# LFY1998/IPDM-PyTorch

Measured on AMD Instinct MI355X. Metric: CT slices/s (full proj+img partial-diffusion sample), higher is better.
Workload: dtype f32

## Files before the change

### include/ipdm_hip.h

```cpp
#ifndef IPDM_HIP_H
#define IPDM_HIP_H
#include <stddef.h>
#include <stdint.h>

#ifdef __cplusplus
extern "C" {
#endif

#define IPDM_OK 0
#define IPDM_ERR_INVALID (-1)
#define IPDM_ERR_HIP (-2)
#define IPDM_ERR_WORKSPACE (-3)
#define IPDM_ERR_UNSUPPORTED (-4)

const char *ipdm_last_error(void);
#define IPDM_ABI_VERSION 5
int ipdm_abi_version(void);

int ipdm_set_option(const char *name, int value);
int ipdm_get_option(const char *name, int *value);

typedef struct ipdm_fbp_geom {
    int32_t n_views, n_det, grid_n;
    double da, det_offset, dtheta_deg, source_origin, fov_half;
// ... 73 lines not shown
                       void *d_ws, size_t ws_bytes, void *stream);

typedef struct ipdm_reverse_args {
    int32_t mode;
    int32_t clip;
    int32_t guidance;
    double constant_guidance, lambda_power, eta;
    int32_t kernel_size;
    double amplitude;
    double p1[5], p2[3];
    uint64_t seed;
    int64_t slice_id0, draw0;
    const float *d_noise;
    const float *d_ldct;
} ipdm_reverse_args;

size_t ipdm_reverse_workspace_bytes(ipdm_unet *net, int32_t B, int32_t H, int32_t W);

int ipdm_reverse_pass(const ipdm_schedule *s, ipdm_unet *net, const float *d_x_in, const float *d_guide,
                      const float *d_Lambda, int32_t mh, int32_t mw, float *d_iter, int32_t B, int32_t H, int32_t W,
                      int32_t ts, const ipdm_reverse_args *a, void *d_ws, size_t ws_bytes, void *stream);

int ipdm_guided_reverse(const ipdm_schedule *s, ipdm_unet *net, const float *d_img, float *d_iters, int32_t B,
                        int32_t H, int32_t W, const int32_t *t_start, int32_t n_pass, const ipdm_reverse_args *a,
                        int64_t *draws_used, void *d_ws, size_t ws_bytes, void *stream);

#define IPDM_SLICE_IDS_MAX 64
int ipdm_randn_ids(float *d_out, int32_t B, int64_t n, uint64_t seed, const int64_t *slice_ids, int64_t draw,
                   void *stream);
int ipdm_q_sample_rng_ids(const ipdm_schedule *s, int32_t t, const float *d_x, float *d_out, int32_t B,
                          int64_t n_per_slice, uint64_t seed, const int64_t *slice_ids, int64_t draw, void *stream);
int ipdm_ddpm_step_rng_ids(const ipdm_schedule *s, int32_t t, const float *d_eps_pred, const float *d_x_t,
                           const float *d_x0, uint64_t seed, const int64_t *slice_ids, int64_t draw, float *d_out,
                           int32_t B, int32_t H, int32_t W, double lambda_scalar, const float *d_lambda_map, int32_t mh,
                           int32_t mw, int32_t clip_denoised, void *d_ws, size_t ws_bytes, void *stream);
int ipdm_reverse_pass_ids(const ipdm_schedule *s, ipdm_unet *net, const float *d_x_in, const float *d_guide,
                          const float *d_Lambda, int32_t mh, int32_t mw, float *d_iter, int32_t B, int32_t H, int32_t W,
                          int32_t ts, const ipdm_reverse_args *a, const int64_t *slice_ids, void *d_ws, size_t ws_bytes,
                          void *stream);

int ipdm_ddim_step_rng(const ipdm_schedule *s, int32_t t, int32_t t_prev, const float *d_eps_pred, const float *d_x_t,
                       const float *d_cond, uint64_t seed, int64_t slice_id0, int64_t draw, float *d_out, int32_t B,
                       int64_t n_per_slice, double lambda_scalar, double ddim_eta, int32_t clip_denoised, void *d_ws,
                       size_t ws_bytes, void *stream);

int ipdm_ddim_sequence(const char *method, int32_t timesteps, int32_t t_start, int32_t n, int32_t *seq, int32_t *prev);

#define IPDM_NOISE_COUNTER 1
#define IPDM_NOISE_INJECTED 2
typedef struct ipdm_sparse_args {
    int32_t clip_denoised;
    double ddim_eta, eta;
    int32_t noise;
    uint64_t seed;
    int64_t slice_id0, draw0;
    const float *d_noise;
} ipdm_sparse_args;

int ipdm_sparse_reverse(const ipdm_schedule *s, ipdm_unet *net, const float *d_cond, float *d_iters, int32_t B, int32_t H,
                        int32_t W, int32_t t_q, const int32_t *n_steps, int32_t n_pass, const int32_t *t_seq,
                        const int32_t *t_prev, const double *lambda, const ipdm_sparse_args *a, int64_t *draws_used,
                        void *d_ws, size_t ws_bytes, void *stream);

int ipdm_q_sample_rng_ts(const ipdm_schedule *s, const int32_t *ts, const float *d_x, float *d_out, int32_t B,
                         int64_t n_per_slice, uint64_t seed, const int64_t *slice_ids, int64_t draw, void *stream);
int ipdm_q_sample_ts(const ipdm_schedule *s, const int32_t *ts, const float *d_x, const float *d_noise, float *d_out, int32_t B,
                     int64_t n_per_slice, void *stream);
size_t ipdm_eps_sse_workspace_bytes(int32_t B);
int ipdm_eps_sse(const float *d_eps_pred, const float *d_noise, double *d_sse, int32_t B, int64_t n_per_slice, void *d_ws,
                 size_t ws_bytes, void *stream);
int ipdm_eps_sse_rng(const float *d_eps_pred, double *d_sse, int32_t B, int64_t n_per_slice, uint64_t seed,
                     const int64_t *slice_ids, int64_t draw, void *d_ws, size_t ws_bytes, void *stream);
size_t ipdm_eps_loss_workspace_bytes(ipdm_unet *net, int32_t B, int32_t H, int32_t W);
int ipdm_eps_loss(const ipdm_schedule *s, ipdm_unet *net, const float *d_x0, const int32_t *ts, double *d_sse, int32_t B,
                  int32_t H, int32_t W, uint64_t seed, const int64_t *slice_ids, int64_t draw, const float *d_noise, void *d_ws,
                  size_t ws_bytes, void *stream);

size_t ipdm_conv2d_grad_workspace_bytes(int32_t B, int32_t Cin, int32_t Cout, int32_t H, int32_t W, int32_t ksize,
                                        int32_t stride);
int32_t ipdm_conv2d_wgrad_slabs(int32_t B, int32_t Ho, int32_t Wo);
int ipdm_conv2d_fprop(const float *d_x, const float *d_w, const float *d_b, float *d_y, int32_t B, int32_t Cin, int32_t Cout,
                      int32_t H, int32_t W, int32_t ksize, int32_t stride, void *d_ws, size_t ws_bytes, void *stream);
int ipdm_conv2d_dgrad(const float *d_dy, const float *d_w, float *d_dx, int32_t B, int32_t Cin, int32_t Cout, int32_t H,
                      int32_t W, int32_t ksize, int32_t stride, void *d_ws, size_t ws_bytes, void *stream);
int ipdm_conv2d_wgrad(const float *d_x, const float *d_dy, float *d_dw, float *d_db, int32_t B, int32_t Cin, int32_t Cout,
                      int32_t H, int32_t W, int32_t ksize, int32_t stride, void *d_ws, size_t ws_bytes, void *stream);

int32_t ipdm_conv2d_wgrad_tuned_code(int32_t B, int32_t Cin, int32_t Cout, int32_t H, int32_t W, int32_t ksize, int32_t stride);
#define IPDM_WGRAD_PLAN_FIELDS 14
int32_t ipdm_conv2d_wgrad_tuned_plan(int32_t B, int32_t Cin, int32_t Cout, int32_t H, int32_t W, int32_t ksize, int32_t stride,
                                     int32_t *out, int32_t n);
#define IPDM_WGRAD_LAUNCH_FIELDS 9
int32_t ipdm_conv2d_wgrad_tuned_launch(int32_t B, int32_t Cin, int32_t Cout, int32_t H, int32_t W, int32_t ksize, int32_t stride,
                                       int32_t *out, int32_t n);
size_t ipdm_conv2d_wgrad_tuned_workspace_bytes(int32_t B, int32_t Cin, int32_t Cout, int32_t H, int32_t W, int32_t ksize,
                                               int32_t stride);
int ipdm_conv2d_wgrad_tuned(const float *d_x, const float *d_dy, float *d_dw, float *d_db, int32_t B, int32_t Cin, int32_t Cout,
                            int32_t H, int32_t W, int32_t ksize, int32_t stride, void *d_ws, size_t ws_bytes, void *stream);

int32_t ipdm_conv2d_wgrad_wino_code(int32_t B, int32_t Cin, int32_t Cout, int32_t H, int32_t W, int32_t ksize, int32_t stride);
#define IPDM_WGRAD_WINO_PLAN_FIELDS 11
int32_t ipdm_conv2d_wgrad_wino_plan(int32_t B, int32_t Cin, int32_t Cout, int32_t H, int32_t W, int32_t ksize, int32_t stride,
                                    int32_t *out, int32_t n);
size_t ipdm_conv2d_wgrad_wino_workspace_bytes(int32_t B, int32_t Cin, int32_t Cout, int32_t H, int32_t W, int32_t ksize,
                                              int32_t stride);
int ipdm_conv2d_wgrad_wino(const float *d_x, const float *d_dy, float *d_dw, float *d_db, int32_t B, int32_t Cin, int32_t Cout,
                           int32_t H, int32_t W, int32_t ksize, int32_t stride, void *d_ws, size_t ws_bytes, void *stream);

int32_t ipdm_conv2d_tuned_code(int32_t role, int32_t B, int32_t Cin, int32_t Cout, int32_t H, int32_t W, int32_t ksize, int32_t stride);
size_t ipdm_conv2d_tuned_workspace_bytes(int32_t role, int32_t B, int32_t Cin, int32_t Cout, int32_t H, int32_t W, int32_t ksize,
                                         int32_t stride);
int ipdm_conv2d_fprop_tuned(const float *d_x, const float *d_w, const float *d_b, float *d_y, int32_t B, int32_t Cin, int32_t Cout,
                            int32_t H, int32_t W, int32_t ksize, int32_t stride, void *d_ws, size_t ws_bytes, void *stream);
int ipdm_conv2d_dgrad_tuned(const float *d_dy, const float *d_w, float *d_dx, int32_t B, int32_t Cin, int32_t Cout, int32_t H,
                            int32_t W, int32_t ksize, int32_t stride, void *d_ws, size_t ws_bytes, void *stream);
size_t ipdm_conv_image_bytes(int32_t image, int32_t role, int32_t Cin, int32_t Cout, int32_t ksize, int32_t stride);
int ipdm_conv_pack_device(int32_t image, int32_t role, const float *d_w, int32_t Cin, int32_t Cout, int32_t ksize, int32_t stride,
                          void *d_image, void *stream);
int ipdm_conv_pack_host(int32_t image, int32_t role, const float *w_host, int32_t Cin, int32_t Cout, int32_t ksize, int32_t stride,
                        void *image_host);

size_t ipdm_gn_act_workspace_bytes(int32_t B, int32_t C, int32_t groups, int32_t HW);
int32_t ipdm_gn_act_plan(int32_t C, int32_t groups, int32_t HW, int32_t *split);
int ipdm_gn_act_fprop(const float *d_x, const float *d_shift, const float *d_gamma, const float *d_beta, float *d_y,
                      double *d_stats, int32_t B, int32_t C, int32_t groups, int32_t HW, double eps, int32_t act, void *d_ws,
                      size_t ws_bytes, void *stream);
int ipdm_gn_act_bgrad(const float *d_x, const float *d_shift, const float *d_gamma, const float *d_beta, const double *d_stats,
                      const float *d_dy, float *d_dx, float *d_dgamma, float *d_dbeta, float *d_dshift, int32_t B, int32_t C,
                      int32_t groups, int32_t HW, double eps, int32_t act, void *d_ws, size_t ws_bytes, void *stream);

size_t ipdm_attn_train_workspace_bytes(int32_t B, int32_t heads, int32_t d, int32_t T);
int32_t ipdm_attn_train_plan(int32_t d, int32_t T, int32_t out[4]);
int ipdm_attn_fprop(const float *d_qkv, float *d_out, float *d_lse, int32_t B, int32_t heads, int32_t d, int32_t T, void *d_ws,
                    size_t ws_bytes, void *stream);
int ipdm_attn_bgrad(const float *d_qkv, const float *d_out, const float *d_lse, const float *d_dout, float *d_dqkv, int32_t B,
                    int32_t heads, int32_t d, int32_t T, void *d_ws, size_t ws_bytes, void *stream);

int ipdm_op_conv2d(const float *d_x1, int32_t C1, const float *d_x2, int32_t C2, int32_t B, int32_t Hs,
                   int32_t Ws, int32_t H, int32_t W, const float *w_host, const float *b_host, int32_t Cout,
                   int32_t ksize, int32_t stride, int32_t act, int32_t groups, const float *gamma_host,
                   const float *beta_host, const float *d_res, float *d_out, void *stream);
int ipdm_op_conv_gn_conv(const float *d_x, int32_t C, int32_t B, int32_t H, int32_t W, const float *wA_host,
                         const float *bA_host, int32_t CA, int32_t ksA, int32_t strideA, const float *d_resA,
                         int32_t groups, const float *gamma_host, const float *beta_host, int32_t act,
                         const float *wB_host, const float *bB_host, int32_t CB, float *d_mid, float *d_out,
                         int32_t *fused_rows, void *stream);
int ipdm_op_up_conv_chain(const float *d_x, int32_t C, int32_t B, int32_t Hs, int32_t Ws, const float *wA_host,
                          const float *bA_host, int32_t CA, const float *d_skip, int32_t C2, int32_t groups,
                          const float *gamma_host, const float *beta_host, int32_t act, const float *wB_host,
                          const float *bB_host, int32_t CB, int32_t ksB, float *d_mid, float *d_out,
                          int32_t *used_up2, void *stream);
int ipdm_op_attention(const float *d_qkv, float *d_out, int32_t B, int32_t heads, int32_t d, int32_t T,
                      void *stream);

typedef struct ipdm_art_geom {
    float dso, dsd;
    int32_t nx, ny;
    float dx, dy, offset_x, offset_y;
    int32_t nr;
    float dr, offset_r, angle_start;
    int32_t na, ta_dimx, ta_dimy;
    float ta_deltax, ta_deltay;
} ipdm_art_geom;
typedef struct ipdm_art_plan ipdm_art_plan;
int ipdm_art_plan_create(const ipdm_art_geom *geom, const float *lut_area_host, const float *betas_host,
                         ipdm_art_plan **out);
int ipdm_art_plan_destroy(ipdm_art_plan *plan);
size_t ipdm_art_workspace_bytes(const ipdm_art_plan *plan, int32_t B);
int32_t ipdm_art_plan_info(const ipdm_art_plan *plan, int32_t out[6]);
int ipdm_art_reconstruct(ipdm_art_plan *plan, const float *d_proj, float *d_volume, int32_t B, int32_t nsart,
                         int32_t ntv, int32_t sample_rate, void *d_ws, size_t ws_bytes, void *stream);
int ipdm_art_project(ipdm_art_plan *plan, const float *d_volume, float *d_proj, int32_t B, void *d_ws,
                     size_t ws_bytes, void *stream);

#define IPDM_METRIC_PSNR 1u
#define IPDM_METRIC_SSIM 2u
#define IPDM_METRIC_FSIM 4u
#define IPDM_METRIC_VIF 8u
#define IPDM_METRIC_NQM 16u
typedef struct ipdm_metrics_plan ipdm_metrics_plan;
int ipdm_metrics_plan_create(int32_t H, int32_t W, ipdm_metrics_plan **out);
int ipdm_metrics_plan_destroy(ipdm_metrics_plan *plan);
size_t ipdm_metrics_workspace_bytes(const ipdm_metrics_plan *plan, int32_t B, uint32_t mask);
int ipdm_metrics(ipdm_metrics_plan *plan, const float *d_ref, int64_t ref_stride, const float *d_img, int32_t B,
                 uint32_t mask, double *d_out, void *d_ws, size_t ws_bytes, void *stream);
int64_t ipdm_metrics_table(const ipdm_metrics_plan *plan, int32_t which, void *host_out, int64_t cap_elems);

int ipdm_lowdose_noise(const float *d_proj, const float *d_z1, const float *d_z2, float *d_out, int32_t B,
                       int64_t n_per_slice, double factor, double n0, double ne, int32_t model, void *stream);
int ipdm_lowdose_noise_rng(const float *d_proj, float *d_out, int32_t B, int64_t n_per_slice, double factor, double n0,
                           double ne, int32_t model, uint64_t seed, int64_t slice_id0, int64_t draw0, void *stream);

size_t ipdm_yj_workspace_bytes(int32_t B);
int ipdm_yj_nll(const float *d_x, int32_t B, int64_t n_per_slice, const double *lambdas_host, double *nll_host, void *d_ws,
                size_t ws_bytes, void *stream);
int ipdm_yj_fit(const float *d_x, int32_t B, int64_t n_per_slice, double *params_host, int32_t *evals_host, void *d_ws,
                size_t ws_bytes, void *stream);
int ipdm_yj_apply(const float *d_x, float *d_out, int32_t B, int64_t n_per_slice, const double *params_host, void *stream);
int ipdm_yj_invert(const float *d_y, float *d_out, int32_t B, int64_t n_per_slice, const double *params_host, void *stream);
int ipdm_yj_fit_host(const float *x_host, int32_t B, int64_t n_per_slice, double *params_host, int32_t *evals_host);

typedef struct ipdm_adam_tensor {
    float *p;
    const float *g;
    float *m, *v;
    int64_t n;
} ipdm_adam_tensor;
typedef struct ipdm_adam_chunk {
    int32_t tensor, len;
    int64_t offset;
} ipdm_adam_chunk;
#define IPDM_ADAM_CHUNK 4096
int64_t ipdm_adam_chunks(const int64_t *sizes, int32_t n_tensors, ipdm_adam_chunk *out, int64_t cap);
int ipdm_adam_step(const ipdm_adam_tensor *d_tensors, int32_t n_tensors, const ipdm_adam_chunk *d_chunks, int64_t n_chunks,
                   double lr, double beta1, double beta2, double eps, double weight_decay, int64_t step, void *stream);
int ipdm_grad_sumsq(const ipdm_adam_tensor *d_tensors, int32_t n_tensors, const ipdm_adam_chunk *d_chunks, int64_t n_chunks,
                    double *d_partials, void *stream);
int ipdm_grad_clip_coef(const double *d_partials, int64_t n_partials, double max_norm, double *d_norm, float *d_coef, void *stream);
int ipdm_adam_step_ex(const ipdm_adam_tensor *d_tensors, int32_t n_tensors, const ipdm_adam_chunk *d_chunks, int64_t n_chunks,
                      double lr, double beta1, double beta2, double eps, double weight_decay, int64_t step,
                      const float *d_gscale, float *const *d_ema, double ema_decay, void *stream);
#define IPDM_CROP_MAX 256
int ipdm_crop_patches(const float *d_slices, float *d_out, int32_t n, int32_t m, int32_t H, int32_t W, int32_t ph, int32_t pw,
                      const int32_t *offsets_host, int32_t div10, void *stream);

#define IPDM_PROF_CLASSES 8
int ipdm_profile_begin(int32_t max_launches);
int ipdm_profile_begin_classes(int32_t max_launches, uint32_t class_mask);
int ipdm_profile_end(double *out_flops, double *out_ms, int64_t *out_launches, int32_t n_classes);
int ipdm_clock_probe(uint64_t *d_out, int32_t samples, int32_t period_us, void *stream);

int ipdm_bench_conv2d(int32_t B, int32_t C1, int32_t C2, int32_t H, int32_t W, int32_t Cout, int32_t ksize,
                      int32_t stride, int32_t act, int32_t with_res, int32_t iters, float *avg_ms);
int ipdm_bench_attention(int32_t B, int32_t heads, int32_t d, int32_t T, int32_t iters, float *avg_ms);
int32_t ipdm_conv_layout_code(int32_t Cout, int32_t ksize, int32_t stride);
int32_t ipdm_conv_kernel_code(int32_t B, int32_t Cout, int32_t Cin, int32_t ksize, int32_t stride, int32_t H, int32_t W);
int32_t ipdm_conv_kernel_code_stats(int32_t B, int32_t Cout, int32_t Cin, int32_t ksize, int32_t stride, int32_t H, int32_t W);
int32_t ipdm_attention_kernel_code(int32_t d);
int ipdm_attention_plan(int32_t B, int32_t heads, int32_t d, int32_t T, int32_t out[6]);

#ifdef __cplusplus
}
#endif
#endif
```

### ipdm-pytorch_amd/_lib.py

```python
import ctypes as C
import os

_HERE = os.path.dirname(os.path.abspath(__file__))
LIB_PATH = os.environ.get("IPDM_LIB_PATH") or os.path.join(_HERE, "libipdm_hip.so")


class IpdmError(RuntimeError):
    pass


class FbpGeom(C.Structure):
    _fields_ = [("n_views", C.c_int32), ("n_det", C.c_int32), ("grid_n", C.c_int32),
                ("da", C.c_double), ("det_offset", C.c_double), ("dtheta_deg", C.c_double),
                ("source_origin", C.c_double), ("fov_half", C.c_double)]


class UnetCfg(C.Structure):
    _fields_ = [("in_channels", C.c_int32), ("model_channels", C.c_int32), ("out_channels", C.c_int32),
                ("num_res_blocks", C.c_int32), ("num_heads", C.c_int32), ("n_mult", C.c_int32),
                ("n_attn", C.c_int32), ("channel_mult", C.c_double * 16),
                ("attention_resolutions", C.c_int32 * 16)]


class ReverseArgs(C.Structure):
    _fields_ = [("mode", C.c_int32), ("clip", C.c_int32), ("guidance", C.c_int32),
                ("constant_guidance", C.c_double), ("lambda_power", C.c_double), ("eta", C.c_double),
                ("kernel_size", C.c_int32), ("amplitude", C.c_double),
                ("p1", C.c_double * 5), ("p2", C.c_double * 3),
                ("seed", C.c_uint64), ("slice_id0", C.c_int64), ("draw0", C.c_int64),
                ("d_noise", C.c_void_p), ("d_ldct", C.c_void_p)]


class SparseArgs(C.Structure):
    _fields_ = [("clip_denoised", C.c_int32), ("ddim_eta", C.c_double), ("eta", C.c_double), ("noise", C.c_int32),
                ("seed", C.c_uint64), ("slice_id0", C.c_int64), ("draw0", C.c_int64), ("d_noise", C.c_void_p)]


NOISE_COUNTER, NOISE_INJECTED = 1, 2

_vp, _i32, _i64, _u64, _f32, _f64, _sz = C.c_void_p, C.c_int32, C.c_int64, C.c_uint64, C.c_float, C.c_double, C.c_size_t

ABI_VERSION = 5
PROF_CLASSES = 8
SLICE_IDS_MAX = 64
ADAM_CHUNK = 4096

PROTOTYPES = {
    "ipdm_last_error": (C.c_char_p, []),
    "ipdm_abi_version": (C.c_int, []),
    "ipdm_set_option": (C.c_int, [C.c_char_p, _i32]),
    "ipdm_get_option": (C.c_int, [C.c_char_p, C.POINTER(_i32)]),
    "ipdm_fbp_plan_create": (C.c_int, [C.POINTER(FbpGeom), C.POINTER(_vp)]),
    "ipdm_fbp_plan_destroy": (C.c_int, [_vp]),
    "ipdm_fbp_workspace_bytes": (_sz, [_vp, _i32]),
    "ipdm_fbp_forward": (C.c_int, [_vp, _vp, _vp, _i32, _i32, _f32, _vp, _sz, _vp]),
    "ipdm_fbp_filter": (C.c_int, [_vp, _vp, _vp, _i32, _i32, _f32, _vp]),
    "ipdm_fbp_backproject": (C.c_int, [_vp, _vp, _vp, _i32, _i32, _vp]),
    "ipdm_fbp_index_map": (C.c_int, [_vp, _vp, _i32, _vp, _vp]),
    "ipdm_fbp_table": (_i64, [_vp, _i32, _vp, _i64]),
    "ipdm_sharpen3x3": (C.c_int, [_vp, _vp, _i32, _i32, _i32, _f32, _vp]),
    "ipdm_schedule_create": (C.c_int, [_i32, _f64, C.POINTER(_vp)]),
    "ipdm_schedule_destroy": (C.c_int, [_vp]),
    "ipdm_schedule_coeffs": (C.c_int, [_vp, _i32, C.POINTER(_f32 * 8)]),
    "ipdm_schedule_alpha_cumprod": (C.c_int, [_vp, _i32, C.POINTER(_f32)]),
    "ipdm_cosine_lambda": (C.c_int, [_i32, _f64, _i32, C.POINTER(_f64)]),
    "ipdm_ddim_step": (C.c_int, [_vp, _i32, _i32, _vp, _vp, _vp, _vp, _vp, _i32, _i64, _f64, _f64, _i32, _vp, _sz, _vp]),
    "ipdm_randn": (C.c_int, [_vp, _i32, _i64, _u64, _i64, _i64, _vp]),
    "ipdm_q_sample": (C.c_int, [_vp, _i32, _vp, _vp, _vp, _i64, _vp]),
    "ipdm_ddpm_workspace_bytes": (_sz, [_i32]),
    "ipdm_ddpm_step": (C.c_int, [_vp, _i32, _vp, _vp, _vp, _vp, _vp, _i32, _i32, _i32, _f64, _vp, _i32, _i32,
                                 _i32, _vp, _sz, _vp]),
    "ipdm_clamp": (C.c_int, [_vp, _vp, _i64, _i32, _vp]),
    "ipdm_axpbypcz": (C.c_int, [_vp, _vp, _vp, _vp, _i64, _f64, _f64, _f64, _vp]),
    "ipdm_guidance_workspace_bytes": (_sz, [_i32, _i32, _i32]),
    "ipdm_guidance_map": (C.c_int, [_vp, _vp, _vp, _vp, _i32, _i32, _i32, _i32, _f64, _i32, C.POINTER(_f64),
                                    C.POINTER(_f64), _vp, _sz, _vp]),
    "ipdm_lambda_ratio": (C.c_int, [_vp, _vp, _i64, _i32, _i32, _vp]),
    "ipdm_slice_median": (C.c_int, [_vp, _vp, _i32, _i64, _vp, _sz, _vp]),
    "ipdm_unet_param_count": (C.c_int, [C.POINTER(UnetCfg)]),
    "ipdm_unet_param_info": (C.c_int, [C.POINTER(UnetCfg), _i32, C.c_char_p, _i32, C.POINTER(_i32 * 4),
                                       C.POINTER(_i32)]),
    "ipdm_unet_create": (C.c_int, [C.POINTER(UnetCfg), C.POINTER(_vp), _i32, C.POINTER(_vp)]),
    "ipdm_unet_destroy": (C.c_int, [_vp]),
    "ipdm_unet_workspace_bytes": (_sz, [_vp, _i32, _i32, _i32]),
    "ipdm_unet_forward": (C.c_int, [_vp, _vp, _i32, _vp, _i32, _i32, _i32, _vp, _sz, _vp]),
    "ipdm_unet_forward_graph": (C.c_int, [_vp, _vp, _i32, _vp, _i32, _i32, _i32, _vp, _sz, _vp]),
    "ipdm_q_sample_rng": (C.c_int, [_vp, _i32, _vp, _vp, _i32, _i64, _u64, _i64, _i64, _vp]),
    "ipdm_ddpm_step_rng": (C.c_int, [_vp, _i32, _vp, _vp, _vp, _u64, _i64, _i64, _vp, _i32, _i32, _i32, _f64, _vp, _i32, _i32,
                                     _i32, _vp, _sz, _vp]),
    "ipdm_reverse_workspace_bytes": (_sz, [_vp, _i32, _i32, _i32]),
    "ipdm_reverse_pass": (C.c_int, [_vp, _vp, _vp, _vp, _vp, _i32, _i32, _vp, _i32, _i32, _i32, _i32, C.POINTER(ReverseArgs),
                                    _vp, _sz, _vp]),
    "ipdm_guided_reverse": (C.c_int, [_vp, _vp, _vp, _vp, _i32, _i32, _i32, C.POINTER(_i32), _i32, C.POINTER(ReverseArgs),
                                      C.POINTER(_i64), _vp, _sz, _vp]),
    "ipdm_randn_ids": (C.c_int, [_vp, _i32, _i64, _u64, C.POINTER(_i64), _i64, _vp]),
    "ipdm_q_sample_rng_ids": (C.c_int, [_vp, _i32, _vp, _vp, _i32, _i64, _u64, C.POINTER(_i64), _i64, _vp]),
    "ipdm_ddpm_step_rng_ids": (C.c_int, [_vp, _i32, _vp, _vp, _vp, _u64, C.POINTER(_i64), _i64, _vp, _i32, _i32, _i32, _f64, _vp,
                                         _i32, _i32, _i32, _vp, _sz, _vp]),
    "ipdm_reverse_pass_ids": (C.c_int, [_vp, _vp, _vp, _vp, _vp, _i32, _i32, _vp, _i32, _i32, _i32, _i32, C.POINTER(ReverseArgs),
                                        C.POINTER(_i64), _vp, _sz, _vp]),
    "ipdm_ddim_step_rng": (C.c_int, [_vp, _i32, _i32, _vp, _vp, _vp, _u64, _i64, _i64, _vp, _i32, _i64, _f64, _f64, _i32, _vp, _sz,
                                     _vp]),
    "ipdm_ddim_sequence": (C.c_int, [C.c_char_p, _i32, _i32, _i32, C.POINTER(_i32), C.POINTER(_i32)]),
    "ipdm_sparse_reverse": (C.c_int, [_vp, _vp, _vp, _vp, _i32, _i32, _i32, _i32, C.POINTER(_i32), _i32, C.POINTER(_i32),
                                      C.POINTER(_i32), C.POINTER(_f64), C.POINTER(SparseArgs), C.POINTER(_i64), _vp, _sz, _vp]),
    "ipdm_q_sample_rng_ts": (C.c_int, [_vp, C.POINTER(_i32), _vp, _vp, _i32, _i64, _u64, C.POINTER(_i64), _i64, _vp]),
    "ipdm_q_sample_ts": (C.c_int, [_vp, C.POINTER(_i32), _vp, _vp, _vp, _i32, _i64, _vp]),
    "ipdm_eps_sse_workspace_bytes": (_sz, [_i32]),
    "ipdm_eps_sse": (C.c_int, [_vp, _vp, _vp, _i32, _i64, _vp, _sz, _vp]),
    "ipdm_eps_sse_rng": (C.c_int, [_vp, _vp, _i32, _i64, _u64, C.POINTER(_i64), _i64, _vp, _sz, _vp]),
    "ipdm_eps_loss_workspace_bytes": (_sz, [_vp, _i32, _i32, _i32]),
    "ipdm_eps_loss": (C.c_int, [_vp, _vp, _vp, C.POINTER(_i32), _vp, _i32, _i32, _i32, _u64, C.POINTER(_i64), _i64, _vp, _vp, _sz,
                                _vp]),
    "ipdm_conv2d_grad_workspace_bytes": (_sz, [_i32] * 7),
    "ipdm_conv2d_wgrad_slabs": (_i32, [_i32, _i32, _i32]),
    "ipdm_conv2d_fprop": (C.c_int, [_vp, _vp, _vp, _vp] + [_i32] * 7 + [_vp, _sz, _vp]),
    "ipdm_conv2d_dgrad": (C.c_int, [_vp, _vp, _vp] + [_i32] * 7 + [_vp, _sz, _vp]),
    "ipdm_conv2d_wgrad": (C.c_int, [_vp, _vp, _vp, _vp] + [_i32] * 7 + [_vp, _sz, _vp]),
    "ipdm_conv2d_wgrad_tuned_code": (_i32, [_i32] * 7),
    "ipdm_conv2d_wgrad_tuned_plan": (_i32, [_i32] * 7 + [C.POINTER(_i32), _i32]),
    "ipdm_conv2d_wgrad_tuned_launch": (_i32, [_i32] * 7 + [C.POINTER(_i32), _i32]),
    "ipdm_conv2d_wgrad_tuned_workspace_bytes": (_sz, [_i32] * 7),
    "ipdm_conv2d_wgrad_tuned": (C.c_int, [_vp, _vp, _vp, _vp] + [_i32] * 7 + [_vp, _sz, _vp]),
    "ipdm_conv2d_wgrad_wino_code": (_i32, [_i32] * 7),
    "ipdm_conv2d_wgrad_wino_plan": (_i32, [_i32] * 7 + [C.POINTER(_i32), _i32]),
    "ipdm_conv2d_wgrad_wino_workspace_bytes": (_sz, [_i32] * 7),
    "ipdm_conv2d_wgrad_wino": (C.c_int, [_vp, _vp, _vp, _vp] + [_i32] * 7 + [_vp, _sz, _vp]),
    "ipdm_conv2d_tuned_code": (_i32, [_i32] * 8),
    "ipdm_conv2d_tuned_workspace_bytes": (_sz, [_i32] * 8),
    "ipdm_conv2d_fprop_tuned": (C.c_int, [_vp, _vp, _vp, _vp] + [_i32] * 7 + [_vp, _sz, _vp]),
    "ipdm_conv2d_dgrad_tuned": (C.c_int, [_vp, _vp, _vp] + [_i32] * 7 + [_vp, _sz, _vp]),
    "ipdm_conv_image_bytes": (_sz, [_i32] * 6),
    "ipdm_conv_pack_device": (C.c_int, [_i32, _i32, _vp] + [_i32] * 4 + [_vp, _vp]),
    "ipdm_conv_pack_host": (C.c_int, [_i32, _i32, _vp] + [_i32] * 4 + [_vp]),
    "ipdm_gn_act_workspace_bytes": (_sz, [_i32] * 4),
    "ipdm_gn_act_plan": (_i32, [_i32, _i32, _i32, C.POINTER(_i32)]),
    "ipdm_gn_act_fprop": (C.c_int, [_vp] * 6 + [_i32] * 4 + [_f64, _i32, _vp, _sz, _vp]),
    "ipdm_gn_act_bgrad": (C.c_int, [_vp] * 10 + [_i32] * 4 + [_f64, _i32, _vp, _sz, _vp]),
    "ipdm_attn_train_workspace_bytes": (_sz, [_i32] * 4),
    "ipdm_attn_train_plan": (_i32, [_i32, _i32, C.POINTER(_i32 * 4)]),
    "ipdm_attn_fprop": (C.c_int, [_vp] * 3 + [_i32] * 4 + [_vp, _sz, _vp]),
    "ipdm_attn_bgrad": (C.c_int, [_vp] * 5 + [_i32] * 4 + [_vp, _sz, _vp]),
    "ipdm_op_conv2d": (C.c_int, [_vp, _i32, _vp, _i32, _i32, _i32, _i32, _i32, _i32, _vp, _vp, _i32, _i32, _i32,
                                 _i32, _i32, _vp, _vp, _vp, _vp, _vp]),
    "ipdm_op_conv_gn_conv": (C.c_int, [_vp, _i32, _i32, _i32, _i32, _vp, _vp, _i32, _i32, _i32, _vp, _i32, _vp, _vp, _i32, _vp, _vp,
                                       _i32, _vp, _vp, C.POINTER(_i32), _vp]),
    "ipdm_op_up_conv_chain": (C.c_int, [_vp, _i32, _i32, _i32, _i32, _vp, _vp, _i32, _vp, _i32, _i32, _vp, _vp, _i32, _vp, _vp,
                                        _i32, _i32, _vp, _vp, C.POINTER(_i32), _vp]),
    "ipdm_profile_begin": (C.c_int, [_i32]),
    "ipdm_profile_begin_classes": (C.c_int, [_i32, C.c_uint32]),
    "ipdm_clock_probe": (C.c_int, [_vp, _i32, _i32, _vp]),
    "ipdm_profile_end": (C.c_int, [C.POINTER(_f64 * PROF_CLASSES), C.POINTER(_f64 * PROF_CLASSES), C.POINTER(_i64 * PROF_CLASSES), _i32]),
    "ipdm_bench_conv2d": (C.c_int, [_i32] * 11 + [C.POINTER(_f32)]),
    "ipdm_bench_attention": (C.c_int, [_i32] * 5 + [C.POINTER(_f32)]),
    "ipdm_op_attention": (C.c_int, [_vp, _vp, _i32, _i32, _i32, _i32, _vp]),
    "ipdm_conv_layout_code": (_i32, [_i32, _i32, _i32]),
    "ipdm_conv_kernel_code": (_i32, [_i32, _i32, _i32, _i32, _i32, _i32, _i32]),
    "ipdm_conv_kernel_code_stats": (_i32, [_i32, _i32, _i32, _i32, _i32, _i32, _i32]),
    "ipdm_attention_kernel_code": (_i32, [_i32]),
    "ipdm_attention_plan": (C.c_int, [_i32, _i32, _i32, _i32, C.POINTER(_i32 * 6)]),
    "ipdm_art_plan_create": (C.c_int, [_vp, _vp, _vp, C.POINTER(_vp)]),
    "ipdm_art_plan_destroy": (C.c_int, [_vp]),
    "ipdm_art_workspace_bytes": (C.c_size_t, [_vp, _i32]),
    "ipdm_art_plan_info": (_i32, [_vp, C.POINTER(_i32 * 6)]),
    "ipdm_art_reconstruct": (C.c_int, [_vp, _vp, _vp, _i32, _i32, _i32, _i32, _vp, C.c_size_t, _vp]),
    "ipdm_art_project": (C.c_int, [_vp, _vp, _vp, _i32, _vp, C.c_size_t, _vp]),
    "ipdm_metrics_plan_create": (C.c_int, [_i32, _i32, C.POINTER(_vp)]),
    "ipdm_metrics_plan_destroy": (C.c_int, [_vp]),
    "ipdm_metrics_workspace_bytes": (_sz, [_vp, _i32, C.c_uint32]),
    "ipdm_metrics": (C.c_int, [_vp, _vp, _i64, _vp, _i32, C.c_uint32, _vp, _vp, _sz, _vp]),
    "ipdm_metrics_table": (_i64, [_vp, _i32, _vp, _i64]),
    "ipdm_lowdose_noise": (C.c_int, [_vp, _vp, _vp, _vp, _i32, _i64, _f64, _f64, _f64, _i32, _vp]),
    "ipdm_lowdose_noise_rng": (C.c_int, [_vp, _vp, _i32, _i64, _f64, _f64, _f64, _i32, _u64, _i64, _i64, _vp]),
    "ipdm_yj_workspace_bytes": (_sz, [_i32]),
    "ipdm_yj_nll": (C.c_int, [_vp, _i32, _i64, C.POINTER(_f64), C.POINTER(_f64), _vp, _sz, _vp]),
    "ipdm_yj_fit": (C.c_int, [_vp, _i32, _i64, C.POINTER(_f64), C.POINTER(_i32), _vp, _sz, _vp]),
    "ipdm_yj_apply": (C.c_int, [_vp, _vp, _i32, _i64, C.POINTER(_f64), _vp]),
    "ipdm_yj_invert": (C.c_int, [_vp, _vp, _i32, _i64, C.POINTER(_f64), _vp]),
    "ipdm_yj_fit_host": (C.c_int, [_vp, _i32, _i64, C.POINTER(_f64), C.POINTER(_i32)]),
    "ipdm_adam_chunks": (_i64, [_vp, _i32, _vp, _i64]),
    "ipdm_adam_step": (C.c_int, [_vp, _i32, _vp, _i64, _f64, _f64, _f64, _f64, _f64, _i64, _vp]),
    "ipdm_grad_sumsq": (C.c_int, [_vp, _i32, _vp, _i64, _vp, _vp]),
    "ipdm_grad_clip_coef": (C.c_int, [_vp, _i64, _f64, _vp, _vp, _vp]),
    "ipdm_adam_step_ex": (C.c_int, [_vp, _i32, _vp, _i64, _f64, _f64, _f64, _f64, _f64, _i64, _vp, _vp, _f64, _vp]),
    "ipdm_crop_patches": (C.c_int, [_vp, _vp] + [_i32] * 6 + [_vp, _i32, _vp]),
}

_lib = None


def lib():
    global _lib
    if _lib is None:
        if not os.path.isfile(LIB_PATH):
            raise IpdmError("%s not found: the HIP extension is mandatory (no CPU fallback). "
                            "Run __graft_entry__.build()." % LIB_PATH)
        try:
            import torch
        except ImportError:
            pass
        handle = C.CDLL(LIB_PATH)
        for name, (res, args) in PROTOTYPES.items():
            fn = getattr(handle, name)
            fn.restype = res
            fn.argtypes = args
        got = handle.ipdm_abi_version()
        if got != ABI_VERSION:
            raise IpdmError("%s has ABI version %d, this package binds version %d (include/ipdm_hip.h): rebuild with "
                            "__graft_entry__.build()" % (LIB_PATH, got, ABI_VERSION))
        _lib = handle
    return _lib


def call(name, *args):
    rc = getattr(lib(), name)(*args)
    if rc != 0:
        raise IpdmError("%s failed (%d): %s" % (name, rc, lib().ipdm_last_error().decode()))
    return rc


def set_option(name, value):
    old = get_option(name)
    call("ipdm_set_option", name.encode(), int(value))
    return old


def get_option(name):
    v = C.c_int32()
    call("ipdm_get_option", name.encode(), C.byref(v))
    return v.value


class option:

    def __init__(self, name, value):
        self.name, self.value = name, value

    def __enter__(self):
        self.old = set_option(self.name, self.value)
        return self

    def __exit__(self, *exc):
        set_option(self.name, self.old)
        return False


def ptr(t):
    if t is None:
        return None
    if hasattr(t, "data_ptr"):
        assert t.is_contiguous(), "non-contiguous tensor handed to the C ABI"
        return C.c_void_p(t.data_ptr())
    return C.c_void_p(t.ctypes.data)


def current_stream():
    import torch
    return C.c_void_p(torch.cuda.current_stream().cuda_stream)
```

### ipdm-pytorch_amd/csrc/attn.hip

```cpp
#include <cstdlib>
#include "unet_kernels.h"
#include "attn_common.h"

using namespace ipdm;
using namespace ipdm::attn;

namespace {

constexpr int KV = 64;
constexpr int KP = 68;
constexpr int VP = 68;

template <int D, int QT>
__global__ void __launch_bounds__(256, 2) attention_kernel(const float *__restrict__ qkv, float *__restrict__ out,
                                                           int heads, int T, float scale)
{
    __shared__ __attribute__((aligned(16))) float k_lds[KV * KP];
    __shared__ __attribute__((aligned(16))) float v_lds[D * VP];
    const int tid = threadIdx.x, lane = tid & 63, wave = tid >> 6;
    const int l31 = lane & 31, lh = lane >> 5;
    const int bh = blockIdx.y;
    const int b = bh / heads, head = bh % heads;
    const float *qp = qkv + ((size_t)b * heads * 3 * D + (size_t)head * 3 * D) * T;
    const float *kp = qp + (size_t)D * T;
// ... 299 lines not shown
#pragma unroll
    for (int qt = 0; qt < QT; ++qt) {
        const int t = t0 + qt * 32 + l31;
        if (t < T) {
            constexpr bool seq = ZSEQ;
            const float inv = 1.0f / (seq ? den : l_run[qt]);
#pragma unroll
            for (int cb = 0; cb < CB; ++cb)
#pragma unroll
                for (int r = 0; r < 16; ++r) {
                    const int c = cb * 32 + crow(r, lh);
                    op[(size_t)c * T + t] = (seq ? num[seq ? cb : 0][r] : o[qt][cb][r]) * inv;
                }
        }
    }
}

template <int D>
__global__ void __launch_bounds__(256) attention_combine_kernel(const float *__restrict__ part, float *__restrict__ out, int T, int Z, int ntiles)
{
    const int t = blockIdx.x * 256 + threadIdx.x, bh = blockIdx.y, c0 = blockIdx.z * 16;
    if (t >= T) return;
    const size_t slice = (size_t)gridDim.y * (D + 2) * T;
    const float *p = part + (size_t)bh * (D + 2) * T;
    const int tps = (ntiles + Z - 1) / Z;
    SliceWeights w[8];
    float M = -INFINITY, den = 0.0f;
#pragma unroll
    for (int z = 0; z < 8; ++z)
        if (z < Z && z * tps < ntiles) {
            w[z] = slice_weights(M, p[z * slice + (size_t)D * T + t]);
            den = slice_fold(den, p[z * slice + (size_t)(D + 1) * T + t], w[z]);
        }
    const float inv = 1.0f / den;
#pragma unroll 4
    for (int c = c0; c < c0 + 16; ++c) {
        float acc = 0.0f;
#pragma unroll
        for (int z = 0; z < 8; ++z)
            if (z < Z && z * tps < ntiles) acc = slice_fold(acc, p[z * slice + (size_t)c * T + t], w[z]);
        out[((size_t)bh * D + c) * T + t] = acc * inv;
    }
}

__global__ void __launch_bounds__(256) attention_combine_any_kernel(const float *__restrict__ part, float *__restrict__ out, int T, int Z, int ntiles, int d)
{
    const int t = blockIdx.x * 256 + threadIdx.x, bh = blockIdx.y, c0 = blockIdx.z * 16;
    if (t >= T) return;
    const size_t slice = (size_t)gridDim.y * (d + 2) * T;
    const float *p = part + (size_t)bh * (d + 2) * T;
    const int tps = (ntiles + Z - 1) / Z;
    SliceWeights w[8];
    float M = -INFINITY, den = 0.0f;
#pragma unroll
    for (int z = 0; z < 8; ++z)
        if (z < Z && z * tps < ntiles) {
            w[z] = slice_weights(M, p[z * slice + (size_t)d * T + t]);
            den = slice_fold(den, p[z * slice + (size_t)(d + 1) * T + t], w[z]);
        }
    const float inv = 1.0f / den;
    for (int c = c0; c < min(c0 + 16, d); ++c) {
        float acc = 0.0f;
#pragma unroll
        for (int z = 0; z < 8; ++z)
            if (z < Z && z * tps < ntiles) acc = slice_fold(acc, p[z * slice + (size_t)c * T + t], w[z]);
        out[((size_t)bh * d + c) * T + t] = acc * inv;
    }
}

int attention_kv_split(int B, int heads, int d, int T)
{
    const bool off = opt(OPT_ATTN_NO_KVSPLIT) != 0;
    (void)B;
    if (off || d != 64) return 1;
    const long wg = (long)cdiv(T, 128) * heads;
    if (wg > 128) return 1;
    const int ntiles = cdiv(T, KV);
    int Z = wg <= 32 ? 8 : (wg <= 64 ? 4 : 2);
    if (Z > ntiles / 2) Z = ntiles / 2;
    return Z < 2 ? 1 : Z;
}

struct AttnPlan {
    int family;
    int qt;
    int Z;
    int form;
    int tps;
    int empty;
};

bool attention_on_gen(int d)
{
    const int any = opt(OPT_ATTN_ANY_DIM);
    return any == 2 || (any == 1 && d != 64 && d != 32);
}

int attention_head_dim_check(int d)
{
    if (opt(OPT_ATTN_ANY_DIM) == 0) {
        if (d != 64 && d != 32) { set_error("attention: head dim %d unsupported (kernel is specialised for 64 and 32)", d); return IPDM_ERR_UNSUPPORTED; }
    } else if (d < 1 || d > ATTN_GEN_DMAX) {
        set_error("attention: head dim %d unsupported (1 .. %d under attn_any_dim)", d, ATTN_GEN_DMAX);
        return IPDM_ERR_UNSUPPORTED;
    }
    return IPDM_OK;
}

AttnPlan attention_plan(int B, int heads, int d, int T, bool have_scratch)
{
    const int ntiles = cdiv(T, KV);
    AttnPlan p = {0, 1, 1, 0, ntiles, 0};
    if (attention_on_gen(d)) {
        p.family = 3;
        p.Z = have_scratch ? attention_gen_split(heads, d, T) : 1;
        if (p.Z > 1) {
            p.form = 1;
            p.tps = cdiv(ntiles, p.Z);
            p.empty = p.Z - cdiv(ntiles, p.tps);
        }
        return p;
    }
    if (d != 64) return p;
    const long wg2 = (long)cdiv(T, 256) * B * heads, wg1 = (long)cdiv(T, 128) * B * heads;
    if (opt(OPT_ATTN_LEGACY) != 0) {
        p.qt = wg2 >= 512 && (wg2 % 512 == 0 || wg2 >= 4 * 512) ? 2 : 1;
        return p;
    }
    const bool exact = opt(OPT_ATTN_EXACT_F32) != 0;
    p.family = exact ? 1 : 2;
    p.Z = have_scratch ? attention_kv_split(B, heads, d, T) : 1;
    if (exact) {
        const auto eff = [](long wg) { return (double)wg / (double)(((wg + 255) / 256) * 256); };
        if (p.Z == 1 && wg2 >= 256 && eff(wg2) >= eff(wg1) - 0.03) p.qt = 2;
    }
    if (p.Z > 1) {
        p.form = p.Z >= 4 && opt(OPT_ATTN_NO_ZSEQ) == 0 && wg1 >= 192 ? 2 : 1;
        p.tps = cdiv(ntiles, p.Z);
        p.empty = p.Z - cdiv(ntiles, p.tps);
    }
    return p;
}

}

namespace ipdm {

size_t attention_scratch_floats(int B, int heads, int d, int T)
{
    const int Z = attention_on_gen(d) ? attention_gen_split(heads, d, T) : attention_kv_split(B, heads, d, T);
    return Z > 1 ? (size_t)Z * B * heads * (d + 2) * T : 0;
}

int attention_launch(const float *qkv, float *out, int B, int heads, int d, int T, hipStream_t st, float *scratch, float *planes)
{
    IPDM_REQUIRE(qkv && out && B > 0 && heads > 0 && T > 0, "attention: bad argument");
    if (int rc = attention_head_dim_check(d)) return rc;
    const float scale = (float)(1.0 / sqrt(sqrt((double)d)));
    const bool prof = prof_enabled();
    if (prof) prof_before(2, st);
    const AttnPlan p = attention_plan(B, heads, d, T, scratch != nullptr);
    const int Z = p.Z;
    const bool seq = p.form == 2, q2 = p.qt == 2;
    if (p.family == 3) {
        if (int rc = attention_gen_launch(qkv, out, B, heads, d, T, scale, Z, scratch, st)) return rc;
        if (p.form == 1)
            hipLaunchKernelGGL(attention_combine_any_kernel, dim3(cdiv(T, 256), B * heads, cdiv(d, 16)), dim3(256), 0, st, scratch, out, T, Z, cdiv(T, KV), d);
    } else if (p.family == 2) {
        if (!attention_planes_floats(B, heads, d, T)) planes = nullptr;
        attention_bx3_launch(qkv, out, B, heads, T, scale, Z, seq, scratch, planes, st);
        if (p.form == 1)
            hipLaunchKernelGGL((attention_combine_kernel<64>), dim3(cdiv(T, 256), B * heads, 4), dim3(256), 0, st, scratch, out, T, Z, cdiv(T, KV));
    } else if (p.family == 1) {
        constexpr size_t lds = (size_t)2 * (KV * KP + 64 * VP) * sizeof(float);
        if (int rc = ensure_dynamic_lds((const void *)attention_ws_kernel<64, 1>, lds)) return rc;
        if (int rc = ensure_dynamic_lds((const void *)attention_ws_kernel<64, 2>, lds)) return rc;
        if (int rc = ensure_dynamic_lds((const void *)attention_ws_kernel<64, 1, true>, lds)) return rc;
        dim3 grid(cdiv(T, q2 ? 256 : 128), B * heads, seq ? 1 : Z);
        if (q2) hipLaunchKernelGGL((attention_ws_kernel<64, 2>), grid, dim3(512), lds, st, qkv, out, heads, T, scale, 1, (float *)nullptr, 1);
        else if (seq) hipLaunchKernelGGL((attention_ws_kernel<64, 1, true>), grid, dim3(512), lds, st, qkv, out, heads, T, scale, 1, (float *)nullptr, Z);
        else hipLaunchKernelGGL((attention_ws_kernel<64, 1>), grid, dim3(512), lds, st, qkv, out, heads, T, scale, Z, scratch, 1);
        if (p.form == 1)
            hipLaunchKernelGGL((attention_combine_kernel<64>), dim3(cdiv(T, 256), B * heads, 4), dim3(256), 0, st, scratch, out, T, Z, cdiv(T, KV));
    } else if (d == 64) {
        dim3 grid(cdiv(T, q2 ? 256 : 128), B * heads);
        if (q2) hipLaunchKernelGGL((attention_kernel<64, 2>), grid, dim3(256), 0, st, qkv, out, heads, T, scale);
        else hipLaunchKernelGGL((attention_kernel<64, 1>), grid, dim3(256), 0, st, qkv, out, heads, T, scale);
    } else {
        dim3 grid(cdiv(T, 128), B * heads);
        hipLaunchKernelGGL((attention_kernel<32, 1>), grid, dim3(256), 0, st, qkv, out, heads, T, scale);
    }
    if (prof) prof_after(2, 4.0 * B * heads * (double)T * T * d, st);
    IPDM_LAUNCH_CHECK();
    return IPDM_OK;
}

}

extern "C" int32_t ipdm_attention_kernel_code(int32_t d)
{
    if (opt(OPT_ATTN_ANY_DIM) != 0 && (d < 1 || d > ATTN_GEN_DMAX)) return 0;
    return d == 64 || attention_on_gen(d) ? attention_plan(1, 1, d, 1, true).family : 0;
}

extern "C" int ipdm_attention_plan(int32_t B, int32_t heads, int32_t d, int32_t T, int32_t out[6])
{
    IPDM_REQUIRE(out && B > 0 && heads > 0 && T > 0, "attention_plan: bad argument");
    if (int rc = attention_head_dim_check(d)) return rc;
    const AttnPlan p = attention_plan(B, heads, d, T, true);
    out[0] = p.family; out[1] = p.qt; out[2] = p.Z; out[3] = p.form; out[4] = p.tps; out[5] = p.empty;
    return IPDM_OK;
}

extern "C" int ipdm_op_attention(const float *d_qkv, float *d_out, int32_t B, int32_t heads, int32_t d, int32_t T,
                                 void *stream)
{
    float *scratch = nullptr, *planes = nullptr;
    if (ipdm::attention_scratch_floats(B, heads, d, T)) {
        IPDM_HIP_CHECK(hipMalloc((void **)&scratch, ipdm::attention_scratch_floats(B, heads, d, T) * sizeof(float)));
    }
    if (const size_t pfl = ipdm::attention_planes_floats(B, heads, d, T)) {
        hipError_t e = hipMalloc((void **)&planes, pfl * sizeof(float));
        if (e == hipSuccess) e = hipMemsetAsync(planes, 0xFF, pfl * sizeof(float), (hipStream_t)stream);
        if (e != hipSuccess) { (void)hipFree(scratch); (void)hipFree(planes); IPDM_HIP_CHECK(e); }
    }
    const int rc = ipdm::attention_launch(d_qkv, d_out, B, heads, d, T, (hipStream_t)stream, scratch, planes);
    if (scratch || planes) {
        (void)hipStreamSynchronize((hipStream_t)stream);
        (void)hipFree(scratch);
        (void)hipFree(planes);
    }
    return rc;
}
```

### ipdm-pytorch_amd/csrc/attn_bx3.hip

```cpp
#include "unet_kernels.h"
#include "attn_common.h"
#include "attn_pipe_schedule.h"
#include <type_traits>

using namespace ipdm;
using namespace ipdm::attn;

typedef unsigned u32x4 __attribute__((ext_vector_type(4)));
typedef __bf16 bf16x8 __attribute__((ext_vector_type(8)));
typedef __bf16 bf16x2 __attribute__((ext_vector_type(2)));

namespace {

constexpr int D = 64;
constexpr int KT = 32;
constexpr int KP = 72;
constexpr int VP = 40;
constexpr int KPLANE = KT * KP, VPLANE = D * VP;
constexpr int STAGE = 3 * KPLANE + 3 * VPLANE;
constexpr int PCHUNK = 256;
constexpr int TILE_CHUNKS = 6 * PCHUNK;

__device__ inline unsigned pk_bf16(float a, float b)
{
    return __builtin_bit_cast(unsigned, bf16x2{(__bf16)a, (__bf16)b});
}
struct Split3 { unsigned h[3]; };
__device__ inline Split3 split3(float a, float b)
{
    Split3 s;
    s.h[0] = pk_bf16(a, b);
    const float ra = a - __builtin_bit_cast(float, s.h[0] << 16), rb = b - __builtin_bit_cast(float, s.h[0] & 0xffff0000u);
    s.h[1] = pk_bf16(ra, rb);
    const float qa = ra - __builtin_bit_cast(float, s.h[1] << 16), qb = rb - __builtin_bit_cast(float, s.h[1] & 0xffff0000u);
    s.h[2] = pk_bf16(qa, qb);
    return s;
}

__device__ inline f32x16 mma(u32x4 a, u32x4 b, f32x16 c)
{
    return __builtin_amdgcn_mfma_f32_32x32x16_bf16(__builtin_bit_cast(bf16x8, a), __builtin_bit_cast(bf16x8, b), c, 0, 0, 0);
}
template <bool FIRST>
__device__ inline f32x16 mma6(const u32x4 (&a)[3], const u32x4 (&b)[3], f32x16 c)
{
    if (FIRST) {
        const f32x16 zero = {0, 0, 0, 0, 0, 0, 0, 0, 0, 0, 0, 0, 0, 0, 0, 0};
        c = mma(a[0], b[2], zero);
        asm volatile("" ::"v"(a[0]), "v"(b[2]));
    } else {
        c = mma(a[0], b[2], c);
    }
    c = mma(a[2], b[0], c);
    c = mma(a[1], b[1], c);
    c = mma(a[0], b[1], c);
    c = mma(a[1], b[0], c);
    return mma(a[0], b[0], c);
}

template <int FROM, int TO, class F>
__device__ inline void static_for(F &&f)
{
    if constexpr (FROM < TO) {
        f(std::integral_constant<int, FROM>{});
        static_for<FROM + 1, TO>(f);
    }
}

__global__ void __launch_bounds__(256) attention_presplit_kernel(const float *__restrict__ qkv, u32x4 *__restrict__ planes, int heads, int T)
{
    constexpr int FP = KT + 1;
    __shared__ float kf[D * FP], vf[D * FP];
    const int bh = blockIdx.y, b = bh / heads, head = bh % heads;
    const float *qp = qkv + ((size_t)b * heads * 3 * D + (size_t)head * 3 * D) * T;
    const int s0 = blockIdx.x * KT, tid = threadIdx.x;
    {
        const int key = tid & 31, c0 = tid >> 5;
        const bool in = s0 + key < T;
#pragma unroll
        for (int r = 0; r < 8; ++r) {
            const int c = c0 + 8 * r;
            kf[c * FP + key] = in ? qp[(size_t)(D + c) * T + s0 + key] : 0.0f;
            vf[c * FP + key] = in ? qp[(size_t)(2 * D + c) * T + s0 + key] : 0.0f;
        }
    }
    __syncthreads();
    u32x4 *pt = planes + ((size_t)bh * gridDim.x + blockIdx.x) * TILE_CHUNKS + tid;
    const int ks = tid >> 3, kg = tid & 7, vc = tid >> 2, vg = tid & 3;
    const int vkey = 16 * (vg >> 1) + 4 * (vg & 1);
    u32x4 hk[3], hv[3];
#pragma unroll
    for (int e = 0; e < 8; e += 2) {
        const Split3 sk = split3(kf[(8 * kg + e) * FP + ks], kf[(8 * kg + e + 1) * FP + ks]);
        const Split3 sv = split3(vf[vc * FP + vkey + 8 * (e >> 2) + (e & 3)], vf[vc * FP + vkey + 8 * (e >> 2) + (e & 3) + 1]);
#pragma unroll
        for (int p = 0; p < 3; ++p) { hk[p][e / 2] = sk.h[p]; hv[p][e / 2] = sv.h[p]; }
    }
#pragma unroll
    for (int p = 0; p < 3; ++p) {
        pt[p * PCHUNK] = hk[p];
        pt[(3 + p) * PCHUNK] = hv[p];
    }
}

template <bool ZSEQ, bool PRE, bool PIPE>
__global__ void __launch_bounds__(384, 3) attention_bx3_kernel(const float *__restrict__ qkv, float *__restrict__ out, int heads, int T,
                                                                float scale, int zsplit, float *__restrict__ part, int zseq,
                                                                const u32x4 *__restrict__ planes)
{
    static_assert(PRE || !PIPE, "the pipelined loop copies planes");
    static_assert(!ZSEQ || !PIPE, "the pipelined loop does not fit the slice walk's registers");
    __shared__ __attribute__((aligned(16))) unsigned short lds[2 * STAGE];
    const int bh = blockIdx.y;
    const int b = bh / heads, head = bh % heads;
    const float *qp = qkv + ((size_t)b * heads * 3 * D + (size_t)head * 3 * D) * T;
    const int ntiles = (T + KT - 1) / KT;
    const int nslice = ZSEQ ? zseq : zsplit;
    const int tps = 2 * (((T + 63) / 64 + nslice - 1) / nslice);
    const int it0 = ZSEQ ? 0 : blockIdx.z * tps, it1 = ZSEQ ? ntiles : min(ntiles, it0 + tps);
    const int npipe = max(it1 - it0, 0);

    if (__builtin_amdgcn_readfirstlane(threadIdx.x >> 6) >= 4) {
        if constexpr (PRE) {
            const int tid = threadIdx.x - 256;
            const __amdgpu_buffer_rsrc_t rs = __builtin_amdgcn_make_buffer_rsrc((void *)(planes + (size_t)bh * ntiles * TILE_CHUNKS), 0,
                                                                                  ntiles * TILE_CHUNKS * 16, 0x00020000);
            int ko[2], vo[2];
#pragma unroll
            for (int n = 0; n < 2; ++n) {
                const int j = tid + 128 * n;
                ko[n] = (j >> 3) * KP + 8 * (j & 7);
                vo[n] = 3 * KPLANE + (j >> 2) * VP + 8 * (j & 3);
            }
            u32x4 r[12];
            const auto load = [&](int it) {
#pragma unroll
                for (int i = 0; i < 12; ++i)
                    r[i] = __builtin_bit_cast(u32x4, __builtin_amdgcn_raw_buffer_load_b128(rs, tid * 16, (it * TILE_CHUNKS + 128 * i) * 16, 0));
            };
            const auto store = [&](int it) {
                unsigned short *st = lds + (it & 1) * STAGE;
#pragma unroll
                for (int i = 0; i < 6; ++i) {
                    *reinterpret_cast<u32x4 *>(st + (i >> 1) * KPLANE + ko[i & 1]) = r[i];
                    *reinterpret_cast<u32x4 *>(st + (i >> 1) * VPLANE + vo[i & 1]) = r[6 + i];
                }
            };
            if constexpr (PIPE) {
                const auto load_half = [&](int it, int h) {
#pragma unroll
                    for (int i = 6 * h; i < 6 * h + 6; ++i)
                        r[i] = __builtin_bit_cast(u32x4, __builtin_amdgcn_raw_buffer_load_b128(rs, tid * 16, (it * TILE_CHUNKS + 128 * i) * 16, 0));
                };
                const auto store_k = [&](int it) {
                    unsigned short *st = lds + attn_pipe::slot(it) * STAGE;
#pragma unroll
                    for (int i = 0; i < 6; ++i) *reinterpret_cast<u32x4 *>(st + (i >> 1) * KPLANE + ko[i & 1]) = r[i];
                };
                const auto store_v = [&](int it) {
                    unsigned short *st = lds + attn_pipe::slot(it) * STAGE;
#pragma unroll
                    for (int i = 0; i < 6; ++i) *reinterpret_cast<u32x4 *>(st + (i >> 1) * VPLANE + vo[i & 1]) = r[6 + i];
                };
                if (npipe > 0) load_half(attn_pipe::k_stored(it0, npipe, 0), 0);
                for (int b = 0; b < attn_pipe::barriers(npipe); ++b) {
                    const int ks = attn_pipe::k_stored(it0, npipe, b), vs = attn_pipe::v_stored(it0, npipe, b);
                    if (ks != attn_pipe::NONE) store_k(ks);
                    if (vs != attn_pipe::NONE) store_v(vs);
                    const int kl = attn_pipe::k_loaded(it0, npipe, b), vl = attn_pipe::v_loaded(it0, npipe, b);
                    if (kl != attn_pipe::NONE) load_half(kl, 0);
                    if (vl != attn_pipe::NONE) load_half(vl, 1);
                    __syncthreads();
                }
                return;
            }
            if (it0 < it1) load(it0);
            for (int it = it0; it < it1; ++it) {
                store(it);
                if (it + 1 < it1) load(it + 1);
                __syncthreads();
            }
            return;
        }
        const int tid = threadIdx.x - 256;
        const __amdgpu_buffer_rsrc_t rs = __builtin_amdgcn_make_buffer_rsrc((void *)qp, 0, 3 * D * T * 4, 0x00020000);
        int ks[2], kg[2], koff[2], vg[2], vc[2], vkey[2], voff[2];
#pragma unroll
        for (int n = 0; n < 2; ++n) {
            const int idx = tid + 128 * n;
            ks[n] = idx & 31;
// ... 175 lines not shown
                    if constexpr (g >= 3 && g < 11 && g % 2 == 1) split_b(0, (g - 3) / 2);
                }
                if constexpr (PIN) __builtin_amdgcn_sched_barrier(0);
            });
            if constexpr (HAS_PV) {
                const unsigned short *vt = lds + attn_pipe::slot(it) * STAGE + 3 * KPLANE + l31 * VP + 8 * lh;
                const auto vterms = [&](int cb, int kb) {
#pragma unroll
                    for (int p = 0; p < 3; ++p) v[cb][p] = *reinterpret_cast<const u32x4 *>(vt + cb * 32 * VP + p * VPLANE + 16 * kb);
                };
                vterms(0, 0);

                static_for<0, 24>([&](auto gc) {
                    constexpr int g = decltype(gc)::value, kb = g / 12, cb = (g / 6) % 2, j = g % 6;
                    constexpr int TA[6] = {0, 2, 1, 0, 1, 0}, TB[6] = {2, 0, 1, 1, 0, 0};
                    o[cb] = mma(v[cb][TA[j]], pp[kb][TB[j]], o[cb]);
                    if constexpr (HAS_S || g >= 2) asm volatile("" ::"v"(ka[g % 2]));
                    if constexpr (g >= 2) asm volatile("" ::"v"(pb[g % 2]));
                    ka[g % 2] = v[cb][TA[j]];
                    pb[g % 2] = pp[kb][TB[j]];
                    if constexpr (g == 2) vterms(1, 0);
                    if constexpr (kb == 0 && j == 5) vterms(cb, 1);
                    if constexpr (g < 8 && g % 2 == 0) split_a(1, g / 2);
                    if constexpr (g < 8 && g % 2 == 1) split_b(1, g / 2);
                    if constexpr (HAS_S && g == 12) { sacc = snext; row_max_alpha(); }
                    if constexpr (PIN) __builtin_amdgcn_sched_barrier(0);
                });
                __builtin_amdgcn_sched_barrier(0);
            }
            if constexpr (HAS_S && !HAS_PV) {
                sacc = snext;
                row_max_alpha();
            }
        };
        if (attn_pipe::barriers(npipe) > 0) {
            __syncthreads();
            interval(std::true_type{}, std::false_type{}, 0);
            for (int b = 1; b <= attn_pipe::steady(npipe); ++b) {
                __syncthreads();
                interval(std::true_type{}, std::true_type{}, b);
            }
            __syncthreads();
            interval(std::false_type{}, std::true_type{}, attn_pipe::barriers(npipe) - 1);
        }
    } else
    for (int it = it0; it < it1; ++it) {
        const int s0 = it * KT;
        __syncthreads();
        reserve();
        const unsigned short *st = lds + (it & 1) * STAGE;
        f32x16 sacc;
        u32x4 k[3];
        {
            const unsigned short *krow = st + l31 * KP + 8 * lh;
#pragma unroll
            for (int kb = 0; kb < 4; ++kb) {
#pragma unroll
                for (int p = 0; p < 3; ++p) k[p] = *reinterpret_cast<const u32x4 *>(krow + p * KPLANE + 16 * kb);
                sacc = kb == 0 ? mma6<true>(k, q[kb], sacc) : mma6<false>(k, q[kb], sacc);
            }
        }
        __builtin_amdgcn_sched_barrier(0);
        if (s0 + KT > T) {
#pragma unroll
            for (int r = 0; r < 16; ++r)
                if (s0 + crow(r, lh) >= T) sacc[r] = -INFINITY;
        }
        float mx = sacc[0];
#pragma unroll
        for (int r = 1; r < 16; ++r) mx = fmaxf(mx, sacc[r]);
        mx = halves_max(mx);
        const float m_new = fmaxf(m_run, mx);
        const float alpha = __builtin_amdgcn_exp2f((m_run - m_new) * LOG2E);
        float rs0 = 0.0f, rs1 = 0.0f;
#pragma unroll
        for (int r = 0; r < 16; r += 2) {
            sacc[r] = __builtin_amdgcn_exp2f((sacc[r] - m_new) * LOG2E);
            sacc[r + 1] = __builtin_amdgcn_exp2f((sacc[r + 1] - m_new) * LOG2E);
            rs0 += sacc[r];
            rs1 += sacc[r + 1];
        }
        const float rs = halves_sum(rs0 + rs1);
        asm volatile("" ::"v"(k[0]), "v"(k[1]), "v"(k[2]));
        l_run = l_run * alpha + rs;
        m_run = m_new;
        if (__any(alpha != 1.0f)) {
#pragma unroll
            for (int cb = 0; cb < 2; ++cb)
#pragma unroll
                for (int r = 0; r < 16; ++r) o[cb][r] *= alpha;
        }
#pragma unroll
        for (int kb = 0; kb < 2; ++kb)
#pragma unroll
            for (int e = 0; e < 8; e += 2) {
                const Split3 s = split3(sacc[8 * kb + e], sacc[8 * kb + e + 1]);
#pragma unroll
                for (int p = 0; p < 3; ++p) pp[kb][p][e / 2] = s.h[p];
            }
        __builtin_amdgcn_sched_barrier(0);
#pragma unroll
        for (int cb = 0; cb < 2; ++cb) {
            const unsigned short *vrow = st + 3 * KPLANE + (cb * 32 + l31) * VP + 8 * lh;
#pragma unroll
            for (int kb = 0; kb < 2; ++kb)
#pragma unroll
                for (int p = 0; p < 3; ++p) v[kb][p] = *reinterpret_cast<const u32x4 *>(vrow + p * VPLANE + 16 * kb);
#pragma unroll
            for (int kb = 0; kb < 2; ++kb) o[cb] = mma6<false>(v[kb], pp[kb], o[cb]);
        }
        __builtin_amdgcn_sched_barrier(0);
        if constexpr (ZSEQ) if (it + 1 == slice_end || it + 1 == it1) {
            const SliceWeights w = slice_weights(M_all, m_run);
            den = slice_fold(den, l_run, w);
#pragma unroll
            for (int cb = 0; cb < 2; ++cb)
#pragma unroll
                for (int r = 0; r < 16; ++r) { num[cb][r] = slice_fold(num[cb][r], o[cb][r], w); o[cb][r] = 0.0f; }
            m_run = -INFINITY;
            l_run = 0.0f;
            slice_end += tps;
        }
    }
    if (t >= T) { reserve(); return; }
    if (zsplit > 1) {
        float *pq = part + ((size_t)blockIdx.z * gridDim.y + bh) * (D + 2) * T;
#pragma unroll
        for (int cb = 0; cb < 2; ++cb)
#pragma unroll
            for (int r = 0; r < 16; ++r) pq[(size_t)(cb * 32 + crow(r, lh)) * T + t] = o[cb][r];
        if (lh == 0) { pq[(size_t)D * T + t] = m_run; pq[(size_t)(D + 1) * T + t] = l_run; }
        reserve();
        return;
    }
    float *op = out + ((size_t)b * heads * D + (size_t)head * D) * T;
    const float inv = 1.0f / (ZSEQ ? den : l_run);
#pragma unroll
    for (int cb = 0; cb < 2; ++cb)
#pragma unroll
        for (int r = 0; r < 16; ++r) op[(size_t)(cb * 32 + crow(r, lh)) * T + t] = (ZSEQ ? num[ZSEQ ? cb : 0][r] : o[cb][r]) * inv;
    reserve();
}

}

namespace ipdm {

size_t attention_planes_floats(int B, int heads, int d, int T)
{
    if (d != D || opt(OPT_ATTN_EXACT_F32) || opt(OPT_ATTN_LEGACY) || opt(OPT_ATTN_NO_PRESPLIT) || opt(OPT_ATTN_ANY_DIM) == 2) return 0;
    return (size_t)B * heads * cdiv(T, KT) * TILE_CHUNKS * 4;
}

void attention_bx3_launch(const float *qkv, float *out, int B, int heads, int T, float scale, int Z, bool seq, float *scratch,
                          float *planes, hipStream_t st)
{
    const dim3 grid(cdiv(T, 128), B * heads, seq ? 1 : Z);
    u32x4 *pl = reinterpret_cast<u32x4 *>(planes);
    if (pl) hipLaunchKernelGGL(attention_presplit_kernel, dim3(cdiv(T, KT), B * heads), dim3(256), 0, st, qkv, pl, heads, T);
    const bool pipe = pl && !seq && !opt(OPT_ATTN_NO_PIPELINE);
    const auto launch = [&](auto kernel, int zsplit, float *part, int zseq) {
        hipLaunchKernelGGL(kernel, grid, dim3(384), 0, st, qkv, out, heads, T, scale, zsplit, part, zseq, pl);
    };
    if (seq) {
        if (pl) launch(attention_bx3_kernel<true, true, false>, 1, nullptr, Z);
        else launch(attention_bx3_kernel<true, false, false>, 1, nullptr, Z);
    } else {
        if (pipe) launch(attention_bx3_kernel<false, true, true>, Z, scratch, 1);
        else if (pl) launch(attention_bx3_kernel<false, true, false>, Z, scratch, 1);
        else launch(attention_bx3_kernel<false, false, false>, Z, scratch, 1);
    }
}

}
```

### ipdm-pytorch_amd/csrc/attn_common.h

```cpp
#pragma once
#include <hip/hip_runtime.h>
#include "kernel_util.h"

namespace ipdm {
namespace attn {

constexpr float LOG2E = 1.4426950408889634f;

__device__ inline float halves_max(float x)
{
    float a = x, b = x;
    asm volatile("s_nop 1\n\tv_permlane32_swap_b32 %0, %1" : "+v"(a), "+v"(b));
    return fmaxf(a, b);
}
__device__ inline float halves_sum(float x)
{
    float a = x, b = x;
    asm volatile("s_nop 1\n\tv_permlane32_swap_b32 %0, %1" : "+v"(a), "+v"(b));
    return a + b;
}

struct SliceWeights { float a, b; };
__device__ inline SliceWeights slice_weights(float &M, float m_k)
{
    const float Mn = fmaxf(M, m_k);
    SliceWeights w;
    w.a = __builtin_amdgcn_exp2f((M - Mn) * LOG2E);
    w.b = __builtin_amdgcn_exp2f((m_k - Mn) * LOG2E);
    M = Mn;
    return w;
}
__device__ inline float slice_fold(float acc, float v, SliceWeights w) { return fmaf(acc, w.a, v * w.b); }

}
}
```

### ipdm-pytorch_amd/csrc/common.h

```cpp
#pragma once
#include <hip/hip_runtime.h>
#include <cstdarg>
#include <cstdio>
#include <cstring>
#include <string>
#include <vector>
#include "../../include/ipdm_hip.h"

namespace ipdm {

void set_error(const char *fmt, ...);

#define IPDM_HIP_CHECK(expr)                                                                   \
    do {                                                                                       \
        hipError_t e_ = (expr);                                                                \
        if (e_ != hipSuccess) {                                                                \
            ipdm::set_error("%s failed: %s (%s:%d)", #expr, hipGetErrorString(e_), __FILE__,  \
                            __LINE__);                                                         \
            return IPDM_ERR_HIP;                                                               \
        }                                                                                      \
    } while (0)

#define IPDM_REQUIRE(cond, ...)                   \
    do {                                          \
        if (!(cond)) {                            \
            ipdm::set_error(__VA_ARGS__);         \
            return IPDM_ERR_INVALID;              \
        }                                         \
    } while (0)

#define IPDM_LAUNCH_CHECK() IPDM_HIP_CHECK(hipGetLastError())

static inline int cdiv(long a, long b) { return (int)((a + b - 1) / b); }
static inline size_t align_up(size_t v, size_t a) { return (v + a - 1) / a * a; }

enum Opt {
    OPT_CONV_NO_UP2,
    OPT_CONV_NO_WUP2,
    OPT_CONV_LEGACY, OPT_CONV1X1_LEGACY, OPT_CONVS2_LEGACY,
    OPT_CONV_NO_DIRECT, OPT_DIRECT_NO_PLANAR, OPT_DIRECT_MAX_CIN, OPT_DIRECT_NO_S2, OPT_DIRECT_NO_SKIP_FUSE,
    OPT_CONV_DBG, OPT_CONV_VEC4_STRICT, OPT_CONV_NO_SPLITK, OPT_CONV_NO_WINO, OPT_WINO_V1, OPT_WINO2_MIN_TILES, OPT_CONV1X1_NO_QUARTER, OPT_CONV_NO_PW, OPT_PW_ITEM, OPT_PW_FORCE,
    OPT_CONV_NM,
    OPT_GN_TWO_STAGE, OPT_GN_UNFUSED,
    OPT_UNET_TRANSPOSE,
    OPT_ATTN_NO_KVSPLIT, OPT_ATTN_LEGACY, OPT_ATTN_NO_ZSEQ,
    OPT_ART_PER_VIEW,
    OPT_CONV_BF16X3,
    OPT_ATTN_EXACT_F32,
    OPT_ATTN_NO_PRESPLIT,
    OPT_ATTN_NO_PIPELINE,
    OPT_GN_TRAIN_ONE_PASS_MAX,
    OPT_ATTN_ANY_DIM,
    OPT_ATTN_TRAIN_ANY_DIM,
    OPT_CONV_TUNED_ALL,
    OPT_COUNT
};
int opt(Opt o);
bool opt_per_call(int o);
const char *opt_name(int o);
void opt_snapshot(int (&dst)[OPT_COUNT]);
int opt_changed_since(const int (&rec)[OPT_COUNT]);
std::vector<int> opt_per_call_values();

int ensure_dynamic_lds(const void *kernel, size_t bytes);
int device_cu_count();

int unet_io_channels(const ipdm_unet *net, int *cin, int *cout);

__device__ inline double wave_sum(double v)
{
#pragma unroll
    for (int o = 32; o > 0; o >>= 1) v += __shfl_down(v, o, 64);
    return v;
}
__device__ inline float wave_sum(float v)
{
#pragma unroll
    for (int o = 32; o > 0; o >>= 1) v += __shfl_down(v, o, 64);
    return v;
}
__device__ inline float wave_max(float v)
{
#pragma unroll
    for (int o = 32; o > 0; o >>= 1) v = fmaxf(v, __shfl_down(v, o, 64));
    return v;
}

}
```

### ipdm-pytorch_amd/csrc/common.hip

```cpp
#include <cctype>
#include <cstdlib>
#include <mutex>
#include <strings.h>
#include <set>
#include <utility>
#include "common.h"

namespace ipdm {
static thread_local char g_err[512] = "";
void set_error(const char *fmt, ...)
{
    va_list ap;
    va_start(ap, fmt);
    vsnprintf(g_err, sizeof(g_err), fmt, ap);
    va_end(ap);
}

namespace {
std::mutex g_attr_mu;
std::set<std::pair<const void *, int>> g_attr_done;
int g_cus[64];
}

namespace {
struct OptDef { const char *name; int def; bool per_call; int lo = 0, hi = 1; };
const OptDef g_opt_def[OPT_COUNT] = {
    {"conv_no_up2", 0, true},
    {"conv_no_wup2", 0, true},
    {"conv_legacy", 0, false}, {"conv1x1_legacy", 0, false}, {"convs2_legacy", 0, false},
    {"conv_no_direct", 0, false}, {"direct_no_planar", 0, false},
    {"direct_max_cin", 160, false, 0, 160},
    {"direct_no_s2", 0, false}, {"direct_no_skip_fuse", 0, true},
    {"conv_dbg", 0, true, 0, 0x3ff}, {"conv_vec4_strict", 0, false}, {"conv_no_splitk", 0, false},
    {"conv_no_wino", 0, true}, {"wino_v1", 0, true}, {"wino2_min_tiles", 192, true, 0, 1 << 24},
    {"conv1x1_no_quarter", 0, true}, {"conv_no_pw", 0, true}, {"pw_item", 0, true, 0, 2}, {"pw_force", 0, true}, {"conv_nm", 0, true, 0, 2},
    {"gn_two_stage", 0, true}, {"gn_unfused", 0, true},
    {"unet_transpose", -1, true, -1, 1},
    {"attn_no_kvsplit", 0, false}, {"attn_legacy", 0, false}, {"attn_no_zseq", 0, true},
    {"art_per_view", 0, true},
    {"conv_bf16x3", 0, true},
    {"attn_exact_f32", 0, true},
    {"attn_no_presplit", 0, true},
    {"attn_no_pipeline", 0, true},
    {"gn_train_one_pass_max", 0, true, 0, 16384},
    {"attn_any_dim", 0, true, 0, 2},
    {"attn_train_any_dim", 0, true},
    {"conv_tuned_all", 0, true},
};
bool opt_value_ok(int i, int v)
{
    return v >= g_opt_def[i].lo && v <= g_opt_def[i].hi;
}
std::mutex g_opt_mu;
int g_opt_val[OPT_COUNT];
bool g_opt_init = false;

void opt_init_locked()
{
    if (g_opt_init) return;
    for (int i = 0; i < OPT_COUNT; ++i) {
        char env[64] = "IPDM_";
        size_t n = 5;
        for (const char *c = g_opt_def[i].name; *c && n + 1 < sizeof(env); ++c) env[n++] = (char)toupper((unsigned char)*c);
        env[n] = 0;
        const char *e = getenv(env);
        g_opt_val[i] = g_opt_def[i].def;
        if (e) {
            char *end = nullptr;
            const long v = strtol(e, &end, 10);
            const int want = (end != e) ? (int)v : 1;
            if (opt_value_ok(i, want)) g_opt_val[i] = want;
            else fprintf(stderr, "libipdm_hip: %s=%s is outside the option's range [%d, %d]: ignored\n", env, e, g_opt_def[i].lo, g_opt_def[i].hi);
        }
    }
    g_opt_init = true;
}
}

int opt(Opt o)
{
    std::lock_guard<std::mutex> lk(g_opt_mu);
    opt_init_locked();
    return g_opt_val[o];
}
bool opt_per_call(int o) { return g_opt_def[o].per_call; }
const char *opt_name(int o) { return g_opt_def[o].name; }
void opt_snapshot(int (&dst)[OPT_COUNT])
{
    std::lock_guard<std::mutex> lk(g_opt_mu);
    opt_init_locked();
    for (int i = 0; i < OPT_COUNT; ++i) dst[i] = g_opt_val[i];
}
std::vector<int> opt_per_call_values()
{
    std::lock_guard<std::mutex> lk(g_opt_mu);
    opt_init_locked();
    std::vector<int> v;
    for (int i = 0; i < OPT_COUNT; ++i)
        if (g_opt_def[i].per_call) v.push_back(g_opt_val[i]);
    return v;
}
int opt_changed_since(const int (&rec)[OPT_COUNT])
{
    std::lock_guard<std::mutex> lk(g_opt_mu);
    opt_init_locked();
    for (int i = 0; i < OPT_COUNT; ++i)
        if (!g_opt_def[i].per_call && g_opt_val[i] != rec[i]) return i;
    return -1;
}
static int opt_find(const char *name)
{
    if (!name) return -1;
    if (!strncmp(name, "IPDM_", 5) || !strncmp(name, "ipdm_", 5)) name += 5;
    for (int i = 0; i < OPT_COUNT; ++i)
        if (!strcasecmp(name, g_opt_def[i].name)) return i;
    return -1;
}

int ensure_dynamic_lds(const void *kernel, size_t bytes)
{
    int dev = 0;
    IPDM_HIP_CHECK(hipGetDevice(&dev));
    std::lock_guard<std::mutex> lk(g_attr_mu);
    if (g_attr_done.count({kernel, dev})) return IPDM_OK;
    IPDM_HIP_CHECK(hipFuncSetAttribute(kernel, hipFuncAttributeMaxDynamicSharedMemorySize, (int)bytes));
    g_attr_done.insert({kernel, dev});
    return IPDM_OK;
}

int device_cu_count()
{
    int dev = 0, v = 0;
    if (hipGetDevice(&dev) != hipSuccess || dev < 0 || dev >= 64) return 256;
    std::lock_guard<std::mutex> lk(g_attr_mu);
    if (!g_cus[dev])
        g_cus[dev] = (hipDeviceGetAttribute(&v, hipDeviceAttributeMultiprocessorCount, dev) == hipSuccess && v > 0) ? v : 256;
    return g_cus[dev];
}
}

extern "C" const char *ipdm_last_error(void) { return ipdm::g_err; }
extern "C" int ipdm_abi_version(void) { return IPDM_ABI_VERSION; }

extern "C" int ipdm_set_option(const char *name, int value)
{
    const int i = ipdm::opt_find(name);
    IPDM_REQUIRE(i >= 0, "ipdm_set_option: unknown option '%s'", name ? name : "(null)");
    IPDM_REQUIRE(ipdm::opt_value_ok(i, value), "ipdm_set_option: %s = %d is outside [%d, %d]", ipdm::g_opt_def[i].name, value,
                 ipdm::g_opt_def[i].lo, ipdm::g_opt_def[i].hi);
    std::lock_guard<std::mutex> lk(ipdm::g_opt_mu);
    ipdm::opt_init_locked();
    ipdm::g_opt_val[i] = value;
    return IPDM_OK;
}

extern "C" int ipdm_get_option(const char *name, int *value)
{
    const int i = ipdm::opt_find(name);
    IPDM_REQUIRE(i >= 0 && value, "ipdm_get_option: unknown option '%s'", name ? name : "(null)");
    *value = ipdm::opt((ipdm::Opt)i);
    return IPDM_OK;
}
```

### ipdm-pytorch_amd/csrc/conv_plan.hip

```cpp
#include "common.h"
#include "unet_kernels.h"

namespace ipdm {

ConvPlan conv_plan(const ConvArgs &args, bool want_stats, bool may_split)
{
    ConvPlan p;
    ConvArgs a = args;
    a.ksplit = 1;
    if (!a.w_interleave) {
        if (!opt(OPT_CONV_NO_DIRECT) && conv_direct_eligible(a)) {
            p.code = (!a.sk_w && conv_nm_eligible(a)) ? 6 : 5;
            p.up2 = conv_direct_up2_eligible(a);
            p.stats_rows = conv_direct_stats_rows(a);
        } else { p.code = 8; p.stats_rows = conv_igemm_stats_rows(a); }
    } else if (conv_up2_eligible(a)) {
        p.code = conv_wup2_eligible(a) ? 11 : 7;
        p.up2 = p.out_planar = true;
        p.stats_rows = conv_up2_stats_rows(a);
    } else {
        const int S = conv_ws_split(a);
        if (S == 1 && conv_pw_eligible(a, want_stats)) {
            p.code = 10;
            p.stats_rows = conv_pw_stats_rows(a);
        } else {
            const bool v1 = opt(OPT_WINO_V1) != 0;
            if (conv_wino_eligible(a) && (S == 1 || (!v1 && conv_wino_split(a) > 1))) {
                if (S > 1 && may_split) p.ksplit = conv_wino_split(a);
                p.code = p.ksplit > 1 ? 9 : conv_wino3_eligible(a) ? 12 : (!v1 && conv_wino2_eligible(a)) ? 2 : 1;
            } else {
                if (may_split) p.ksplit = S;
                p.code = p.ksplit > 1 ? 4 : 3;
            }
            p.stats_rows = p.ksplit > 1 ? conv_splitk_stats_rows(a) : conv_ws_stats_rows(a);
        }
    }
    if (p.ksplit > 1) p.split_ws_bytes = (size_t)p.ksplit * a.B * a.Cout * a.Ho * a.Wo * sizeof(float);
    if (!want_stats) p.stats_rows = 0;
    return p;
}

bool conv_planar_ok(const ConvArgs &a)
{
    if (a.upsample || (a.Hs & 1) || (a.Ws & 1)) return false;
    if (a.w_interleave) return conv_ws_planar_ok(a);
    return a.stride == 1 && !opt(OPT_CONV_NO_DIRECT) && !opt(OPT_DIRECT_NO_PLANAR) && conv_direct_eligible(a);
}

int conv2d_launch(const ConvArgs &a, hipStream_t st)
{
    IPDM_REQUIRE(a.x1 && a.w && a.out && a.B > 0 && a.Cout > 0 && a.C1 > 0, "conv2d: bad argument");
    IPDM_REQUIRE(a.C2 == 0 || a.x2, "conv2d: second source missing");
    IPDM_REQUIRE(!a.act || (a.gn_scale && a.gn_shift), "conv2d: GN prologue without scale/shift");
    const ConvPlan p = conv_plan(a, a.stats != nullptr, a.split_ws != nullptr);
    switch (p.code) {
    case 1: case 2: case 12: return conv2d_wino_launch(a, p.code, st);
    case 3: return conv2d_ws_launch(a, st);
    case 4: case 9: return conv2d_splitk_launch(a, p, st);
    case 5: return conv2d_direct_launch(a, st);
    case 6: return conv2d_nm_launch(a, st);
    case 7: return conv2d_up2_launch(a, st);
    case 10: return conv2d_pw_launch(a, st);
    case 11: return conv2d_wup2_launch(a, st, 7);
    default: return conv2d_igemm_launch(a, st);
    }
}

}
```

### ipdm-pytorch_amd/csrc/conv_pw.hip

```cpp
#include <cstdlib>
#include <type_traits>
#include "common.h"
#include "unet_kernels.h"
#include "kernel_util.h"

using namespace ipdm;

#ifndef IPDM_PW_SAFE_WAIT
#define IPDM_PW_SAFE_WAIT 0
#endif
#ifndef IPDM_PW_KO
#define IPDM_PW_KO 0
#endif

namespace {

constexpr int BN = 128;
constexpr int NW = 8;
constexpr int KC_MIN = 32;

__device__ inline f32x4 bload4(__amdgpu_buffer_rsrc_t r, int voff, int soff)
{
    return __builtin_bit_cast(f32x4, __builtin_amdgcn_raw_buffer_load_b128(r, voff, soff, 0));
}

__device__ inline i32x4 make_rsrc(const void *p, int bytes)
{
    const unsigned long long u = (unsigned long long)p;
    return i32x4{(int)(unsigned)u, (int)((unsigned)(u >> 32) & 0xffffu), bytes, 0x00020000};
}
__device__ inline void ring_load_x(float &x, int x_v, i32x4 x_rsrc, int x_s)
{
    asm volatile("buffer_load_dword %0, %1, %2, %3 offen" : "=&v"(x) : "v"(x_v), "s"(x_rsrc), "s"(x_s));
}
__device__ inline void ring_load_w(f32x4 &w, int w_v, i32x4 w_rsrc, int w_s)
{
    asm volatile("buffer_load_dwordx4 %0, %1, %2, %3 offen" : "=&v"(w) : "v"(w_v), "s"(w_rsrc), "s"(w_s));
}
template <int N>
__device__ inline void ring_wait(float (&x)[1], f32x4 &w)
{
    asm volatile("s_waitcnt vmcnt(%2)" : "+v"(x[0]), "+v"(w) : "n"(IPDM_PW_SAFE_WAIT ? 0 : N));
}
template <int N>
__device__ inline void ring_wait(float (&x)[2], f32x4 &w)
{
    asm volatile("s_waitcnt vmcnt(%3)" : "+v"(x[0]), "+v"(x[1]), "+v"(w) : "n"(IPDM_PW_SAFE_WAIT ? 0 : N));
}

struct Item { int n, p0, co0; };

template <bool ACT, bool PLANAR, int NPB>
__global__ void __launch_bounds__(512) conv_pw_kernel(ConvArgs a, int nitems)
{
    constexpr int DEPTH = 16 / NPB;
    constexpr int KC = 2 * DEPTH;
    constexpr int BP = 32 * NPB;
    constexpr int WAITN = (NPB + 1) * (DEPTH - 1);
    extern __shared__ __attribute__((aligned(16))) float lds[];
    const int tid = threadIdx.x, lane = tid & 63;
    const int swave = __builtin_amdgcn_readfirstlane(tid >> 6);
    const int lk = lane >> 5, l31 = lane & 31;
    const int G = gridDim.x, per = G >> 3;
    const int local = ((blockIdx.x & 7) * per + (blockIdx.x >> 3)) * NW + swave;
    const int WT = G * NW;
    if (local >= nitems) return;
    const int n_my = (nitems - 1 - local) / WT + 1;
    const int Ctot = a.C1 + a.C2, nch = Ctot / KC, HW = a.Ho * a.Wo;
    const int plane_bytes = HW * 4;
    auto decode = [&](int k) {
        const int item = k * WT + local;
        Item t;
        t.co0 = (item % a.co_tiles) * BN;
        const int rest = item / a.co_tiles;
        t.p0 = (rest % a.tiles_x) * BP;
        t.n = rest / a.tiles_x;
        return t;
    };

    Item nx = decode(0);
    int i_ch = 0, i_k = 0;
    int vx[NPB], vxp[PLANAR ? NPB : 1];
    auto lane_offsets = [&]() __attribute__((always_inline)) {
#pragma unroll
        for (int pb = 0; pb < NPB; ++pb) {
            const int p = nx.p0 + 32 * pb + l31;
            vx[pb] = (lk * HW + p) * 4;
            if (PLANAR) {
                const int pc = p < HW ? p : HW - 1;
                const int y = pc / a.Wo, x = pc - y * a.Wo;
                vxp[PLANAR ? pb : 0] = (lk * HW + ((y & 1) * 2 + (x & 1)) * (HW >> 2) + (y >> 1) * (a.Wo >> 1) + (x >> 1)) * 4;
            }
        }
    };
    const int wv = (lk * a.cout_pad + l31 * 4) * 4;
    const i32x4 w_rsrc = make_rsrc(a.w, Ctot * a.cout_pad * 4);
    float xs[DEPTH][NPB];
    f32x4 ws[DEPTH];

    f32x16 acc[NPB][4];
    const f32x16 zero16 = {0, 0, 0, 0, 0, 0, 0, 0, 0, 0, 0, 0, 0, 0, 0, 0};
    float *const tab = lds + swave * (ACT ? Ctot * 2 : 0);
    int tab_n = -1;
    const __amdgpu_buffer_rsrc_t b_rsrc = __builtin_amdgcn_make_buffer_rsrc((void *)(a.bias ? a.bias : a.out), 0, a.bias ? a.Cout * 4 : 0, 0x00020000);
    float bv[4] = {0.0f, 0.0f, 0.0f, 0.0f};
    const float one_k0 = lk == 0 ? 1.0f : 0.0f;
    const int vo = (l31 * HW + 4 * lk) * 4;

    auto chunk = [&](int c_ch) __attribute__((always_inline)) {
        const int c0 = i_ch * KC;
        const bool from1 = c0 < a.C1;
        const i32x4 x_rsrc = make_rsrc(from1 ? a.x1 + (size_t)nx.n * a.C1 * HW : a.x2 + (size_t)nx.n * a.C2 * HW, (from1 ? a.C1 : a.C2) * plane_bytes);
        const int x_s = (from1 ? c0 : c0 - a.C1) * plane_bytes;
        const int w_s = (c0 * a.cout_pad + nx.co0) * 4;
        const float *const tc = tab + (c_ch * KC + lk) * 2;
#pragma unroll
        for (int j = 0; j < DEPTH; ++j) {
            ring_wait<WAITN>(xs[j], ws[j]);
            float xv[NPB];
#pragma unroll
            for (int pb = 0; pb < NPB; ++pb) xv[pb] = xs[j][pb];
            if (ACT) {
                const f32x2 st = *reinterpret_cast<const f32x2 *>(tc + j * 4);
#pragma unroll
                for (int pb = 0; pb < NPB; ++pb) xv[pb] = __builtin_fmaf(xv[pb], st[0], st[1]);
            }
            const f32x4 wq = ws[j];
            __builtin_amdgcn_sched_barrier(0);
#pragma unroll
            for (int pb = 0; pb < NPB; ++pb)
#pragma unroll
                for (int b = 0; b < 4; ++b) acc[pb][b] = __builtin_amdgcn_mfma_f32_32x32x2f32(xv[pb], wq[b], acc[pb][b], 0, 0, 0);
            if (!(IPDM_PW_KO & 1)) {
#pragma unroll
                for (int pb = 0; pb < NPB; ++pb)
                    ring_load_x(xs[j][pb], (PLANAR && from1) ? vxp[PLANAR ? pb : 0] : vx[pb], x_rsrc, x_s + j * 2 * plane_bytes);
                ring_load_w(ws[j], wv, w_rsrc, w_s + j * 2 * a.cout_pad * 4);
            }
            __builtin_amdgcn_sched_barrier(0);
        }
        if (++i_ch == nch) {
            i_ch = 0;
            if (++i_k < n_my) { nx = decode(i_k); lane_offsets(); }
        }
    };

    lane_offsets();
    Item cur = nx;
    {
        const i32x4 x_rsrc = make_rsrc(a.x1 + (size_t)nx.n * a.C1 * HW, a.C1 * plane_bytes);
#pragma unroll
        for (int j = 0; j < DEPTH; ++j) {
#pragma unroll
            for (int pb = 0; pb < NPB; ++pb) ring_load_x(xs[j][pb], PLANAR ? vxp[PLANAR ? pb : 0] : vx[pb], x_rsrc, j * 2 * plane_bytes);
            ring_load_w(ws[j], wv, w_rsrc, (j * 2 * a.cout_pad + nx.co0) * 4);
        }
        i_ch = 1;
    }

    for (int k = 0; k < n_my; ++k) {
#pragma unroll
        for (int pb = 0; pb < NPB; ++pb)
#pragma unroll
            for (int b = 0; b < 4; ++b) acc[pb][b] = zero16;
#pragma unroll
        for (int b = 0; b < 4; ++b) bv[b] = bload(b_rsrc, l31 * 4, (cur.co0 + 32 * b) * 4);
        if (ACT && cur.n != tab_n) {
            for (int c = lane; c < Ctot; c += 64)
                *reinterpret_cast<f32x2 *>(tab + c * 2) = f32x2{a.gn_scale[(size_t)cur.n * Ctot + c], a.gn_shift[(size_t)cur.n * Ctot + c]};
            tab_n = cur.n;
        }
        for (int c_ch = 0; c_ch < nch; ++c_ch) chunk(c_ch);

#pragma unroll
        for (int pb = 0; pb < NPB; ++pb)
#pragma unroll
            for (int b = 0; b < 4; ++b) acc[pb][b] = __builtin_amdgcn_mfma_f32_32x32x2f32(one_k0, bv[b], acc[pb][b], 0, 0, 0);
        const size_t sample = (size_t)cur.n * a.Cout * HW;
        const __amdgpu_buffer_rsrc_t o_rsrc = __builtin_amdgcn_make_buffer_rsrc((void *)(a.out + sample), 0, a.Cout * plane_bytes, 0x00020000);
        const bool has_res = !ACT && a.res;
        const __amdgpu_buffer_rsrc_t r_rsrc = __builtin_amdgcn_make_buffer_rsrc((void *)((has_res ? a.res : a.out) + sample), 0,
                                                                                   has_res ? a.Cout * plane_bytes : 0, 0x00020000);
        auto block = [&](int pb, int b, const f32x4 (&r)[4]) __attribute__((always_inline)) {
            const int so = ((cur.co0 + 32 * b) * HW + cur.p0 + 32 * pb) * 4;
            float s1 = 0.0f, s2 = 0.0f;
#pragma unroll
            for (int q = 0; q < 4; ++q) {
                const f32x4 v = f32x4{acc[pb][b][4 * q], acc[pb][b][4 * q + 1], acc[pb][b][4 * q + 2], acc[pb][b][4 * q + 3]} + r[q];
                __builtin_amdgcn_raw_buffer_store_b128(__builtin_bit_cast(__attribute__((__vector_size__(4 * sizeof(unsigned)))) unsigned, v), o_rsrc, vo, so + q * 32, 0);
#pragma unroll
                for (int e = 0; e < 4; ++e) { s1 += v[e]; s2 = __builtin_fmaf(v[e], v[e], s2); }
            }
            if (a.stats) {
                s1 += __shfl_xor(s1, 32, 64);
                s2 += __shfl_xor(s2, 32, 64);
                if (lk == 0)
                    *reinterpret_cast<f32x2 *>(a.stats + (((size_t)cur.n * a.stats_rows + cur.p0 / 32 + pb) * a.Cout + cur.co0 + 32 * b + l31) * 2) = f32x2{s1, s2};
            }
        };
        auto ragged_block = [&](int pb, int b, int nv) __attribute__((always_inline)) {
            const int so = ((cur.co0 + 32 * b) * HW + cur.p0 + 32 * pb) * 4;
            float s1 = 0.0f, s2 = 0.0f;
#pragma unroll
            for (int i = 0; i < 16; ++i) {
                const int px = 8 * (i >> 2) + 4 * lk + (i & 3);
                const int off = px < nv ? vo + (i >> 2) * 32 + (i & 3) * 4 : OOB;
                const float v = ACT ? acc[pb][b][i] : acc[pb][b][i] + bload(r_rsrc, off, so);
                __builtin_amdgcn_raw_buffer_store_b32(__builtin_bit_cast(unsigned, v), o_rsrc, off, so, 0);
                const float vm = px < nv ? v : 0.0f;
                s1 += vm; s2 = __builtin_fmaf(vm, vm, s2);
            }
            if (a.stats) {
                s1 += __shfl_xor(s1, 32, 64);
                s2 += __shfl_xor(s2, 32, 64);
                if (lk == 0)
                    *reinterpret_cast<f32x2 *>(a.stats + (((size_t)cur.n * a.stats_rows + cur.p0 / 32 + pb) * a.Cout + cur.co0 + 32 * b + l31) * 2) = f32x2{s1, s2};
            }
        };
        if (HW - cur.p0 >= BP) {
            if (has_res) {
                f32x4 r[2][4];
                auto fetch = [&](int t) __attribute__((always_inline)) {
#pragma unroll
                    for (int q = 0; q < 4; ++q)
                        r[t & 1][q] = bload4(r_rsrc, vo, ((cur.co0 + 32 * (t & 3)) * HW + cur.p0 + 32 * (t >> 2)) * 4 + q * 32);
                };
                fetch(0);
#pragma unroll
                for (int t = 0; t < 4 * NPB; ++t) {
                    if (t + 1 < 4 * NPB) fetch(t + 1);
                    block(t >> 2, t & 3, r[t & 1]);
                }
            } else {
                const f32x4 z4 = {0.0f, 0.0f, 0.0f, 0.0f};
                const f32x4 r0[4] = {z4, z4, z4, z4};
#pragma unroll
                for (int t = 0; t < 4 * NPB; ++t) block(t >> 2, t & 3, r0);
            }
        } else {
            for (int pb = 0; pb < NPB; ++pb) {
                const int nv = HW - cur.p0 - 32 * pb;
                if (nv <= 0) break;
                if (nv >= 32) {
#pragma unroll
                    for (int b = 0; b < 4; ++b) {
                        f32x4 r[4] = {};
                        if (!ACT) {
#pragma unroll
                            for (int q = 0; q < 4; ++q) r[q] = bload4(r_rsrc, vo, ((cur.co0 + 32 * b) * HW + cur.p0 + 32 * pb) * 4 + q * 32);
                        }
                        if (pb == 0) block(0, b, r); else block(NPB - 1, b, r);
                    }
                } else {
#pragma unroll
                    for (int b = 0; b < 4; ++b) { if (pb == 0) ragged_block(0, b, nv); else ragged_block(NPB - 1, b, nv); }
                }
            }
        }
        cur = nx;
    }
}

}

namespace ipdm {

static bool conv_pw_layer_ok(const ConvArgs &a)
{
    if (opt(OPT_CONV_NO_PW)) return false;
    const int Ctot = a.C1 + a.C2;
    if (a.ksize != 1 || a.stride != 1 || a.w_interleave != 4 || a.Cout % BN || a.cout_pad != a.Cout) return false;
    if (a.upsample || a.H != a.Hs || a.W != a.Ws || a.Ho != a.H || a.Wo != a.W) return false;
    if (Ctot % KC_MIN || Ctot < 2 * KC_MIN || (a.C2 && a.C1 % KC_MIN) || a.act == 2 || a.sk_w || (a.act && a.res)) return false;
    return (long)(a.C1 > a.C2 ? a.C1 : a.C2) * a.Ho * a.Wo < (1L << 29) && (long)a.Cout * a.Ho * a.Wo < (1L << 29);
}

bool conv_pw_eligible(const ConvArgs &a, bool stats)
{
    if (!conv_pw_layer_ok(a)) return false;
    if (opt(OPT_PW_FORCE)) return true;
    const long items = (long)cdiv((long)a.Ho * a.Wo, 32) * (a.Cout / BN);
    return stats ? items >= 1024 : 10 * items * a.B >= 13L * device_cu_count() * NW;
}

int conv_pw_stats_rows(const ConvArgs &a) { return cdiv((long)a.Ho * a.Wo, 32); }

namespace {
template <int NPB>
const void *pw_kernel(bool act, bool planar)
{
    return act ? (planar ? (const void *)conv_pw_kernel<true, true, NPB> : (const void *)conv_pw_kernel<true, false, NPB>)
               : (planar ? (const void *)conv_pw_kernel<false, true, NPB> : (const void *)conv_pw_kernel<false, false, NPB>);
}
}

int conv2d_pw_launch(const ConvArgs &args, hipStream_t st)
{
    ConvArgs a = args;
    IPDM_REQUIRE(conv_pw_eligible(a, a.stats != nullptr), "conv2d_pw: not a layer of this kernel");
    IPDM_REQUIRE(!a.x1_planar || (!(a.Ho & 1) && !(a.Wo & 1)), "conv2d_pw: parity-planar source of odd size %dx%d", a.Ho, a.Wo);
    const int HW = a.Ho * a.Wo, Ctot = a.C1 + a.C2;
    IPDM_REQUIRE(!a.stats || a.stats_rows == conv_pw_stats_rows(a), "conv2d_pw: statistics rows %d != %d", a.stats_rows, conv_pw_stats_rows(a));
    const int cus = device_cu_count();
    a.co_tiles = a.Cout / BN;
    const long waves = (long)cus * NW;
    const long r32 = cdiv((long)cdiv(HW, 32) * a.co_tiles * a.B, waves), r64 = cdiv((long)cdiv(HW, 64) * a.co_tiles * a.B, waves);
    const int forced = opt(OPT_PW_ITEM);
    const int npb = forced ? forced : (1.86 * r64 <= (double)r32 ? 2 : 1);
    a.tiles_x = cdiv(HW, 32 * npb);
    a.tiles_y = 1;
    const long nitems = (long)a.tiles_x * a.co_tiles * a.B;
    IPDM_REQUIRE(nitems < (1L << 31), "conv2d_pw: too many items");
    long G = cdiv(nitems, NW) < cus ? cdiv(nitems, NW) : cus;
    G = (G + 7) / 8 * 8;
    const size_t lds_bytes = a.act ? (size_t)NW * Ctot * 2 * sizeof(float) : 0;
    IPDM_REQUIRE(lds_bytes <= 64 * 1024, "conv2d_pw: %d input channels exceed the scale/shift tables", Ctot);
    const bool prof = prof_enabled();
    if (prof) prof_before(1, st);
    int ni = (int)nitems;
    void *params[] = {&a, &ni};
    (void)hipLaunchKernel(npb == 2 ? pw_kernel<2>(a.act, a.x1_planar) : pw_kernel<1>(a.act, a.x1_planar), dim3((unsigned)G), dim3(512), params, lds_bytes, st);
    if (prof) prof_after(1, 2.0 * a.B * HW * (double)a.Cout * Ctot, st);
    IPDM_LAUNCH_CHECK();
    return IPDM_OK;
}

}
```

### ipdm-pytorch_amd/csrc/ops.hip

```cpp
#include <vector>
#include "conv_layer.h"

using namespace ipdm;

namespace {

struct GnTables { float *gamma = nullptr, *beta = nullptr, *scale = nullptr, *shift = nullptr; double *partials = nullptr; };

int gn_tables(DevScratch &s, const float *gamma_host, const float *beta_host, int B, int C, int groups, GnTables &t)
{
    int rc = s.get(gamma_host, C * sizeof(float), &t.gamma);
    if (!rc) rc = s.get(beta_host, C * sizeof(float), &t.beta);
    if (!rc) rc = s.get(nullptr, ((size_t)B * C + 64) * sizeof(float), &t.scale);
    if (!rc) rc = s.get(nullptr, ((size_t)B * C + 64) * sizeof(float), &t.shift);
    if (!rc) rc = s.get(nullptr, gn_partials_bytes(B, groups), &t.partials);
    return rc;
}

int gn_fill(const GnTables &t, const float *stats, int rows, const float *x1, int C1, const float *x2, int C2, int B, long HW, int groups,
            hipStream_t st)
{
    if (rows > 0) {
        GnTileArgs g;
        g.nsrc = 1; g.src[0].stats = stats; g.src[0].rows = rows; g.src[0].C = C1; g.B = B; g.HW = HW; g.groups = groups;
        g.gamma = t.gamma; g.beta = t.beta; g.eps = 1e-5f; g.partials = t.partials; g.scale = t.scale; g.shift = t.shift;
        return gn_tiles_launch(g, st);
    }
    GnArgs g;
    g.x1 = x1; g.x2 = x2; g.C1 = C1; g.C2 = C2; g.B = B; g.HW = HW; g.groups = groups;
    g.gamma = t.gamma; g.beta = t.beta; g.eps = 1e-5f; g.partials = t.partials; g.scale = t.scale; g.shift = t.shift;
    return gn_stats_launch(g, st);
}

int put_conv(DevScratch &s, const PackedConv &L, const float *bias_host, ConvArgs &a)
{
    const int rc = s.put_layer(L, a);
    return (rc || !bias_host) ? rc : s.get(bias_host, a.Cout * sizeof(float), &a.bias);
}

int put_plan_buffers(DevScratch &s, const ConvPlan &p, ConvArgs &a, hipStream_t st)
{
    if (p.split_ws_bytes)
        if (const int rc = s.get(nullptr, p.split_ws_bytes, &a.split_ws)) return rc;
    if (p.stats_rows > 0) {
        const size_t bytes = (size_t)a.B * p.stats_rows * a.Cout * 2 * sizeof(float);
        if (const int rc = s.get(nullptr, bytes, &a.stats)) return rc;
        IPDM_HIP_CHECK(hipMemsetAsync(a.stats, 0xff, bytes, st));
        a.stats_rows = p.stats_rows;
    }
    return IPDM_OK;
}

int finish(hipStream_t st)
{
    IPDM_HIP_CHECK(hipStreamSynchronize(st));
    return IPDM_OK;
}

struct Events {
    hipEvent_t e0 = nullptr, e1 = nullptr;
    ~Events() { if (e0) (void)hipEventDestroy(e0); if (e1) (void)hipEventDestroy(e1); }
};

template <class F> int time_launches(int warm, int iters, float *avg_ms, F launch)
{
    for (int i = 0; i < warm; ++i)
        if (const int rc = launch()) return rc;
    Events ev;
    IPDM_HIP_CHECK(hipEventCreate(&ev.e0));
    IPDM_HIP_CHECK(hipEventCreate(&ev.e1));
    IPDM_HIP_CHECK(hipEventRecord(ev.e0, nullptr));
    int rc = IPDM_OK;
    for (int i = 0; i < iters && !rc; ++i) rc = launch();
    IPDM_HIP_CHECK(hipEventRecord(ev.e1, nullptr));
    IPDM_HIP_CHECK(hipEventSynchronize(ev.e1));
    float ms = 0;
    IPDM_HIP_CHECK(hipEventElapsedTime(&ms, ev.e0, ev.e1));
    *avg_ms = ms / iters;
    return rc;
}

}

extern "C" int ipdm_op_conv2d(const float *d_x1, int32_t C1, const float *d_x2, int32_t C2, int32_t B, int32_t Hs, int32_t Ws,
                              int32_t H, int32_t W, const float *w_host, const float *b_host, int32_t Cout, int32_t ksize,
                              int32_t stride, int32_t act, int32_t groups, const float *gamma_host, const float *beta_host,
                              const float *d_res, float *d_out, void *stream)
{
    IPDM_REQUIRE(d_x1 && w_host && d_out, "op_conv2d: null argument");
    IPDM_REQUIRE(!act || (gamma_host && beta_host && groups > 0), "op_conv2d: GN prologue needs gamma/beta/groups");
    hipStream_t st = (hipStream_t)stream;
    const int Cin = C1 + C2;
    PackedConv L;
    conv_pack_layer(w_host, Cout, Cin, ksize, stride, H != Hs || W != Ws, L);
    L.up2.clear(); L.wup2.clear();
    ConvArgs a = conv_args(B, C1, C2, Hs, Ws, H, W, Cout, ksize, stride, L.interleave, L.cout_pad);
    a.x1 = d_x1; a.x2 = d_x2; a.act = act; a.res = d_res; a.out = d_out;
    DevScratch s(st);
    if (const int rc = put_conv(s, L, b_host, a)) return rc;
    if (act) {
        GnTables t;
        if (const int rc = gn_tables(s, gamma_host, beta_host, B, Cin, groups, t)) return rc;
        if (const int rc = gn_fill(t, nullptr, 0, d_x1, C1, d_x2, C2, B, (long)Hs * Ws, groups, st)) return rc;
        a.gn_scale = t.scale; a.gn_shift = t.shift;
    }
    if (const int rc = put_plan_buffers(s, conv_plan(a, false, true), a, st)) return rc;
    if (const int rc = conv2d_launch(a, st)) return rc;
    return finish(st);
}

extern "C" int ipdm_op_up_conv_chain(const float *d_x, int32_t C, int32_t B, int32_t Hs, int32_t Ws, const float *wA_host,
                                     const float *bA_host, int32_t CA, const float *d_skip, int32_t C2, int32_t groups,
                                     const float *gamma_host, const float *beta_host, int32_t act, const float *wB_host,
                                     const float *bB_host, int32_t CB, int32_t ksB, float *d_mid, float *d_out,
                                     int32_t *used_up2, void *stream)
{
    IPDM_REQUIRE(d_x && wA_host && wB_host && gamma_host && beta_host && d_mid && d_out && groups > 0 && (C2 == 0 || d_skip),
                 "op_up_conv_chain: null argument");
    hipStream_t st = (hipStream_t)stream;
    const int H = 2 * Hs, W = 2 * Ws, Cc = CA + C2;
    const size_t mid_bytes = (size_t)B * CA * H * W * sizeof(float);
    PackedConv LA, LB;
    conv_pack_layer(wA_host, CA, C, 3, 1, true, LA);
    conv_pack_layer(wB_host, CB, Cc, ksB, 1, false, LB);
    DevScratch s(st);
    GnTables t;
    float *d_pl = nullptr;
    ConvArgs a = conv_args(B, C, 0, Hs, Ws, H, W, CA, 3, 1, LA.interleave, LA.cout_pad);
    ConvArgs b = conv_args(B, CA, C2, H, W, H, W, CB, ksB, 1, LB.interleave, LB.cout_pad);
    if (const int rc = put_conv(s, LA, bA_host, a)) return rc;
    if (const int rc = put_conv(s, LB, bB_host, b)) return rc;
    if (const int rc = gn_tables(s, gamma_host, beta_host, B, Cc, groups, t)) return rc;
    if (const int rc = s.get(nullptr, mid_bytes, &d_pl)) return rc;
    a.x1 = d_x; a.out = d_pl;
    const ConvPlan planA = conv_plan(a, C2 == 0, false);
    const bool up2 = planA.out_planar;
    if (used_up2) *used_up2 = !planA.up2 ? 0 : !up2 ? 2 : planA.code == 11 ? 3 : 1;
    if (const int rc = put_plan_buffers(s, planA, a, st)) return rc;
    if (const int rc = conv2d_launch(a, st)) return rc;
    if (up2) { if (const int rc = planar_to_linear_launch(d_pl, d_mid, (long)B * CA, H, W, st)) return rc; }
    else IPDM_HIP_CHECK(hipMemcpyAsync(d_mid, d_pl, mid_bytes, hipMemcpyDeviceToDevice, st));
    if (const int rc = gn_fill(t, a.stats, planA.stats_rows, d_pl, CA, d_skip, C2, B, (long)H * W, groups, st)) return rc;
    b.x1 = d_pl; b.x2 = d_skip; b.act = act; b.gn_scale = t.scale; b.gn_shift = t.shift; b.out = d_out;
    if (up2 && !conv_planar_ok(b)) {
        float *d_lin = nullptr;
        if (const int rc = s.get(nullptr, mid_bytes, &d_lin)) return rc;
        if (const int rc = planar_to_linear_launch(d_pl, d_lin, (long)B * CA, H, W, st)) return rc;
        b.x1 = d_lin;
    } else b.x1_planar = up2 ? 1 : 0;
    if (const int rc = put_plan_buffers(s, conv_plan(b, false, true), b, st)) return rc;
    if (const int rc = conv2d_launch(b, st)) return rc;
    return finish(st);
}

extern "C" int ipdm_op_conv_gn_conv(const float *d_x, int32_t C, int32_t B, int32_t H, int32_t W, const float *wA_host,
                                    const float *bA_host, int32_t CA, int32_t ksA, int32_t strideA, const float *d_resA,
                                    int32_t groups, const float *gamma_host, const float *beta_host, int32_t act,
                                    const float *wB_host, const float *bB_host, int32_t CB, float *d_mid, float *d_out,
                                    int32_t *fused_rows, void *stream)
{
    IPDM_REQUIRE(d_x && wA_host && wB_host && gamma_host && beta_host && d_mid && d_out && groups > 0, "op_conv_gn_conv: null argument");
    hipStream_t st = (hipStream_t)stream;
    PackedConv LA, LB;
    conv_pack_layer(wA_host, CA, C, ksA, strideA, false, LA);
    conv_pack_layer(wB_host, CB, CA, 3, 1, false, LB);
    DevScratch s(st);
    GnTables t;
    ConvArgs a = conv_args(B, C, 0, H, W, H, W, CA, ksA, strideA, LA.interleave, LA.cout_pad);
    const int Hm = a.Ho, Wm = a.Wo;
    ConvArgs b = conv_args(B, CA, 0, Hm, Wm, Hm, Wm, CB, 3, 1, LB.interleave, LB.cout_pad);
    if (const int rc = put_conv(s, LA, bA_host, a)) return rc;
    if (const int rc = put_conv(s, LB, bB_host, b)) return rc;
    if (const int rc = gn_tables(s, gamma_host, beta_host, B, CA, groups, t)) return rc;
    a.x1 = d_x; a.res = d_resA; a.out = d_mid;
    const ConvPlan planA = conv_plan(a, true, true);
    if (fused_rows) *fused_rows = planA.stats_rows;
    if (const int rc = put_plan_buffers(s, planA, a, st)) return rc;
    if (const int rc = conv2d_launch(a, st)) return rc;
    if (const int rc = gn_fill(t, a.stats, planA.stats_rows, d_mid, CA, nullptr, 0, B, (long)Hm * Wm, groups, st)) return rc;
    b.x1 = d_mid; b.act = act; b.gn_scale = t.scale; b.gn_shift = t.shift; b.out = d_out;
    if (const int rc = conv2d_launch(b, st)) return rc;
    return finish(st);
}

extern "C" int ipdm_bench_conv2d(int32_t B, int32_t C1, int32_t C2, int32_t H, int32_t W, int32_t Cout, int32_t ksize,
                                 int32_t stride, int32_t act, int32_t with_res, int32_t iters, float *avg_ms)
{
    IPDM_REQUIRE(avg_ms && iters > 0, "bench_conv2d: bad argument");
    const bool x1_planar = (act & 256) != 0;
    const bool up = (act & 512) != 0;
    act &= 255;
    IPDM_REQUIRE(!up || (ksize == 3 && stride == 1 && !C2 && !with_res && !act && !x1_planar), "bench_conv2d: bad Upsample configuration");
    const int Cin = C1 + C2;
    std::vector<float> w((size_t)Cout * Cin * ksize * ksize);
    for (size_t i = 0; i < w.size(); ++i) w[i] = (float)((i * 2654435761u) % 2001) / 1000.0f - 1.0f;
    PackedConv L;
    conv_pack_layer(w.data(), Cout, Cin, ksize, stride, up, L);
    if (!L.interleave) L.up2.clear();
    ConvArgs a = conv_args(B, C1, C2, H, W, up ? 2 * H : H, up ? 2 * W : W, Cout, ksize, stride, L.interleave, L.cout_pad);
    a.act = act;
    if (x1_planar) { IPDM_REQUIRE(conv_planar_ok(a), "bench_conv2d: this shape has no parity-planar reader"); a.x1_planar = 1; }
    DevScratch s(nullptr);
    if (const int rc = s.put_layer(L, a)) return rc;
    auto randn = [&](int rows, int64_t n, size_t pad, int seed, const float **out) {
        const int rc = s.get(nullptr, ((size_t)rows * n + pad) * sizeof(float), out);
        return rc ? rc : ipdm_randn(const_cast<float *>(*out), rows, n, seed, 0, 0, nullptr);
    };
    const int64_t n_out = (int64_t)Cout * a.Ho * a.Wo;
    if (const int rc = randn(B, (int64_t)C1 * H * W, 0, 1, &a.x1)) return rc;
    if (C2) if (const int rc = randn(B, (int64_t)C2 * H * W, 0, 2, &a.x2)) return rc;
    if (with_res) if (const int rc = randn(B, n_out, 0, 3, &a.res)) return rc;
    if (const int rc = randn(1, (int64_t)B * Cin, 64, 4, &a.gn_scale)) return rc;
    if (const int rc = randn(1, (int64_t)B * Cin, 64, 5, &a.gn_shift)) return rc;
    if (const int rc = randn(1, Cout, 0, 6, &a.bias)) return rc;
    if (const int rc = s.get(nullptr, (size_t)B * n_out * sizeof(float), &a.out)) return rc;
    if (const int rc = put_plan_buffers(s, conv_plan(a, up, true), a, nullptr)) return rc;
    const bool stamps = (opt(OPT_CONV_DBG) & 24) != 0;
    if (stamps)
        if (const int rc = s.get(nullptr, 4096 * 8 * 8, &a.dbg_buf)) return rc;
    if (const int rc = time_launches(3, iters, avg_ms, [&] { return conv2d_launch(a, nullptr); })) return rc;
    if (stamps) {
        std::vector<unsigned long long> h(4096 * 8);
        IPDM_HIP_CHECK(hipMemcpy(h.data(), a.dbg_buf, h.size() * 8, hipMemcpyDeviceToHost));
        double s4[8] = {0, 0, 0, 0, 0, 0, 0, 0}; int nz = 0;
        for (int g = 0; g < 4096; ++g) if (h[g * 8 + 3]) { for (int k = 0; k < 8; ++k) s4[k] += (double)h[g * 8 + k]; ++nz; }
        if (nz) fprintf(stderr, "  stamps over %d workgroups (s_memtime ticks, avg): consumer mfma %.0f epilogue %.0f barrier %.0f total %.0f | "
                        "producer issue %.0f wait %.0f math %.0f store %.0f\n", nz, s4[0] / nz, s4[1] / nz, s4[2] / nz, s4[3] / nz,
                        s4[4] / nz, s4[5] / nz, s4[6] / nz, s4[7] / nz);
    }
    return IPDM_OK;
}

extern "C" int ipdm_bench_attention(int32_t B, int32_t heads, int32_t d, int32_t T, int32_t iters, float *avg_ms)
{
    IPDM_REQUIRE(avg_ms && iters > 0, "bench_attention: bad argument");
    DevScratch s(nullptr);
    float *d_qkv = nullptr, *d_out = nullptr, *d_scr = nullptr, *d_pl = nullptr;
    if (const int rc = s.get(nullptr, (size_t)B * heads * 3 * d * T * sizeof(float), &d_qkv)) return rc;
    if (const int rc = s.get(nullptr, (size_t)B * heads * d * T * sizeof(float), &d_out)) return rc;
    ipdm_randn(d_qkv, B, (int64_t)heads * 3 * d * T, 9, 0, 0, nullptr);
    if (const size_t n = attention_scratch_floats(B, heads, d, T))
        if (const int rc = s.get(nullptr, n * sizeof(float), &d_scr)) return rc;
    if (const size_t n = attention_planes_floats(B, heads, d, T))
        if (const int rc = s.get(nullptr, n * sizeof(float), &d_pl)) return rc;
    return time_launches(2, iters, avg_ms, [&] { return attention_launch(d_qkv, d_out, B, heads, d, T, nullptr, d_scr, d_pl); });
}

extern "C" int32_t ipdm_conv_layout_code(int32_t Cout, int32_t ksize, int32_t stride)
{
    return conv_weight_interleave(Cout, ksize, stride);
}

static int32_t conv_kernel_code_impl(int32_t B, int32_t Cout, int32_t Cin, int32_t ksize, int32_t stride, int32_t H, int32_t W, bool with_stats)
{
    if (B <= 0 || Cout <= 0 || Cin <= 0 || H <= 0 || W <= 0 || (ksize != 1 && ksize != 3) || stride < 1 || stride > 2) return -1;
    static float dummy;
    const int il = conv_weight_interleave(Cout, ksize, stride);
    ConvArgs a = conv_args(B, Cin, 0, H, W, H, W, Cout, ksize, stride, il, conv_cout_pad(Cout, il));
    a.x1 = a.w = a.out = &dummy;
    a.w_wino = conv_wino_shape_ok(Cout, Cin, ksize, stride, il) ? &dummy : nullptr;
    return conv_plan(a, with_stats, true).code;
}

extern "C" int32_t ipdm_conv_kernel_code(int32_t B, int32_t Cout, int32_t Cin, int32_t ksize, int32_t stride, int32_t H, int32_t W)
{
    return conv_kernel_code_impl(B, Cout, Cin, ksize, stride, H, W, false);
}
extern "C" int32_t ipdm_conv_kernel_code_stats(int32_t B, int32_t Cout, int32_t Cin, int32_t ksize, int32_t stride, int32_t H, int32_t W)
{
    return conv_kernel_code_impl(B, Cout, Cin, ksize, stride, H, W, true);
}
```

### ipdm-pytorch_amd/csrc/unet.hip

```cpp
#include <algorithm>
#include <cmath>
#include <cstdlib>
#include <map>
#include <string>
#include <tuple>
#include <vector>
#include "conv_layer.h"

using namespace ipdm;

namespace {

__global__ void __launch_bounds__(256) temb_kernel(const float *__restrict__ freqs, int mc, float t,
                                                   const float *__restrict__ w0, const float *__restrict__ b0,
                                                   const float *__restrict__ w2, const float *__restrict__ b2,
                                                   float *__restrict__ tmp, float *__restrict__ silu_emb)
{
    extern __shared__ float sm[];
    float *e0 = sm;
    float *h1 = sm + mc;
    const int half = mc / 2, ted = 4 * mc;
    for (int i = threadIdx.x; i < mc; i += 256) {
        float v = 0.0f;
        if (i < half) v = cosf(t * freqs[i]);
// ... 502 lines not shown
    }
    TRY(upload(net, wm.get("time_embed.0.weight"), (size_t)ted * mc, &net->te_w0));
    TRY(upload(net, wm.get("time_embed.0.bias"), ted, &net->te_b0));
    TRY(upload(net, wm.get("time_embed.2.weight"), (size_t)ted * ted, &net->te_w2));
    TRY(upload(net, wm.get("time_embed.2.bias"), ted, &net->te_b2));

    std::vector<float> tW, tb, c1b;
    auto do_layer = [&](const Layer &l) -> int {
        const std::string &p = l.prefix;
        int r = 0;
        switch (l.kind) {
            case L_CONV: r = make_conv(net, wm, p + ".weight", p + ".bias", l.cout, l.cin, 3, net->convs[p]); break;
            case L_DOWN: r = make_conv(net, wm, p + ".op.weight", p + ".op.bias", l.cout, l.cin, 3, net->convs[p], 2); break;
            case L_UP: r = make_conv(net, wm, p + ".conv.weight", p + ".conv.bias", l.cout, l.cin, 3, net->convs[p], 1, true); break;
            case L_RES: {
                ResP &rp = net->res[p];
                if ((r = make_norm(net, wm, p + ".conv1.0", l.cin, rp.n1))) break;
                if ((r = make_conv(net, wm, p + ".conv1.2.weight", "", l.cout, l.cin, 3, rp.c1))) break;
                if ((r = make_norm(net, wm, p + ".conv2.0", l.cout, rp.n2))) break;
                if ((r = make_conv(net, wm, p + ".conv2.2.weight", p + ".conv2.2.bias", l.cout, l.cout, 3, rp.c2))) break;
                rp.has_sc = l.cin != l.cout;
                if (rp.has_sc && (r = make_conv(net, wm, p + ".shortcut.weight", p + ".shortcut.bias", l.cout, l.cin, 1, rp.sc))) break;
                if (rp.has_sc) {
                    const float *b2 = wm.get(p + ".conv2.2.bias"), *bs = wm.get(p + ".shortcut.bias");
                    std::vector<float> both(l.cout);
                    for (int c = 0; c < l.cout; ++c) both[c] = b2[c] + bs[c];
                    if ((r = upload(net, both.data(), both.size(), &rp.b2sc))) break;
                }
                const float *tw = wm.get(p + ".time_emb.1.weight"), *tbb = wm.get(p + ".time_emb.1.bias"),
                            *cb = wm.get(p + ".conv1.2.bias");
                if (!tw || !tbb || !cb) { set_error("unet_create: missing time_emb/conv1 bias of %s", p.c_str()); r = IPDM_ERR_INVALID; break; }
                rp.bias_off = (int)tb.size();
                tW.insert(tW.end(), tw, tw + (size_t)l.cout * ted);
                tb.insert(tb.end(), tbb, tbb + l.cout);
                c1b.insert(c1b.end(), cb, cb + l.cout);
                break;
            }
            case L_ATTN: {
                AttnP &ap = net->attn[p];
                if ((r = make_norm(net, wm, p + ".norm", l.cin, ap.n))) break;
                if ((r = make_conv(net, wm, p + ".qkv.weight", "", 3 * l.cin, l.cin, 1, ap.qkv))) break;
                r = make_conv(net, wm, p + ".proj.weight", p + ".proj.bias", l.cin, l.cin, 1, ap.proj);
                const int hd = l.cin / cfg->num_heads;
                if (!r && opt(OPT_ATTN_ANY_DIM) == 0 && hd != 64 && hd != 32) { set_error("unet_create: attention head dim %d unsupported (64 or 32)", hd); r = IPDM_ERR_UNSUPPORTED; }
                if (!r && opt(OPT_ATTN_ANY_DIM) != 0 && (hd < 1 || hd > ATTN_GEN_DMAX)) { set_error("unet_create: attention head dim %d unsupported (1 .. %d under attn_any_dim)", hd, ATTN_GEN_DMAX); r = IPDM_ERR_UNSUPPORTED; }
                break;
            }
        }
        return r;
    };
    for (auto &blk : net->topo.down) for (auto &l : blk) TRY(do_layer(l));
    for (auto &l : net->topo.middle) TRY(do_layer(l));
    for (auto &blk : net->topo.up) for (auto &l : blk) TRY(do_layer(l));
    TRY(make_norm(net, wm, "out.0", net->topo.out_ch_in, net->out_norm));
    TRY(make_conv(net, wm, "out.2.weight", "out.2.bias", cfg->out_channels, net->topo.out_ch_in, 3, net->out_conv));
    net->temb_rows = (int)tb.size();
    TRY(upload(net, tW.data(), tW.size(), &net->temb_W));
    TRY(upload(net, tb.data(), tb.size(), &net->temb_b));
    TRY(upload(net, c1b.data(), c1b.size(), &net->conv1_b));
#undef TRY
    for (auto &blk : net->topo.up) for (auto &l : blk) if (l.cin > net->max_ch) net->max_ch = l.cin;
    *out = net;
    return IPDM_OK;
}

extern "C" int ipdm_unet_destroy(ipdm_unet *net)
{
    if (!net) return IPDM_OK;
    for (auto &kv : net->graphs) (void)hipGraphExecDestroy(kv.second);
    for (float *p : net->owned) (void)hipFree(p);
    delete net;
    return IPDM_OK;
}

int ipdm::unet_io_channels(const ipdm_unet *net, int *cin, int *cout)
{
    if (!net || !cin || !cout) return IPDM_ERR_INVALID;
    *cin = net->cfg.in_channels;
    *cout = net->cfg.out_channels;
    return IPDM_OK;
}

namespace {

struct Fwd {
    ipdm_unet *net;
    int rc = 0;

    const float *ptr(const Tensor *t) const { return t->external ? t->ext : (const float *)(net->ws + t->off); }
    float *wptr(Tensor *t) const { return (float *)(net->ws + t->off); }

    Tensor *make(int C, int H, int W)
    {
        Tensor *t = new Tensor();
        t->C = C; t->H = H; t->W = W;
        t->bytes = (size_t)net->B * C * H * W * sizeof(float);
        t->off = net->arena.alloc(t->bytes);
        if (t->off == (size_t)-1) { set_error("unet_forward: workspace exhausted"); rc = IPDM_ERR_WORKSPACE; t->off = 0; }
        t->refs = 1;
        net->live.push_back(t);
        return t;
    }
    void retain(Tensor *t) { t->refs++; }
    void release(Tensor *t)
    {
        if (--t->refs == 0) {
            if (!t->external) net->arena.release(t->off, t->bytes);
            if (t->st_off != (size_t)-1) net->arena.release(t->st_off, t->st_bytes);
            for (size_t i = 0; i < net->live.size(); ++i)
                if (net->live[i] == t) { net->live.erase(net->live.begin() + i); break; }
            delete t;
        }
    }

    Tensor *linear_copy(const Tensor *t)
    {
        if (!t || !t->planar) return nullptr;
        Tensor *o = make(t->C, t->H, t->W);
        if (!rc && !net->dry) rc = planar_to_linear_launch(ptr(t), wptr(o), (long)net->B * t->C, t->H, t->W, net->st);
        return o;
    }

    void gn(const Tensor *x1, const Tensor *x2, const NormP &np)
    {
        if (rc || net->dry) return;
        StatRef refs[2];
        int nref = 0;
        bool have = !net->no_fused_stats;
        for (const Tensor *t : {x1, x2}) {
            if (!t) continue;
            if (t->nst == 0 || nref + t->nst > 2) { have = false; break; }
            for (int k = 0; k < t->nst; ++k) refs[nref++] = t->st[k];
        }
        if (have) {
            GnTileArgs g;
            g.nsrc = nref;
            for (int k = 0; k < nref; ++k) { g.src[k].stats = (const float *)(net->ws + refs[k].off); g.src[k].rows = refs[k].rows; g.src[k].C = refs[k].C; }
            g.B = net->B; g.HW = (long)x1->H * x1->W; g.groups = np.groups; g.gamma = np.g; g.beta = np.b; g.eps = 1e-5f;
            g.partials = net->gn_part; g.scale = net->gn_scale; g.shift = net->gn_shift;
            rc = gn_tiles_launch(g, net->st);
            return;
        }
        GnArgs a;
        a.x1 = ptr(x1); a.x2 = x2 ? ptr(x2) : nullptr;
        a.C1 = x1->C; a.C2 = x2 ? x2->C : 0; a.B = net->B;
        a.HW = (long)x1->H * x1->W;
        a.groups = np.groups; a.gamma = np.g; a.beta = np.b; a.eps = 1e-5f;
        a.partials = net->gn_part; a.scale = net->gn_scale; a.shift = net->gn_shift;
        rc = gn_stats_launch(a, net->st);
    }

    Tensor *conv(const Tensor *x1, const Tensor *x2, const ConvP &cp, int stride, int act, const float *bias,
                 const Tensor *res, int H, int W, float *ext_out = nullptr, bool want_stats = false,
                 const Tensor *sk_x1 = nullptr, const Tensor *sk_x2 = nullptr, const ConvP *sk = nullptr)
    {
        ConvArgs a = conv_args(net->B, x1->C, x2 ? x2->C : 0, x1->H, x1->W, H, W, cp.cout, cp.ks, stride, cp.interleave, cp.cout_pad);
        const int Ho = a.Ho, Wo = a.Wo;
        Tensor *o;
        if (ext_out) { o = new Tensor(); o->C = cp.cout; o->H = Ho; o->W = Wo; o->external = true; o->ext = ext_out; o->refs = 1; net->live.push_back(o); }
        else o = make(cp.cout, Ho, Wo);
        Tensor *lin1 = nullptr, *lin2 = linear_copy(x2), *linr = linear_copy(res);
        if (lin2) x2 = lin2;
        if (linr) res = linr;
        conv_set_images(a, cp.img[net->transposed ? 1 : 0]);
        if (ext_out && cp.interleave) a.w_up2 = nullptr;
        a.bias = bias; a.act = act; a.gn_scale = net->gn_scale; a.gn_shift = net->gn_shift;
        a.res = res ? (const float *)(uintptr_t)256 : nullptr;
        if (x1->planar && !conv_planar_ok(a)) x1 = lin1 = linear_copy(x1);
        a.x1_planar = x1->planar ? 1 : 0;
        Tensor *lins = sk ? linear_copy(sk_x2) : nullptr;
        if (lins) sk_x2 = lins;
        struct LinGuard { Fwd &f; Tensor *a, *b, *c, *d; ~LinGuard() { if (a) f.release(a); if (b) f.release(b); if (c) f.release(c); if (d) f.release(d); } }
            lin_guard{*this, lin1, lin2, linr, lins};
        if (sk) {
            a.sk_C1 = sk_x1->C; a.sk_C2 = sk_x2 ? sk_x2->C : 0; a.sk_cout_pad = sk->cout_pad; a.sk_planar = sk_x1->planar ? 1 : 0;
            a.sk_w = sk->img[0].plain;
        }
        const ConvPlan plan = conv_plan(a, want_stats && !ext_out && !net->no_fused_stats, true);
        o->planar = plan.out_planar;
        size_t split_off = (size_t)-1;
        if (plan.split_ws_bytes) {
            split_off = net->arena.alloc(plan.split_ws_bytes);
            if (split_off == (size_t)-1) { set_error("unet_forward: workspace exhausted"); rc = IPDM_ERR_WORKSPACE; split_off = 0; }
        }
        struct SplitGuard { Arena &ar; size_t off, bytes; ~SplitGuard() { if (off != (size_t)-1) ar.release(off, bytes); } } split_guard{net->arena, split_off, plan.split_ws_bytes};
        if (plan.stats_rows > 0) {
            o->st_bytes = (size_t)net->B * plan.stats_rows * cp.cout * 2 * sizeof(float);
            o->st_off = net->arena.alloc(o->st_bytes);
            if (o->st_off == (size_t)-1) { set_error("unet_forward: workspace exhausted"); rc = IPDM_ERR_WORKSPACE; o->st_off = 0; }
            o->nst = 1;
            o->st[0].off = o->st_off; o->st[0].rows = plan.stats_rows; o->st[0].C = cp.cout;
        }
        if (rc || net->dry) return o;
        a.x1 = ptr(x1); a.x2 = x2 ? ptr(x2) : nullptr; a.res = res ? ptr(res) : nullptr; a.out = ext_out ? ext_out : wptr(o);
        if (sk) { a.sk_x1 = ptr(sk_x1); a.sk_x2 = sk_x2 ? ptr(sk_x2) : nullptr; }
        if (plan.split_ws_bytes) a.split_ws = (float *)(net->ws + split_off);
        if (o->nst) { a.stats = (float *)(net->ws + o->st_off); a.stats_rows = plan.stats_rows; }
        rc = conv2d_launch(a, net->st);
#if IPDM_UNET_TRACE
        if (!rc) trace_conv(a, (size_t)net->B * cp.cout * Ho * Wo, net->st);
#endif
        return o;
    }

    Tensor *res_block(const Tensor *x1, const Tensor *x2, const Layer &l)
    {
        const ResP &rp = net->res[l.prefix];
        const int H = x1->H, W = x1->W;
        gn(x1, x2, rp.n1);
        Tensor *h1 = conv(x1, x2, rp.c1, 1, 2, net->bias_eff + rp.bias_off, nullptr, H, W, nullptr, true);
        Tensor *sc = nullptr;
        const Tensor *resid;
        bool fuse = false;
        if (rp.has_sc && rp.b2sc && rp.sc.interleave == 0 && (!x2 || !x2->planar)) {
            ConvArgs q = conv_args(net->B, rp.c2.cin, 0, H, W, H, W, rp.c2.cout, 3, 1, rp.c2.interleave, rp.c2.cout_pad);
            q.act = 2;
            q.sk_C1 = x1->C; q.sk_C2 = x2 ? x2->C : 0; q.sk_cout_pad = rp.sc.cout_pad;
            fuse = conv_direct_skip_ok(q);
        }
        if (fuse) resid = nullptr;
        else if (rp.has_sc) { sc = conv(x1, x2, rp.sc, 1, 0, rp.sc.b, nullptr, H, W); resid = sc; }
        else if (x2) {
            sc = make(x1->C + x2->C, H, W);
            Tensor *l1 = linear_copy(x1), *l2 = linear_copy(x2);
            struct G { Fwd &f; Tensor *a, *b; ~G() { if (a) f.release(a); if (b) f.release(b); } } g_{*this, l1, l2};
            if (l1) x1 = l1;
            if (l2) x2 = l2;
            if (!rc && !net->dry) {
                const long total = (long)net->B * (x1->C + x2->C) * H * W;
                int g = cdiv(total, 1024); if (g > 4096) g = 4096;
                hipLaunchKernelGGL(concat_kernel, dim3(g), dim3(256), 0, net->st, ptr(x1), ptr(x2), wptr(sc), x1->C, x2->C, (long)H * W, total);
            }
            resid = sc;
        } else resid = x1;
        gn(h1, nullptr, rp.n2);
        Tensor *o = fuse ? conv(h1, nullptr, rp.c2, 1, 2, rp.b2sc, nullptr, H, W, nullptr, true, x1, x2, &rp.sc)
                         : conv(h1, nullptr, rp.c2, 1, 2, rp.c2.b, resid, H, W, nullptr, true);
        release(h1);
        if (sc) release(sc);
        return o;
    }

    Tensor *attn_block(const Tensor *x, const Layer &l)
    {
        const AttnP &ap = net->attn[l.prefix];
        const int H = x->H, W = x->W;
        gn(x, nullptr, ap.n);
        Tensor *qkv = conv(x, nullptr, ap.qkv, 1, 1, nullptr, nullptr, H, W);
        Tensor *a = make(x->C, H, W);
        const int heads = net->cfg.num_heads, hd = x->C / heads;
        const size_t sfl = attention_scratch_floats(net->B, heads, hd, H * W);
        Tensor *scr = sfl ? make((int)((sfl + (size_t)net->B * H * W - 1) / ((size_t)net->B * H * W)), H, W) : nullptr;
        const size_t pfl = attention_planes_floats(net->B, heads, hd, H * W);
        Tensor *pl = pfl ? make((int)((pfl + (size_t)net->B * H * W - 1) / ((size_t)net->B * H * W)), H, W) : nullptr;
        if (!rc && !net->dry)
            rc = attention_launch(ptr(qkv), wptr(a), net->B, heads, hd, H * W, net->st, scr ? wptr(scr) : nullptr, pl ? wptr(pl) : nullptr);
        if (pl) release(pl);
        if (scr) release(scr);
        release(qkv);
        Tensor *o = conv(a, nullptr, ap.proj, 1, 0, ap.proj.b, x, H, W, nullptr, true);
        release(a);
        return o;
    }

    Tensor *run_block(const std::vector<Layer> &layers, Tensor *x1, Tensor *x2, int size_h, int size_w)
    {
        Tensor *h = nullptr;
        Tensor *cat = nullptr;
        int align = conv_k_chunk();
        if (x2 && !layers.empty() && layers[0].kind == L_RES) {
            const ResP &rp0 = net->res[layers[0].prefix];
            if (rp0.has_sc) align = std::max(align, conv_ws_k_chunk(1, rp0.sc.interleave));
            align = std::max(align, conv_ws_k_chunk(3, rp0.c1.interleave));
        }
        if (x2 && (x1->C % align) != 0) {
            cat = make(x1->C + x2->C, x1->H, x1->W);
            Tensor *l1 = linear_copy(x1), *l2 = linear_copy(x2);
            if (!rc && !net->dry) {
                const long total = (long)net->B * cat->C * x1->H * x1->W;
                int g = cdiv(total, 1024); if (g > 4096) g = 4096;
                hipLaunchKernelGGL(concat_kernel, dim3(g), dim3(256), 0, net->st, ptr(l1 ? l1 : x1), ptr(l2 ? l2 : x2), wptr(cat), x1->C, x2->C, (long)x1->H * x1->W, total);
            }
            if (l1) release(l1);
            if (l2) release(l2);
            if (x1->nst == 1 && x2->nst == 1) { cat->nst = 2; cat->st[0] = x1->st[0]; cat->st[1] = x2->st[0]; }
            x1 = cat;
            x2 = nullptr;
        }
        for (size_t i = 0; i < layers.size(); ++i) {
            const Layer &l = layers[i];
            const Tensor *in1 = h ? h : x1;
            const Tensor *in2 = h ? nullptr : x2;
            Tensor *o = nullptr;
            switch (l.kind) {
                case L_CONV: { const ConvP &cp = net->convs[l.prefix]; o = conv(in1, in2, cp, 1, 0, cp.b, nullptr, in1->H, in1->W, nullptr, true); break; }
                case L_DOWN: { const ConvP &cp = net->convs[l.prefix]; o = conv(in1, in2, cp, 2, 0, cp.b, nullptr, in1->H, in1->W, nullptr, true); break; }
                case L_UP: { const ConvP &cp = net->convs[l.prefix]; o = conv(in1, in2, cp, 1, 0, cp.b, nullptr, size_h, size_w, nullptr, true); break; }
                case L_RES: o = res_block(in1, in2, l); break;
                case L_ATTN: o = attn_block(in1, l); break;
            }
            if (h) release(h);
            h = o;
        }
        if (cat) release(cat);
        return h;
    }
};

size_t fixed_ws_bytes(const ipdm_unet *net, int B)
{
    size_t s = 0;
    s += align_up((size_t)net->topo.ted * 2 * sizeof(float), 256);
    s += align_up((size_t)(net->temb_rows ? net->temb_rows : 1) * sizeof(float), 256);
    s += 2 * align_up(((size_t)B * net->max_ch + 64) * sizeof(float), 256);
    s += align_up(gn_partials_bytes(B, net->max_gn_groups), 256);
    return s;
}

bool choose_transposed(const ipdm_unet *net, int H, int W)
{
    if (const int force = opt(OPT_UNET_TRANSPOSE); force >= 0) return force != 0;
    if (H == W) return false;
    double cost[2] = {0.0, 0.0};
    int h = H, w = W;
    const int nlev = net->cfg.n_mult - 1;
    for (int level = 0; level < nlev; ++level) {
        const double ch = (double)(int)(net->cfg.channel_mult[level + 1] * net->cfg.model_channels);
        if (ch > 32) {
            const double wgt = ch * ch;
            cost[0] += wgt * (double)(cdiv(w, 32) * 32) * (double)(cdiv(h, 8) * 8);
            cost[1] += wgt * (double)(cdiv(h, 32) * 32) * (double)(cdiv(w, 8) * 8);
        }
        if (level != nlev - 1) { h = (h - 1) / 2 + 1; w = (w - 1) / 2 + 1; }
    }
    return cost[1] < 0.98 * cost[0];
}

int run_forward(ipdm_unet *net, const float *d_x, int t, float *d_eps, int B, int H, int W, void *d_ws, size_t ws_bytes,
                hipStream_t st, bool dry, size_t *need)
{
    if (const int ch = opt_changed_since(net->opts); ch >= 0) {
        set_error("unet_forward: option '%s' changed after ipdm_unet_create (was %d): create the network again", opt_name(ch), net->opts[ch]);
        return IPDM_ERR_INVALID;
    }
    net->B = B; net->st = st; net->dry = dry; net->ws = (char *)d_ws;
    net->no_fused_stats = opt(OPT_GN_UNFUSED) != 0;
    const size_t fixed = fixed_ws_bytes(net, B);
    if (!dry && ws_bytes < fixed) { set_error("unet_forward: workspace too small"); return IPDM_ERR_WORKSPACE; }
    char *w = (char *)d_ws;
    float *emb_tmp = (float *)w; float *silu_emb = emb_tmp + net->topo.ted;
    w += align_up((size_t)net->topo.ted * 2 * sizeof(float), 256);
    net->bias_eff = (float *)w; w += align_up((size_t)(net->temb_rows ? net->temb_rows : 1) * sizeof(float), 256);
    net->gn_scale = (float *)w; w += align_up(((size_t)B * net->max_ch + 64) * sizeof(float), 256);
    net->gn_shift = (float *)w; w += align_up(((size_t)B * net->max_ch + 64) * sizeof(float), 256);
    net->gn_part = (double *)w;
    if (!dry) {
        (void)hipMemsetAsync(net->gn_scale, 0, ((size_t)B * net->max_ch + 64) * sizeof(float), st);
        (void)hipMemsetAsync(net->gn_shift, 0, ((size_t)B * net->max_ch + 64) * sizeof(float), st);
    }
    net->ws = (char *)d_ws + fixed;
    net->arena.reset(dry ? (size_t)1 << 46 : ws_bytes - fixed);
    for (Tensor *tt : net->live) delete tt;
    net->live.clear();

    net->transposed = choose_transposed(net, H, W);
    Fwd f{net};
    if (!dry) {
        f.rc = temb_launch(net->d_freqs, net->cfg.model_channels, t, net->te_w0, net->te_b0, net->te_w2, net->te_b2, emb_tmp, silu_emb, st);
        if (!f.rc && net->temb_rows)
            f.rc = gemv_bias_launch(net->temb_W, net->temb_b, net->conv1_b, silu_emb, net->bias_eff, net->temb_rows, net->topo.ted, st);
    }
    Tensor *x;
    if (net->transposed) {
        x = f.make(net->cfg.in_channels, W, H);
        if (!f.rc && !dry)
            hipLaunchKernelGGL(transpose_hw_kernel, dim3(cdiv(W, 32), cdiv(H, 32), B * net->cfg.in_channels), dim3(256), 0, st, d_x,
                               f.wptr(x), H, W);
        std::swap(H, W);
    } else {
        x = new Tensor();
        x->C = net->cfg.in_channels; x->H = H; x->W = W; x->external = true; x->ext = d_x; x->refs = 1;
        net->live.push_back(x);
    }

    std::vector<Tensor *> hs;
    Tensor *h = x;
    for (auto &blk : net->topo.down) {
        Tensor *o = f.run_block(blk, h, nullptr, 0, 0);
        f.release(h);
        h = o;
        f.retain(h);
        hs.push_back(h);
    }
    {
        Tensor *o = f.run_block(net->topo.middle, h, nullptr, 0, 0);
        f.release(h);
        h = o;
    }
    Tensor *h_ = hs.back(); hs.pop_back();
    for (auto &blk : net->topo.up) {
        Tensor *skip = h_;
        bool popped = false;
        if (!hs.empty()) { h_ = hs.back(); hs.pop_back(); popped = true; }
        Tensor *o = f.run_block(blk, h, skip, h_->H, h_->W);
        f.release(h);
        if (popped) f.release(skip);
        h = o;
    }
    f.release(h_);
// ... 158 lines not shown
```

### ipdm-pytorch_amd/csrc/unet_kernels.h

```cpp
#pragma once
#include <vector>
#include "common.h"

namespace ipdm {

struct GnTileSrc { const float *stats = nullptr; int rows = 0, C = 0; };
struct GnTileArgs {
    GnTileSrc src[2];
    int nsrc = 1, B = 0;
    long HW = 0;
    int groups = 0;
    const float *gamma = nullptr, *beta = nullptr;
    float eps = 1e-5f;
    double *partials = nullptr;
    float *scale = nullptr, *shift = nullptr;
};

struct ConvArgs {
    const float *x1 = nullptr, *x2 = nullptr;
    int C1 = 0, C2 = 0, B = 0;
    int Hs = 0, Ws = 0;
    int H = 0, W = 0;
    int upsample = 0;
    float scale_y = 1.f, scale_x = 1.f;
    const float *w = nullptr;
    int cout_pad = 0;
    int w_interleave = 0;
    const float *bias = nullptr;
    int Cout = 0, ksize = 0, stride = 0;
    int Ho = 0, Wo = 0;
    int act = 0;
    const float *gn_scale = nullptr, *gn_shift = nullptr;
    const float *res = nullptr;
    float *out = nullptr;
    int tiles_x = 0, tiles_y = 0, co_tiles = 0;
    float *stats = nullptr;
    int stats_rows = 0;
    float *split_ws = nullptr;
    int ksplit = 1;
    const float *w_up2 = nullptr;
    const float *w_wup2 = nullptr;
    const float *w_wino = nullptr;
    const float *sk_x1 = nullptr, *sk_x2 = nullptr, *sk_w = nullptr;
    int sk_C1 = 0, sk_C2 = 0, sk_cout_pad = 0, sk_planar = 0;
    int x1_planar = 0;
    int up2 = 0;
    int dbg = 0;
    unsigned long long *dbg_buf = nullptr;
};

struct ConvPlan {
    int code = 0;
    int ksplit = 1;
    size_t split_ws_bytes = 0;
    int stats_rows = 0;
    bool up2 = false;
    bool out_planar = false;
};
ConvPlan conv_plan(const ConvArgs &a, bool want_stats, bool may_split);
bool conv_planar_ok(const ConvArgs &a);
int conv2d_launch(const ConvArgs &a, hipStream_t st);

int conv2d_igemm_launch(const ConvArgs &a, hipStream_t st);
bool conv_direct_eligible(const ConvArgs &a);
bool conv_direct_up2_eligible(const ConvArgs &a);
bool conv_direct_skip_ok(const ConvArgs &a);
int conv2d_direct_launch(const ConvArgs &a, hipStream_t st);
bool conv_nm_eligible(const ConvArgs &a);
int conv2d_nm_launch(const ConvArgs &a, hipStream_t st);
int conv2d_ws_launch(const ConvArgs &a, hipStream_t st);
int conv_ws_split(const ConvArgs &a);
bool conv_ws_planar_ok(const ConvArgs &a);
int conv2d_splitk_launch(const ConvArgs &a, const ConvPlan &p, hipStream_t st);
bool conv_up2_eligible(const ConvArgs &a);
int conv2d_up2_launch(const ConvArgs &a, hipStream_t st);
bool conv_wup2_shape_ok(int Cout, int Cin);
bool conv_wup2_eligible(const ConvArgs &a);
int conv2d_wup2_launch(const ConvArgs &orig, hipStream_t st, int prof_cls);
bool conv_wino_shape_ok(int Cout, int Cin, int ks, int stride, int interleave);
bool conv_wino_eligible(const ConvArgs &a);
int conv2d_wino_launch(const ConvArgs &a, int code, hipStream_t st);
int conv_wino_split(const ConvArgs &a);
bool conv_wino2_eligible(const ConvArgs &a);
bool conv_wino3_eligible(const ConvArgs &a);
int conv2d_wino2_launch(const ConvArgs &prepared, hipStream_t st);
int conv2d_wino3_launch(const ConvArgs &prepared, hipStream_t st);
bool conv_pw_eligible(const ConvArgs &a, bool stats);
int conv2d_pw_launch(const ConvArgs &a, hipStream_t st);
int conv_igemm_stats_rows(const ConvArgs &a);
int conv_direct_stats_rows(const ConvArgs &a);
int conv_ws_stats_rows(const ConvArgs &a);
int conv_up2_stats_rows(const ConvArgs &a);
int conv_splitk_stats_rows(const ConvArgs &a);
int conv_pw_stats_rows(const ConvArgs &a);
int conv_k_chunk();
int conv_ws_k_chunk(int ks, int interleave);

constexpr int PROF_CLASSES = 8;
bool prof_enabled();
void prof_before(int cls, hipStream_t st);
void prof_after(int cls, double flops, hipStream_t st);
int conv_weight_interleave(int Cout, int ks, int stride);
void conv_pack_weights(const float *w, int Cout, int Cin, int ks, int interleave, std::vector<float> &packed, int &cin_pad, int &cout_pad);

struct GnArgs {
    const float *x1, *x2;
    int C1, C2, B;
    long HW;
    int groups;
    const float *gamma, *beta;
    float eps;
    double *partials;
    float *scale, *shift;
    int split = 0;
};
constexpr int GN_SPLIT = 64;
int gn_tiles_launch(const GnTileArgs &a, hipStream_t st);
void conv_pack_weights_wup2(const float *w, int Cout, int Cin, std::vector<float> &packed);
void conv_pack_weights_wino(const float *w, int Cout, int Cin, std::vector<float> &packed);
void conv_pack_weights_up2(const float *w, int Cout, int Cin, int interleave, std::vector<float> &packed);
int planar_to_linear_launch(const float *src, float *dst, long planes, int H, int W, hipStream_t st);
size_t gn_partials_bytes(int B, int groups);
int gn_stats_launch(const GnArgs &a, hipStream_t st);

int attention_launch(const float *qkv, float *out, int B, int heads, int d, int T, hipStream_t st, float *scratch = nullptr,
                     float *planes = nullptr);
size_t attention_scratch_floats(int B, int heads, int d, int T);
size_t attention_planes_floats(int B, int heads, int d, int T);
void attention_bx3_launch(const float *qkv, float *out, int B, int heads, int T, float scale, int Z, bool seq, float *scratch, float *planes,
                          hipStream_t st);
constexpr int ATTN_GEN_DMAX = 128;
int attention_gen_split(int heads, int d, int T);
int attention_gen_launch(const float *qkv, float *out, int B, int heads, int d, int T, float scale, int Z, float *scratch, hipStream_t st);

int temb_launch(const float *freqs, int mc, int t, const float *w0, const float *b0, const float *w2, const float *b2,
                float *tmp, float *silu_emb, hipStream_t st);
int gemv_bias_launch(const float *W, const float *b, const float *base, const float *v, float *y, int rows, int K,
                     hipStream_t st);

}
```

Baseline: 2.180.

## Fuse K/V bf16 presplit plane writing into the pointwise QKV convolution epilogue

The pointwise qkv projection kernel gains a PLANES variant that, besides writing fp32 qkv, splits K and V into three bf16 pieces and stores them straight into the attention tile planes. The attention launch then skips its separate presplit kernel when the planes are already filled. This removes one kernel launch and the re-read of K/V from global memory per attention block. The cost is a heavier conv epilogue with more LDS use and register pressure, and the path applies only when head dim is 64 and the conv plan picks the pointwise kernel.

```diff
diff --git a/include/ipdm_hip.h b/include/ipdm_hip.h
--- a/include/ipdm_hip.h
+++ b/include/ipdm_hip.h
@@ -249,6 +249,10 @@
                           int32_t *used_up2, void *stream);
 int ipdm_op_attention(const float *d_qkv, float *d_out, int32_t B, int32_t heads, int32_t d, int32_t T,
                       void *stream);
+int ipdm_op_qkv_planes(const float *d_x, int32_t C, int32_t B, int32_t H, int32_t W, const float *w_host, int32_t heads,
+                       int32_t act, int32_t groups, const float *gamma_host, const float *beta_host, int32_t x_planar,
+                       int32_t fused, float *d_qkv, void *d_planes, void *stream);
+int32_t ipdm_qkv_planes_fused(int32_t B, int32_t C, int32_t heads, int32_t H, int32_t W);
 
 typedef struct ipdm_art_geom {
     float dso, dsd;
@@ -330,6 +334,7 @@
 int ipdm_bench_conv2d(int32_t B, int32_t C1, int32_t C2, int32_t H, int32_t W, int32_t Cout, int32_t ksize,
                       int32_t stride, int32_t act, int32_t with_res, int32_t iters, float *avg_ms);
 int ipdm_bench_attention(int32_t B, int32_t heads, int32_t d, int32_t T, int32_t iters, float *avg_ms);
+int ipdm_bench_qkv_attention(int32_t B, int32_t C, int32_t heads, int32_t H, int32_t W, int32_t iters, float *avg_ms);
 int32_t ipdm_conv_layout_code(int32_t Cout, int32_t ksize, int32_t stride);
 int32_t ipdm_conv_kernel_code(int32_t B, int32_t Cout, int32_t Cin, int32_t ksize, int32_t stride, int32_t H, int32_t W);
 int32_t ipdm_conv_kernel_code_stats(int32_t B, int32_t Cout, int32_t Cin, int32_t ksize, int32_t stride, int32_t H, int32_t W);
diff --git a/ipdm-pytorch_amd/_lib.py b/ipdm-pytorch_amd/_lib.py
--- a/ipdm-pytorch_amd/_lib.py
+++ b/ipdm-pytorch_amd/_lib.py
@@ -153,7 +153,10 @@
     "ipdm_profile_end": (C.c_int, [C.POINTER(_f64 * PROF_CLASSES), C.POINTER(_f64 * PROF_CLASSES), C.POINTER(_i64 * PROF_CLASSES), _i32]),
     "ipdm_bench_conv2d": (C.c_int, [_i32] * 11 + [C.POINTER(_f32)]),
     "ipdm_bench_attention": (C.c_int, [_i32] * 5 + [C.POINTER(_f32)]),
+    "ipdm_bench_qkv_attention": (C.c_int, [_i32] * 6 + [C.POINTER(_f32)]),
     "ipdm_op_attention": (C.c_int, [_vp, _vp, _i32, _i32, _i32, _i32, _vp]),
+    "ipdm_op_qkv_planes": (C.c_int, [_vp, _i32, _i32, _i32, _i32, _vp, _i32, _i32, _i32, _vp, _vp, _i32, _i32, _vp, _vp, _vp]),
+    "ipdm_qkv_planes_fused": (_i32, [_i32] * 5),
     "ipdm_conv_layout_code": (_i32, [_i32, _i32, _i32]),
     "ipdm_conv_kernel_code": (_i32, [_i32, _i32, _i32, _i32, _i32, _i32, _i32]),
     "ipdm_conv_kernel_code_stats": (_i32, [_i32, _i32, _i32, _i32, _i32, _i32, _i32]),
diff --git a/ipdm-pytorch_amd/csrc/attn.hip b/ipdm-pytorch_amd/csrc/attn.hip
--- a/ipdm-pytorch_amd/csrc/attn.hip
+++ b/ipdm-pytorch_amd/csrc/attn.hip
@@ -475,7 +475,8 @@
     return Z > 1 ? (size_t)Z * B * heads * (d + 2) * T : 0;
 }
 
-int attention_launch(const float *qkv, float *out, int B, int heads, int d, int T, hipStream_t st, float *scratch, float *planes)
+int attention_launch(const float *qkv, float *out, int B, int heads, int d, int T, hipStream_t st, float *scratch, float *planes,
+                     bool planes_filled)
 {
     IPDM_REQUIRE(qkv && out && B > 0 && heads > 0 && T > 0, "attention: bad argument");
     if (int rc = attention_head_dim_check(d)) return rc;
@@ -485,13 +486,15 @@
     const AttnPlan p = attention_plan(B, heads, d, T, scratch != nullptr);
     const int Z = p.Z;
     const bool seq = p.form == 2, q2 = p.qt == 2;
+    IPDM_REQUIRE(!planes_filled || (p.family == 2 && planes && attention_planes_floats(B, heads, d, T)),
+                 "attention: K/V planes written by the qkv projection, but this launch does not read planes");
     if (p.family == 3) {
         if (int rc = attention_gen_launch(qkv, out, B, heads, d, T, scale, Z, scratch, st)) return rc;
         if (p.form == 1)
             hipLaunchKernelGGL(attention_combine_any_kernel, dim3(cdiv(T, 256), B * heads, cdiv(d, 16)), dim3(256), 0, st, scratch, out, T, Z, cdiv(T, KV), d);
     } else if (p.family == 2) {
         if (!attention_planes_floats(B, heads, d, T)) planes = nullptr;
-        attention_bx3_launch(qkv, out, B, heads, T, scale, Z, seq, scratch, planes, st);
+        attention_bx3_launch(qkv, out, B, heads, T, scale, Z, seq, scratch, planes, st, planes_filled);
         if (p.form == 1)
             hipLaunchKernelGGL((attention_combine_kernel<64>), dim3(cdiv(T, 256), B * heads, 4), dim3(256), 0, st, scratch, out, T, Z, cdiv(T, KV));
     } else if (p.family == 1) {
diff --git a/ipdm-pytorch_amd/csrc/attn_bx3.hip b/ipdm-pytorch_amd/csrc/attn_bx3.hip
--- a/ipdm-pytorch_amd/csrc/attn_bx3.hip
+++ b/ipdm-pytorch_amd/csrc/attn_bx3.hip
@@ -8,34 +8,15 @@
 
 typedef unsigned u32x4 __attribute__((ext_vector_type(4)));
 typedef __bf16 bf16x8 __attribute__((ext_vector_type(8)));
-typedef __bf16 bf16x2 __attribute__((ext_vector_type(2)));
 
 namespace {
 
 constexpr int D = 64;
-constexpr int KT = 32;
+constexpr int KT = PLANE_KT;
 constexpr int KP = 72;
 constexpr int VP = 40;
 constexpr int KPLANE = KT * KP, VPLANE = D * VP;
 constexpr int STAGE = 3 * KPLANE + 3 * VPLANE;
-constexpr int PCHUNK = 256;
-constexpr int TILE_CHUNKS = 6 * PCHUNK;
-
-__device__ inline unsigned pk_bf16(float a, float b)
-{
-    return __builtin_bit_cast(unsigned, bf16x2{(__bf16)a, (__bf16)b});
-}
-struct Split3 { unsigned h[3]; };
-__device__ inline Split3 split3(float a, float b)
-{
-    Split3 s;
-    s.h[0] = pk_bf16(a, b);
-    const float ra = a - __builtin_bit_cast(float, s.h[0] << 16), rb = b - __builtin_bit_cast(float, s.h[0] & 0xffff0000u);
-    s.h[1] = pk_bf16(ra, rb);
-    const float qa = ra - __builtin_bit_cast(float, s.h[1] << 16), qb = rb - __builtin_bit_cast(float, s.h[1] & 0xffff0000u);
-    s.h[2] = pk_bf16(qa, qb);
-    return s;
-}
 
 __device__ inline f32x16 mma(u32x4 a, u32x4 b, f32x16 c)
 {
@@ -517,12 +498,17 @@
     return (size_t)B * heads * cdiv(T, KT) * TILE_CHUNKS * 4;
 }
 
+void attention_presplit_launch(const float *qkv, float *planes, int B, int heads, int T, hipStream_t st)
+{
+    hipLaunchKernelGGL(attention_presplit_kernel, dim3(cdiv(T, KT), B * heads), dim3(256), 0, st, qkv, reinterpret_cast<u32x4 *>(planes), heads, T);
+}
+
 void attention_bx3_launch(const float *qkv, float *out, int B, int heads, int T, float scale, int Z, bool seq, float *scratch,
-                          float *planes, hipStream_t st)
+                          float *planes, hipStream_t st, bool planes_filled)
 {
     const dim3 grid(cdiv(T, 128), B * heads, seq ? 1 : Z);
     u32x4 *pl = reinterpret_cast<u32x4 *>(planes);
-    if (pl) hipLaunchKernelGGL(attention_presplit_kernel, dim3(cdiv(T, KT), B * heads), dim3(256), 0, st, qkv, pl, heads, T);
+    if (pl && !planes_filled) attention_presplit_launch(qkv, planes, B, heads, T, st);
     const bool pipe = pl && !seq && !opt(OPT_ATTN_NO_PIPELINE);
     const auto launch = [&](auto kernel, int zsplit, float *part, int zseq) {
         hipLaunchKernelGGL(kernel, grid, dim3(384), 0, st, qkv, out, heads, T, scale, zsplit, part, zseq, pl);
diff --git a/ipdm-pytorch_amd/csrc/attn_common.h b/ipdm-pytorch_amd/csrc/attn_common.h
--- a/ipdm-pytorch_amd/csrc/attn_common.h
+++ b/ipdm-pytorch_amd/csrc/attn_common.h
@@ -32,5 +32,26 @@
 }
 __device__ inline float slice_fold(float acc, float v, SliceWeights w) { return fmaf(acc, w.a, v * w.b); }
 
+typedef __bf16 bf16x2 __attribute__((ext_vector_type(2)));
+__device__ inline unsigned pk_bf16(float a, float b)
+{
+    return __builtin_bit_cast(unsigned, bf16x2{(__bf16)a, (__bf16)b});
+}
+struct Split3 { unsigned h[3]; };
+__device__ inline Split3 split3(float a, float b)
+{
+    Split3 s;
+    s.h[0] = pk_bf16(a, b);
+    const float ra = a - __builtin_bit_cast(float, s.h[0] << 16), rb = b - __builtin_bit_cast(float, s.h[0] & 0xffff0000u);
+    s.h[1] = pk_bf16(ra, rb);
+    const float qa = ra - __builtin_bit_cast(float, s.h[1] << 16), qb = rb - __builtin_bit_cast(float, s.h[1] & 0xffff0000u);
+    s.h[2] = pk_bf16(qa, qb);
+    return s;
+}
+
+constexpr int PLANE_KT = 32;
+constexpr int PCHUNK = 256;
+constexpr int TILE_CHUNKS = 6 * PCHUNK;
+
 }
 }
diff --git a/ipdm-pytorch_amd/csrc/common.h b/ipdm-pytorch_amd/csrc/common.h
--- a/ipdm-pytorch_amd/csrc/common.h
+++ b/ipdm-pytorch_amd/csrc/common.h
@@ -53,6 +53,7 @@
     OPT_ATTN_ANY_DIM,
     OPT_ATTN_TRAIN_ANY_DIM,
     OPT_CONV_TUNED_ALL,
+    OPT_ATTN_NO_FUSED_SPLIT,
     OPT_COUNT
 };
 int opt(Opt o);
diff --git a/ipdm-pytorch_amd/csrc/common.hip b/ipdm-pytorch_amd/csrc/common.hip
--- a/ipdm-pytorch_amd/csrc/common.hip
+++ b/ipdm-pytorch_amd/csrc/common.hip
@@ -46,6 +46,7 @@
     {"attn_any_dim", 0, true, 0, 2},
     {"attn_train_any_dim", 0, true},
     {"conv_tuned_all", 0, true},
+    {"attn_no_fused_split", 0, true},
 };
 bool opt_value_ok(int i, int v)
 {
diff --git a/ipdm-pytorch_amd/csrc/conv_plan.hip b/ipdm-pytorch_amd/csrc/conv_plan.hip
--- a/ipdm-pytorch_amd/csrc/conv_plan.hip
+++ b/ipdm-pytorch_amd/csrc/conv_plan.hip
@@ -40,6 +40,13 @@
     return p;
 }
 
+bool conv_qkv_planes_fused(const ConvArgs &a, int heads)
+{
+    if (opt(OPT_ATTN_NO_FUSED_SPLIT) || heads <= 0 || a.Cout != heads * 192) return false;
+    if (!attention_planes_floats(a.B, heads, 64, a.Ho * a.Wo)) return false;
+    return conv_plan(a, false, true).code == 10 && conv_pw_planes_ok(a, heads);
+}
+
 bool conv_planar_ok(const ConvArgs &a)
 {
     if (a.upsample || (a.Hs & 1) || (a.Ws & 1)) return false;
@@ -53,6 +60,7 @@
     IPDM_REQUIRE(a.C2 == 0 || a.x2, "conv2d: second source missing");
     IPDM_REQUIRE(!a.act || (a.gn_scale && a.gn_shift), "conv2d: GN prologue without scale/shift");
     const ConvPlan p = conv_plan(a, a.stats != nullptr, a.split_ws != nullptr);
+    IPDM_REQUIRE(!a.kv_planes || p.code == 10, "conv2d: K/V planes asked of kernel code %d (the pointwise kernel alone writes them)", p.code);
     switch (p.code) {
     case 1: case 2: case 12: return conv2d_wino_launch(a, p.code, st);
     case 3: return conv2d_ws_launch(a, st);
diff --git a/ipdm-pytorch_amd/csrc/conv_pw.hip b/ipdm-pytorch_amd/csrc/conv_pw.hip
--- a/ipdm-pytorch_amd/csrc/conv_pw.hip
+++ b/ipdm-pytorch_amd/csrc/conv_pw.hip
@@ -3,6 +3,7 @@
 #include "common.h"
 #include "unet_kernels.h"
 #include "kernel_util.h"
+#include "attn_common.h"
 
 using namespace ipdm;
 
@@ -18,6 +19,10 @@
 constexpr int BN = 128;
 constexpr int NW = 8;
 constexpr int KC_MIN = 32;
+constexpr int KTP = 36;
+constexpr int KTILE = 32 * KTP;
+
+typedef unsigned u32x4 __attribute__((ext_vector_type(4)));
 
 __device__ inline f32x4 bload4(__amdgpu_buffer_rsrc_t r, int voff, int soff)
 {
@@ -48,9 +53,17 @@
     asm volatile("s_waitcnt vmcnt(%3)" : "+v"(x[0]), "+v"(x[1]), "+v"(w) : "n"(IPDM_PW_SAFE_WAIT ? 0 : N));
 }
 
+template <int N>
+__device__ inline void store_words(const unsigned (&h)[N], __amdgpu_buffer_rsrc_t r, int voff, int soff)
+{
+    typedef unsigned u32x2 __attribute__((ext_vector_type(2)));
+    if constexpr (N == 4) __builtin_amdgcn_raw_buffer_store_b128(u32x4{h[0], h[1], h[2], h[3]}, r, voff, soff, 0);
+    else __builtin_amdgcn_raw_buffer_store_b64(u32x2{h[0], h[1]}, r, voff, soff, 0);
+}
+
 struct Item { int n, p0, co0; };
 
-template <bool ACT, bool PLANAR, int NPB>
+template <bool ACT, bool PLANAR, int NPB, bool PLANES = false>
 __global__ void __launch_bounds__(512) conv_pw_kernel(ConvArgs a, int nitems)
 {
     constexpr int DEPTH = 16 / NPB;
@@ -166,7 +179,9 @@
 #pragma unroll
         for (int b = 0; b < 4; ++b) bv[b] = bload(b_rsrc, l31 * 4, (cur.co0 + 32 * b) * 4);
         if (ACT && cur.n != tab_n) {
-            for (int c = lane; c < Ctot; c += 64)
+            int fl = lane;
+            if constexpr (PLANES) asm volatile("" : "+v"(fl));
+            for (int c = fl; c < Ctot; c += 64)
                 *reinterpret_cast<f32x2 *>(tab + c * 2) = f32x2{a.gn_scale[(size_t)cur.n * Ctot + c], a.gn_shift[(size_t)cur.n * Ctot + c]};
             tab_n = cur.n;
         }
@@ -178,24 +193,29 @@
             for (int b = 0; b < 4; ++b) acc[pb][b] = __builtin_amdgcn_mfma_f32_32x32x2f32(one_k0, bv[b], acc[pb][b], 0, 0, 0);
         const size_t sample = (size_t)cur.n * a.Cout * HW;
         const __amdgpu_buffer_rsrc_t o_rsrc = __builtin_amdgcn_make_buffer_rsrc((void *)(a.out + sample), 0, a.Cout * plane_bytes, 0x00020000);
-        const bool has_res = !ACT && a.res;
+        const bool has_res = !ACT && !PLANES && a.res;
         const __amdgpu_buffer_rsrc_t r_rsrc = __builtin_amdgcn_make_buffer_rsrc((void *)((has_res ? a.res : a.out) + sample), 0,
                                                                                    has_res ? a.Cout * plane_bytes : 0, 0x00020000);
+        int ln = lane;
+        if constexpr (PLANES) asm volatile("" : "+v"(ln));
+        const int e31 = PLANES ? ln & 31 : l31, ek = PLANES ? ln >> 5 : lk, evo = PLANES ? (e31 * HW + 4 * ek) * 4 : vo;
         auto block = [&](int pb, int b, const f32x4 (&r)[4]) __attribute__((always_inline)) {
             const int so = ((cur.co0 + 32 * b) * HW + cur.p0 + 32 * pb) * 4;
             float s1 = 0.0f, s2 = 0.0f;
 #pragma unroll
             for (int q = 0; q < 4; ++q) {
-                const f32x4 v = f32x4{acc[pb][b][4 * q], acc[pb][b][4 * q + 1], acc[pb][b][4 * q + 2], acc[pb][b][4 * q + 3]} + r[q];
-                __builtin_amdgcn_raw_buffer_store_b128(__builtin_bit_cast(__attribute__((__vector_size__(4 * sizeof(unsigned)))) unsigned, v), o_rsrc, vo, so + q * 32, 0);
+                f32x4 av = f32x4{acc[pb][b][4 * q], acc[pb][b][4 * q + 1], acc[pb][b][4 * q + 2], acc[pb][b][4 * q + 3]};
+                if constexpr (PLANES) asm volatile("s_nop 0" : "+v"(av));
+                const f32x4 v = av + r[q];
+                __builtin_amdgcn_raw_buffer_store_b128(__builtin_bit_cast(__attribute__((__vector_size__(4 * sizeof(unsigned)))) unsigned, v), o_rsrc, evo, so + q * 32, 0);
 #pragma unroll
                 for (int e = 0; e < 4; ++e) { s1 += v[e]; s2 = __builtin_fmaf(v[e], v[e], s2); }
             }
-            if (a.stats) {
+            if (!PLANES && a.stats) {
                 s1 += __shfl_xor(s1, 32, 64);
                 s2 += __shfl_xor(s2, 32, 64);
-                if (lk == 0)
-                    *reinterpret_cast<f32x2 *>(a.stats + (((size_t)cur.n * a.stats_rows + cur.p0 / 32 + pb) * a.Cout + cur.co0 + 32 * b + l31) * 2) = f32x2{s1, s2};
+                if (ek == 0)
+                    *reinterpret_cast<f32x2 *>(a.stats + (((size_t)cur.n * a.stats_rows + cur.p0 / 32 + pb) * a.Cout + cur.co0 + 32 * b + e31) * 2) = f32x2{s1, s2};
             }
         };
         auto ragged_block = [&](int pb, int b, int nv) __attribute__((always_inline)) {
@@ -203,21 +223,96 @@
             float s1 = 0.0f, s2 = 0.0f;
 #pragma unroll
             for (int i = 0; i < 16; ++i) {
-                const int px = 8 * (i >> 2) + 4 * lk + (i & 3);
-                const int off = px < nv ? vo + (i >> 2) * 32 + (i & 3) * 4 : OOB;
-                const float v = ACT ? acc[pb][b][i] : acc[pb][b][i] + bload(r_rsrc, off, so);
+                const int px = 8 * (i >> 2) + 4 * ek + (i & 3);
+                const int off = px < nv ? evo + (i >> 2) * 32 + (i & 3) * 4 : OOB;
+                const float v = (ACT || PLANES) ? acc[pb][b][i] : acc[pb][b][i] + bload(r_rsrc, off, so);
                 __builtin_amdgcn_raw_buffer_store_b32(__builtin_bit_cast(unsigned, v), o_rsrc, off, so, 0);
                 const float vm = px < nv ? v : 0.0f;
                 s1 += vm; s2 = __builtin_fmaf(vm, vm, s2);
             }
-            if (a.stats) {
+            if (!PLANES && a.stats) {
                 s1 += __shfl_xor(s1, 32, 64);
                 s2 += __shfl_xor(s2, 32, 64);
-                if (lk == 0)
-                    *reinterpret_cast<f32x2 *>(a.stats + (((size_t)cur.n * a.stats_rows + cur.p0 / 32 + pb) * a.Cout + cur.co0 + 32 * b + l31) * 2) = f32x2{s1, s2};
+                if (ek == 0)
+                    *reinterpret_cast<f32x2 *>(a.stats + (((size_t)cur.n * a.stats_rows + cur.p0 / 32 + pb) * a.Cout + cur.co0 + 32 * b + e31) * 2) = f32x2{s1, s2};
             }
         };
-        if (HW - cur.p0 >= BP) {
+        if constexpr (PLANES) {
+            const int ntiles = (HW + 31) / 32;
+            const int head_bytes = ntiles * attn::TILE_CHUNKS * 16;
+            const __amdgpu_buffer_rsrc_t p_rsrc = __builtin_amdgcn_make_buffer_rsrc(
+                (void *)((char *)a.kv_planes + (size_t)cur.n * a.kv_heads * head_bytes), 0, a.kv_heads * head_bytes, 0x00020000);
+            float *const kt = lds + (ACT ? NW * Ctot * 2 : 0) + swave * KTILE;
+            constexpr int SW = NPB == 2 ? 2 : 4;
+            const f32x4 z4 = {0.0f, 0.0f, 0.0f, 0.0f};
+            const f32x4 r0[4] = {z4, z4, z4, z4};
+            auto kv_block = [&](int pb, int b, bool is_v, int nv) __attribute__((always_inline)) {
+                const int co = cur.co0 + 32 * b;
+                const int hi = (co >> 5) & 1;
+                const int to = (co / 192) * head_bytes + (cur.p0 / 32 + pb) * (attn::TILE_CHUNKS * 16);
+                if (is_v) {
+#pragma unroll
+                    for (int j = 0; j < 2; ++j)
+#pragma unroll
+                        for (int e0 = 0; e0 < 8; e0 += 2 * SW) {
+                            unsigned h[3][SW];
+#pragma unroll
+                            for (int e = e0; e < e0 + 2 * SW; e += 2) {
+                                const int px = 16 * j + 8 * (e >> 2) + 4 * ek + (e & 3);
+                                const attn::Split3 s = attn::split3(px < nv ? acc[pb][b][8 * j + e] : 0.0f, px + 1 < nv ? acc[pb][b][8 * j + e + 1] : 0.0f);
+#pragma unroll
+                                for (int p = 0; p < 3; ++p) h[p][(e - e0) / 2] = s.h[p];
+                            }
+#pragma unroll
+                            for (int p = 0; p < 3; ++p)
+                                store_words<SW>(h[p], p_rsrc, (4 * e31 + ek) * 16, to + (3 * attn::PCHUNK + p * attn::PCHUNK + 128 * hi + 2 * j) * 16 + e0 * 2);
+                            __builtin_amdgcn_sched_barrier(0);
+                        }
+                } else {
+                    __builtin_amdgcn_wave_barrier();
+#pragma unroll
+                    for (int q = 0; q < 4; ++q) {
+                        f32x4 v;
+#pragma unroll
+                        for (int e = 0; e < 4; ++e) v[e] = 8 * q + 4 * ek + e < nv ? acc[pb][b][4 * q + e] : 0.0f;
+                        *reinterpret_cast<f32x4 *>(kt + e31 * KTP + 8 * q + 4 * ek) = v;
+                    }
+                    __builtin_amdgcn_fence(__ATOMIC_RELEASE, "wavefront");
+                    __builtin_amdgcn_wave_barrier();
+                    __builtin_amdgcn_fence(__ATOMIC_ACQUIRE, "wavefront");
+#pragma unroll
+                    for (int n = 0; n < 2; ++n) {
+                        const int s_key = (ln >> 2) + 16 * n, cg = ln & 3;
+#pragma unroll
+                        for (int e0 = 0; e0 < 8; e0 += 2 * SW) {
+                            unsigned h[3][SW];
+#pragma unroll
+                            for (int e = e0; e < e0 + 2 * SW; e += 2) {
+                                const attn::Split3 s = attn::split3(kt[(8 * cg + e) * KTP + s_key], kt[(8 * cg + e + 1) * KTP + s_key]);
+#pragma unroll
+                                for (int p = 0; p < 3; ++p) h[p][(e - e0) / 2] = s.h[p];
+                            }
+#pragma unroll
+                            for (int p = 0; p < 3; ++p)
+                                store_words<SW>(h[p], p_rsrc, (8 * s_key + cg) * 16, to + (p * attn::PCHUNK + 4 * hi) * 16 + e0 * 2);
+                            __builtin_amdgcn_sched_barrier(0);
+                        }
+                    }
+                }
+            };
+#pragma unroll
+            for (int pb = 0; pb < NPB; ++pb) {
+                const int nv = HW - cur.p0 - 32 * pb;
+                if (nv > 0) {
+#pragma unroll
+                    for (int b = 0; b < 4; ++b) {
+                        const int sec = ((cur.co0 + 32 * b) >> 6) % 3;
+                        if (sec == 0) { if (nv >= 32) block(pb, b, r0); else ragged_block(pb, b, nv); }
+                        else kv_block(pb, b, sec == 2, nv < 32 ? nv : 32);
+                    }
+                }
+            }
+        } else if (HW - cur.p0 >= BP) {
             if (has_res) {
                 f32x4 r[2][4];
                 auto fetch = [&](int t) __attribute__((always_inline)) {
@@ -285,12 +380,24 @@
 
 int conv_pw_stats_rows(const ConvArgs &a) { return cdiv((long)a.Ho * a.Wo, 32); }
 
+static size_t pw_lds_bytes(const ConvArgs &a, bool planes)
+{
+    return ((a.act ? (size_t)NW * (a.C1 + a.C2) * 2 : 0) + (planes ? (size_t)NW * KTILE : 0)) * sizeof(float);
+}
+
+bool conv_pw_planes_ok(const ConvArgs &a, int heads)
+{
+    if (!conv_pw_layer_ok(a) || heads <= 0 || a.Cout != heads * 192 || a.res || a.C2) return false;
+    const long sample_bytes = (long)heads * cdiv((long)a.Ho * a.Wo, attn::PLANE_KT) * attn::TILE_CHUNKS * 16;
+    return sample_bytes < (1L << 31) && pw_lds_bytes(a, true) <= 64 * 1024;
+}
+
 namespace {
-template <int NPB>
+template <int NPB, bool PLANES>
 const void *pw_kernel(bool act, bool planar)
 {
-    return act ? (planar ? (const void *)conv_pw_kernel<true, true, NPB> : (const void *)conv_pw_kernel<true, false, NPB>)
-               : (planar ? (const void *)conv_pw_kernel<false, true, NPB> : (const void *)conv_pw_kernel<false, false, NPB>);
+    return act ? (planar ? (const void *)conv_pw_kernel<true, true, NPB, PLANES> : (const void *)conv_pw_kernel<true, false, NPB, PLANES>)
+               : (planar ? (const void *)conv_pw_kernel<false, true, NPB, PLANES> : (const void *)conv_pw_kernel<false, false, NPB, PLANES>);
 }
 }
 
@@ -300,6 +407,8 @@
     IPDM_REQUIRE(conv_pw_eligible(a, a.stats != nullptr), "conv2d_pw: not a layer of this kernel");
     IPDM_REQUIRE(!a.x1_planar || (!(a.Ho & 1) && !(a.Wo & 1)), "conv2d_pw: parity-planar source of odd size %dx%d", a.Ho, a.Wo);
     const int HW = a.Ho * a.Wo, Ctot = a.C1 + a.C2;
+    const bool planes = a.kv_planes != nullptr;
+    IPDM_REQUIRE(!planes || (conv_pw_planes_ok(a, a.kv_heads) && !a.stats), "conv2d_pw: not a qkv projection of %d heads the plane epilogue takes", a.kv_heads);
     IPDM_REQUIRE(!a.stats || a.stats_rows == conv_pw_stats_rows(a), "conv2d_pw: statistics rows %d != %d", a.stats_rows, conv_pw_stats_rows(a));
     const int cus = device_cu_count();
     a.co_tiles = a.Cout / BN;
@@ -313,13 +422,15 @@
     IPDM_REQUIRE(nitems < (1L << 31), "conv2d_pw: too many items");
     long G = cdiv(nitems, NW) < cus ? cdiv(nitems, NW) : cus;
     G = (G + 7) / 8 * 8;
-    const size_t lds_bytes = a.act ? (size_t)NW * Ctot * 2 * sizeof(float) : 0;
+    const size_t lds_bytes = pw_lds_bytes(a, planes);
     IPDM_REQUIRE(lds_bytes <= 64 * 1024, "conv2d_pw: %d input channels exceed the scale/shift tables", Ctot);
     const bool prof = prof_enabled();
     if (prof) prof_before(1, st);
     int ni = (int)nitems;
     void *params[] = {&a, &ni};
-    (void)hipLaunchKernel(npb == 2 ? pw_kernel<2>(a.act, a.x1_planar) : pw_kernel<1>(a.act, a.x1_planar), dim3((unsigned)G), dim3(512), params, lds_bytes, st);
+    const void *kernel = planes ? (npb == 2 ? pw_kernel<2, true>(a.act, a.x1_planar) : pw_kernel<1, true>(a.act, a.x1_planar))
+                                : (npb == 2 ? pw_kernel<2, false>(a.act, a.x1_planar) : pw_kernel<1, false>(a.act, a.x1_planar));
+    (void)hipLaunchKernel(kernel, dim3((unsigned)G), dim3(512), params, lds_bytes, st);
     if (prof) prof_after(1, 2.0 * a.B * HW * (double)a.Cout * Ctot, st);
     IPDM_LAUNCH_CHECK();
     return IPDM_OK;
diff --git a/ipdm-pytorch_amd/csrc/ops.hip b/ipdm-pytorch_amd/csrc/ops.hip
--- a/ipdm-pytorch_amd/csrc/ops.hip
+++ b/ipdm-pytorch_amd/csrc/ops.hip
@@ -107,6 +107,52 @@
     if (const int rc = put_plan_buffers(s, conv_plan(a, false, true), a, st)) return rc;
     if (const int rc = conv2d_launch(a, st)) return rc;
     return finish(st);
+}
+
+extern "C" int ipdm_op_qkv_planes(const float *d_x, int32_t C, int32_t B, int32_t H, int32_t W, const float *w_host, int32_t heads,
+                                  int32_t act, int32_t groups, const float *gamma_host, const float *beta_host, int32_t x_planar,
+                                  int32_t fused, float *d_qkv, void *d_planes, void *stream)
+{
+    IPDM_REQUIRE(d_x && w_host && d_qkv && d_planes && C > 0 && B > 0 && H > 0 && W > 0 && heads > 0, "op_qkv_planes: bad argument");
+    IPDM_REQUIRE(C == heads * 64, "op_qkv_planes: %d channels are not %d heads of dim 64", C, heads);
+    IPDM_REQUIRE(act == 0 || (act == 1 && gamma_host && beta_host && groups > 0), "op_qkv_planes: act is 0 or 1 (GroupNorm with gamma/beta/groups)");
+    IPDM_REQUIRE(!x_planar || (!(H & 1) && !(W & 1)), "op_qkv_planes: parity-planar source of odd size %dx%d", H, W);
+    IPDM_REQUIRE(attention_planes_floats(B, heads, 64, H * W), "op_qkv_planes: the options in force leave attention without planes");
+    hipStream_t st = (hipStream_t)stream;
+    PackedConv L;
+    conv_pack_layer(w_host, 3 * C, C, 1, 1, false, L);
+    ConvArgs a = conv_args(B, C, 0, H, W, H, W, 3 * C, 1, 1, L.interleave, L.cout_pad);
+    a.x1 = d_x; a.act = act; a.out = d_qkv; a.x1_planar = x_planar ? 1 : 0;
+    DevScratch s(st);
+    if (const int rc = put_conv(s, L, nullptr, a)) return rc;
+    IPDM_REQUIRE(!(fused || x_planar) || conv_plan(a, false, true).code == 10, "op_qkv_planes: this layer does not run on the pointwise kernel");
+    IPDM_REQUIRE(!fused || conv_pw_planes_ok(a, heads), "op_qkv_planes: the plane epilogue does not take this layer");
+    if (act) {
+        GnTables t;
+        if (const int rc = gn_tables(s, gamma_host, beta_host, B, C, groups, t)) return rc;
+        if (const int rc = gn_fill(t, nullptr, 0, d_x, C, nullptr, 0, B, (long)H * W, groups, st)) return rc;
+        a.gn_scale = t.scale; a.gn_shift = t.shift;
+    }
+    if (fused) { a.kv_planes = (float *)d_planes; a.kv_heads = heads; }
+    else if (const int rc = put_plan_buffers(s, conv_plan(a, false, true), a, st)) return rc;
+    if (const int rc = conv2d_launch(a, st)) return rc;
+    if (!fused) {
+        attention_presplit_launch(d_qkv, (float *)d_planes, B, heads, H * W, st);
+        IPDM_LAUNCH_CHECK();
+    }
+    return finish(st);
+}
+
+extern "C" int32_t ipdm_qkv_planes_fused(int32_t B, int32_t C, int32_t heads, int32_t H, int32_t W)
+{
+    if (B <= 0 || C <= 0 || heads <= 0 || H <= 0 || W <= 0 || C % heads) return -1;
+    if (C / heads != 64) return 0;
+    static float dummy;
+    const int il = conv_weight_interleave(3 * C, 1, 1);
+    ConvArgs a = conv_args(B, C, 0, H, W, H, W, 3 * C, 1, 1, il, conv_cout_pad(3 * C, il));
+    a.x1 = a.w = a.out = &dummy;
+    a.act = 1;
+    return conv_qkv_planes_fused(a, heads) ? 1 : 0;
 }
 
 extern "C" int ipdm_op_up_conv_chain(const float *d_x, int32_t C, int32_t B, int32_t Hs, int32_t Ws, const float *wA_host,
@@ -246,6 +292,41 @@
     return time_launches(2, iters, avg_ms, [&] { return attention_launch(d_qkv, d_out, B, heads, d, T, nullptr, d_scr, d_pl); });
 }
 
+extern "C" int ipdm_bench_qkv_attention(int32_t B, int32_t C, int32_t heads, int32_t H, int32_t W, int32_t iters, float *avg_ms)
+{
+    IPDM_REQUIRE(avg_ms && iters > 0 && B > 0 && heads > 0 && H > 0 && W > 0 && C == heads * 64, "bench_qkv_attention: bad argument");
+    const int T = H * W;
+    std::vector<float> w((size_t)3 * C * C);
+    for (size_t i = 0; i < w.size(); ++i) w[i] = ((float)((i * 2654435761u) % 2001) / 1000.0f - 1.0f) / 16.0f;
+    PackedConv L;
+    conv_pack_layer(w.data(), 3 * C, C, 1, 1, false, L);
+    ConvArgs a = conv_args(B, C, 0, H, W, H, W, 3 * C, 1, 1, L.interleave, L.cout_pad);
+    a.act = 1;
+    DevScratch s(nullptr);
+    if (const int rc = s.put_layer(L, a)) return rc;
+    auto randn = [&](int rows, int64_t n, size_t pad, int seed, const float **out) {
+        const int rc = s.get(nullptr, ((size_t)rows * n + pad) * sizeof(float), out);
+        return rc ? rc : ipdm_randn(const_cast<float *>(*out), rows, n, seed, 0, 0, nullptr);
+    };
+    if (const int rc = randn(B, (int64_t)C * T, 0, 1, &a.x1)) return rc;
+    if (const int rc = randn(1, (int64_t)B * C, 64, 4, &a.gn_scale)) return rc;
+    if (const int rc = randn(1, (int64_t)B * C, 64, 5, &a.gn_shift)) return rc;
+    float *d_out = nullptr, *d_scr = nullptr, *d_pl = nullptr;
+    if (const int rc = s.get(nullptr, (size_t)B * 3 * C * T * sizeof(float), &a.out)) return rc;
+    if (const int rc = s.get(nullptr, (size_t)B * C * T * sizeof(float), &d_out)) return rc;
+    if (const size_t n = attention_scratch_floats(B, heads, 64, T))
+        if (const int rc = s.get(nullptr, n * sizeof(float), &d_scr)) return rc;
+    if (const size_t n = attention_planes_floats(B, heads, 64, T))
+        if (const int rc = s.get(nullptr, n * sizeof(float), &d_pl)) return rc;
+    const bool fused = d_pl && conv_qkv_planes_fused(a, heads);
+    if (fused) { a.kv_planes = d_pl; a.kv_heads = heads; }
+    else if (const int rc = put_plan_buffers(s, conv_plan(a, false, true), a, nullptr)) return rc;
+    return time_launches(2, iters, avg_ms, [&] {
+        const int rc = conv2d_launch(a, nullptr);
+        return rc ? rc : attention_launch(a.out, d_out, B, heads, 64, T, nullptr, d_scr, d_pl, fused);
+    });
+}
+
 extern "C" int32_t ipdm_conv_layout_code(int32_t Cout, int32_t ksize, int32_t stride)
 {
     return conv_weight_interleave(Cout, ksize, stride);
diff --git a/ipdm-pytorch_amd/csrc/unet.hip b/ipdm-pytorch_amd/csrc/unet.hip
--- a/ipdm-pytorch_amd/csrc/unet.hip
+++ b/ipdm-pytorch_amd/csrc/unet.hip
@@ -678,7 +678,8 @@
 
     Tensor *conv(const Tensor *x1, const Tensor *x2, const ConvP &cp, int stride, int act, const float *bias,
                  const Tensor *res, int H, int W, float *ext_out = nullptr, bool want_stats = false,
-                 const Tensor *sk_x1 = nullptr, const Tensor *sk_x2 = nullptr, const ConvP *sk = nullptr)
+                 const Tensor *sk_x1 = nullptr, const Tensor *sk_x2 = nullptr, const ConvP *sk = nullptr,
+                 Tensor *kv_planes = nullptr, int kv_heads = 0)
     {
         ConvArgs a = conv_args(net->B, x1->C, x2 ? x2->C : 0, x1->H, x1->W, H, W, cp.cout, cp.ks, stride, cp.interleave, cp.cout_pad);
         const int Ho = a.Ho, Wo = a.Wo;
@@ -722,6 +723,7 @@
         if (sk) { a.sk_x1 = ptr(sk_x1); a.sk_x2 = sk_x2 ? ptr(sk_x2) : nullptr; }
         if (plan.split_ws_bytes) a.split_ws = (float *)(net->ws + split_off);
         if (o->nst) { a.stats = (float *)(net->ws + o->st_off); a.stats_rows = plan.stats_rows; }
+        if (kv_planes) { a.kv_planes = wptr(kv_planes); a.kv_heads = kv_heads; }
         rc = conv2d_launch(a, net->st);
 #if IPDM_UNET_TRACE
         if (!rc) trace_conv(a, (size_t)net->B * cp.cout * Ho * Wo, net->st);
@@ -772,15 +774,24 @@
         const AttnP &ap = net->attn[l.prefix];
         const int H = x->H, W = x->W;
         gn(x, nullptr, ap.n);
-        Tensor *qkv = conv(x, nullptr, ap.qkv, 1, 1, nullptr, nullptr, H, W);
+        const int heads = net->cfg.num_heads, hd = x->C / heads;
+        const size_t pfl = attention_planes_floats(net->B, heads, hd, H * W);
+        const auto make_planes = [&] { return make((int)((pfl + (size_t)net->B * H * W - 1) / ((size_t)net->B * H * W)), H, W); };
+        bool fused = false;
+        if (pfl && hd == 64 && !x->planar) {
+            ConvArgs q = conv_args(net->B, x->C, 0, H, W, H, W, ap.qkv.cout, ap.qkv.ks, 1, ap.qkv.interleave, ap.qkv.cout_pad);
+            conv_set_images(q, ap.qkv.img[net->transposed ? 1 : 0]);
+            q.act = 1;
+            fused = conv_qkv_planes_fused(q, heads);
+        }
+        Tensor *pl = fused ? make_planes() : nullptr;
+        Tensor *qkv = conv(x, nullptr, ap.qkv, 1, 1, nullptr, nullptr, H, W, nullptr, false, nullptr, nullptr, nullptr, pl, heads);
         Tensor *a = make(x->C, H, W);
-        const int heads = net->cfg.num_heads, hd = x->C / heads;
         const size_t sfl = attention_scratch_floats(net->B, heads, hd, H * W);
         Tensor *scr = sfl ? make((int)((sfl + (size_t)net->B * H * W - 1) / ((size_t)net->B * H * W)), H, W) : nullptr;
-        const size_t pfl = attention_planes_floats(net->B, heads, hd, H * W);
-        Tensor *pl = pfl ? make((int)((pfl + (size_t)net->B * H * W - 1) / ((size_t)net->B * H * W)), H, W) : nullptr;
+        if (pfl && !fused) pl = make_planes();
         if (!rc && !net->dry)
-            rc = attention_launch(ptr(qkv), wptr(a), net->B, heads, hd, H * W, net->st, scr ? wptr(scr) : nullptr, pl ? wptr(pl) : nullptr);
+            rc = attention_launch(ptr(qkv), wptr(a), net->B, heads, hd, H * W, net->st, scr ? wptr(scr) : nullptr, pl ? wptr(pl) : nullptr, fused);
         if (pl) release(pl);
         if (scr) release(scr);
         release(qkv);
diff --git a/ipdm-pytorch_amd/csrc/unet_kernels.h b/ipdm-pytorch_amd/csrc/unet_kernels.h
--- a/ipdm-pytorch_amd/csrc/unet_kernels.h
+++ b/ipdm-pytorch_amd/csrc/unet_kernels.h
@@ -47,6 +47,8 @@
     int up2 = 0;
     int dbg = 0;
     unsigned long long *dbg_buf = nullptr;
+    float *kv_planes = nullptr;
+    int kv_heads = 0;
 };
 
 struct ConvPlan {
@@ -87,6 +89,8 @@
 int conv2d_wino3_launch(const ConvArgs &prepared, hipStream_t st);
 bool conv_pw_eligible(const ConvArgs &a, bool stats);
 int conv2d_pw_launch(const ConvArgs &a, hipStream_t st);
+bool conv_pw_planes_ok(const ConvArgs &a, int heads);
+bool conv_qkv_planes_fused(const ConvArgs &a, int heads);
 int conv_igemm_stats_rows(const ConvArgs &a);
 int conv_direct_stats_rows(const ConvArgs &a);
 int conv_ws_stats_rows(const ConvArgs &a);
@@ -124,11 +128,12 @@
 int gn_stats_launch(const GnArgs &a, hipStream_t st);
 
 int attention_launch(const float *qkv, float *out, int B, int heads, int d, int T, hipStream_t st, float *scratch = nullptr,
-                     float *planes = nullptr);
+                     float *planes = nullptr, bool planes_filled = false);
+void attention_presplit_launch(const float *qkv, float *planes, int B, int heads, int T, hipStream_t st);
 size_t attention_scratch_floats(int B, int heads, int d, int T);
 size_t attention_planes_floats(int B, int heads, int d, int T);
 void attention_bx3_launch(const float *qkv, float *out, int B, int heads, int T, float scale, int Z, bool seq, float *scratch, float *planes,
-                          hipStream_t st);
+                          hipStream_t st, bool planes_filled = false);
 constexpr int ATTN_GEN_DMAX = 128;
 int attention_gen_split(int heads, int d, int T);
 int attention_gen_launch(const float *qkv, float *out, int B, int heads, int d, int T, float scale, int Z, float *scratch, hipStream_t st);
```

Result: no change. 2.190, median of 4 (+0.4%).
